# jewettaij/visfd

Hardware: AMD Instinct MI355X
Metric: Mvoxels/s (Gauss+DoG+TV pipeline) on 1024^3 float32; % HBM roofline (higher is better)
Workload: dtype f32

## Files before the change

include/visfd_hip.h:

```cpp
#ifndef VISFD_HIP_H
#define VISFD_HIP_H

#include <stddef.h>
#include <stdint.h>

#ifdef __cplusplus
extern "C" {
#endif

#define VISFD_HIP_OK 0
#define VISFD_HIP_EINVAL 1
#define VISFD_HIP_EDEVICE 2
#define VISFD_HIP_ENOMEM 3
#define VISFD_HIP_ECAPACITY 4

#define VISFD_HIP_INCREASING_EIVALS 0
#define VISFD_HIP_DECREASING_EIVALS 1

typedef struct visfd_hip_ctx visfd_hip_ctx;

int visfd_hip_create(int device, void* stream, visfd_hip_ctx** out);
int visfd_hip_destroy(visfd_hip_ctx* ctx);
int visfd_hip_synchronize(visfd_hip_ctx* ctx);
void* visfd_hip_get_stream(visfd_hip_ctx* ctx);
// ... 146 lines not shown
                              float threshold_tensor_saliency, float threshold_tensor_neighbor,
                              int tensor_is_positive_definite_near_target, int connectivity,
                              int64_t label_undefined, int sort_by_size, int standardize_directions,
                              int start_from_saliency_maxima, int64_t* n_clusters, float* cluster_maxima,
                              float* cluster_sizes, float* cluster_saliencies, int64_t cluster_capacity);
int visfd_hip_label_connected_ex(const float* saliency, int64_t* labels, const float* mask, int64_t nx, int64_t ny,
                              int64_t nz, float threshold_saliency, float* direction,
                              float threshold_vector_saliency, float threshold_vector_neighbor,
                              int consider_dot_product_sign, const float* tensor,
                              float threshold_tensor_saliency, float threshold_tensor_neighbor,
                              int tensor_is_positive_definite_near_target, int connectivity,
                              int64_t label_undefined, int sort_by_size, int standardize_directions,
                              int start_from_saliency_maxima, int64_t* n_clusters, float* cluster_maxima,
                              float* cluster_sizes, float* cluster_saliencies, int64_t cluster_capacity,
                                 const float* voxel_weights, const float* must_link_crds,
                                 const int64_t* must_link_group_sizes, int64_t must_link_ngroups,
                                 const int* must_link_directions);

int visfd_hip_principal_directions_host(const float* tensor, const float* mask, int64_t nvox, int order,
                                        float* direction);
int visfd_hip_tensor_saliency_host(const float* tensor, const float* mask, int64_t nvox, int order,
                                   float* saliency);

int visfd_hip_diagonalize_flat_sym3_host(const float* m6, float* out6, int64_t n, int eival_order);
int visfd_hip_convert_flat_sym2_evects3_host(const float* m6, int eival_order, float* eivals3, float* eivects9);
int visfd_hip_diagonalize_sym3_f32_host(const float* m9, int order, float* eivals3, float* eivects9);
int visfd_hip_surface_points(const float* saliency, const float* voxel2cluster, const float* direction,
                             const float* mask, int64_t nx, int64_t ny, int64_t nz, int select_cluster,
                             const float voxel_width[3], float curve_ds, int find_ridge,
                             float max_distance_to_feature, float* crds, float* norms, int64_t capacity,
                             int64_t* n_points);

int visfd_hip_bin_array3d(visfd_hip_ctx*, const float* src, const int64_t size_src[3], float* dst,
                          const int64_t size_dst[3], const int* offset);
int visfd_hip_bin_array3d_dev(visfd_hip_ctx*, const float* src, const int64_t size_src[3], float* dst,
                              const int64_t size_dst[3], const int* offset);
int visfd_hip_unbin_array3d(visfd_hip_ctx*, const float* src, const int64_t size_src[3], float* dst,
                            const int64_t size_dst[3], const int* offset);
int visfd_hip_unbin_array3d_dev(visfd_hip_ctx*, const float* src, const int64_t size_src[3], float* dst,
                                const int64_t size_dst[3], const int* offset);

int visfd_hip_calc_hessian(visfd_hip_ctx*, const float* src, float* gradient, float* hessian,
                           const float* mask, int64_t nx, int64_t ny, int64_t nz, float sigma,
                           float truncate_ratio);
int visfd_hip_calc_hessian_dev(visfd_hip_ctx*, const float* src, float* gradient, float* hessian,
                               const float* mask, int64_t nx, int64_t ny, int64_t nz, float sigma,
                               float truncate_ratio);

int visfd_hip_diagonalize_flat_sym3(visfd_hip_ctx*, const float* m6, float* out6, int64_t n,
                                    int eival_order);
int visfd_hip_diagonalize_flat_sym3_dev(visfd_hip_ctx*, const float* m6, float* out6, int64_t n,
                                        int eival_order);

int visfd_hip_hessian_saliency(visfd_hip_ctx*, const float* hessian, const float* mask,
                               int64_t nvox, int eival_order, float* saliency, float* direction);
int visfd_hip_hessian_saliency_dev(visfd_hip_ctx*, const float* hessian, const float* mask,
                                   int64_t nvox, int eival_order, float* saliency,
                                   float* direction);
int visfd_hip_ridge_saliency_dev(visfd_hip_ctx*, const float* src, const float* mask,
                                 int64_t nx, int64_t ny, int64_t nz, float sigma,
                                 float truncate_ratio, int eival_order, float* saliency,
                                 float* direction);
int visfd_hip_ridge_scores_dev(visfd_hip_ctx*, const float* src, const float* mask, int64_t nx, int64_t ny,
                               int64_t nz, float sigma, float truncate_ratio, int eival_order, float* saliency,
                               float* smoothed);
int visfd_hip_ridge_directions_dev(visfd_hip_ctx*, const float* smoothed, int64_t nx, int64_t ny, int64_t nz,
                                   float sigma, int eival_order, const float* saliency, float* direction);
int visfd_hip_peak_background_dev(visfd_hip_ctx*, const float* image, const float* mask, int64_t nx, int64_t ny, int64_t nz,
                                  float sigma_background, float truncate_ratio, int normalize, float* background);
int visfd_hip_ridge_scores_bg_dev(visfd_hip_ctx*, const float* src, const float* mask, int64_t nx, int64_t ny,
                                  int64_t nz, float sigma, float truncate_ratio, int eival_order, const float* background,
                                  float* saliency, float* smoothed);

int visfd_hip_threshold_fraction(visfd_hip_ctx*, float* saliency, const float* mask, int64_t nvox,
                                 float fraction, float* threshold_out);
int visfd_hip_threshold_fraction_dev(visfd_hip_ctx*, float* saliency, const float* mask,
                                     int64_t nvox, float fraction, float* threshold_out);
int visfd_hip_select_histogram_dev(visfd_hip_ctx*, const float* saliency, const float* mask,
                                   int64_t nvox, int round, uint32_t prefix,
                                   uint64_t* hist_host , uint64_t* n_unmasked_host);
int visfd_hip_select_histogram_todev(visfd_hip_ctx*, const float* saliency, const float* mask, int64_t nvox, int round,
                                     uint32_t prefix, uint64_t* hist_dev );
int visfd_hip_apply_threshold_dev(visfd_hip_ctx*, float* saliency, int64_t nvox, float threshold);

int visfd_hip_tv_dense_stick(visfd_hip_ctx*, const float* saliency, const float* direction,
                             float* tensor, const float* mask_src, const float* mask_dst,
                             int64_t nx, int64_t ny, int64_t nz, float sigma_tv, int exponent,
                             float cutoff_ratio, int detect_curves);
int visfd_hip_tv_dense_stick_dev(visfd_hip_ctx*, const float* saliency, const float* direction,
                                 float* tensor, const float* mask_src, const float* mask_dst,
                                 int64_t nx, int64_t ny, int64_t nz, float sigma_tv, int exponent,
                                 float cutoff_ratio, int detect_curves);
int visfd_hip_tv_dense_stick_slab_dev(visfd_hip_ctx*, const float* saliency, const float* direction,
                                      float* tensor, const float* mask_src, const float* mask_dst,
                                      int64_t nx, int64_t ny, int64_t nz_local, int64_t z_out0,
                                      int64_t z_out1, float sigma_tv, int exponent,
                                      float cutoff_ratio, int detect_curves);
int visfd_hip_tv_weight_sum(visfd_hip_ctx*, const float* saliency, float* den, const float* mask_src, const float* mask_dst,
                            int64_t nx, int64_t ny, int64_t nz, float sigma_tv, float cutoff_ratio);
int visfd_hip_tv_tables(float sigma_tv, float cutoff_ratio, int* halfwidth_out, float* w,
                        float* rhat);

int visfd_hip_tensor_saliency(visfd_hip_ctx*, const float* tensor, const float* mask, int64_t nvox,
                              int eival_order, float* saliency_inout);
int visfd_hip_tensor_saliency_dev(visfd_hip_ctx*, const float* tensor, const float* mask,
                                  int64_t nvox, int eival_order, float* saliency_inout);
int visfd_hip_tensor_saliency_bg_dev(visfd_hip_ctx*, const float* tensor, const float* mask, int64_t nvox, int eival_order,
                                     const float* image, const float* background, float* saliency_inout);

int visfd_hip_membrane_detect(visfd_hip_ctx*, const float* src, const float* mask,
                              int64_t nx, int64_t ny, int64_t nz, float sigma, float truncate_ratio,
                              int eival_order, float best_fraction, float threshold_abs, float sigma_tv,
                              int tv_exponent, float tv_cutoff_ratio, float* saliency_out,
                              float* tensor_out, float* direction_out, float* threshold_out);
int visfd_hip_membrane_detect_dev(visfd_hip_ctx*, const float* src, const float* mask,
                                  int64_t nx, int64_t ny, int64_t nz, float sigma, float truncate_ratio,
                                  int eival_order, float best_fraction, float threshold_abs,
                                  float sigma_tv, int tv_exponent, float tv_cutoff_ratio,
                                  float* saliency_out, float* tensor_out, float* direction_out,
                                  float* threshold_out);
int visfd_hip_membrane_detect_bg(visfd_hip_ctx*, const float* src, const float* mask,
                                 int64_t nx, int64_t ny, int64_t nz, float sigma, float truncate_ratio,
                                 int eival_order, float best_fraction, float threshold_abs, float sigma_tv,
                                 int tv_exponent, float tv_cutoff_ratio, float sigma_background, int normalize_background,
                                 float* saliency_out, float* tensor_out, float* direction_out, float* threshold_out);
int visfd_hip_membrane_detect_bg_dev(visfd_hip_ctx*, const float* src, const float* mask,
                                     int64_t nx, int64_t ny, int64_t nz, float sigma, float truncate_ratio,
                                     int eival_order, float best_fraction, float threshold_abs,
                                     float sigma_tv, int tv_exponent, float tv_cutoff_ratio, float sigma_background,
                                     int normalize_background, float* saliency_out, float* tensor_out, float* direction_out,
                                     float* threshold_out);

int visfd_hip_apply_gauss_slab_dev(visfd_hip_ctx*, const float* src, float* dst,
                                   int64_t nx, int64_t ny, int64_t nz_local, int64_t z_lo,
                                   int64_t nz_global, const float sigma[3], const int halfwidth[3],
                                   int normalize, float* A_out);

typedef struct visfd_hip_slab visfd_hip_slab;
typedef struct visfd_hip_transport {
  int (*sendrecv)(void* user, int peer, const void* sendbuf, void* recvbuf, size_t bytes, void* stream);
  int (*allreduce_sum_u64)(void* user, uint64_t* buf, size_t count, void* stream);
  int (*group_start)(void* user);
  int (*group_end)(void* user);
  void* user;
} visfd_hip_transport;
int visfd_hip_slab_unique_id(void* id_out_128_bytes);
int visfd_hip_slab_rccl_available(void);
int visfd_hip_slab_create_rccl(visfd_hip_ctx*, const void* unique_id_128_bytes , int rank,
                               int world, int64_t nz_global, int ghost, visfd_hip_slab** out);
int visfd_hip_slab_create_custom(visfd_hip_ctx*, const visfd_hip_transport*, int rank, int world, int64_t nz_global,
                                 int ghost, visfd_hip_slab** out);
int visfd_hip_slab_destroy(visfd_hip_slab*);
int visfd_hip_slab_layout(visfd_hip_slab*, int64_t out[7]);
int visfd_hip_slab_selftest(visfd_hip_slab*, int64_t count);
int visfd_hip_slab_set_reserve(visfd_hip_slab*, int reserve_workgroups);
int visfd_hip_slab_exchange_dev(visfd_hip_slab*, float* const* volumes, int nvol, int64_t nx, int64_t ny, int depth);
int visfd_hip_membrane_detect_slab_dev(visfd_hip_slab*, float* src, float* sal, float* dirs, float* tensor, float* scratch,
                                       int64_t nx, int64_t ny, float sigma, float truncate_ratio, int eival_order,
                                       float best_fraction, float sigma_tv, int exponent, float tv_truncate_ratio,
                                       int src_halo_ready, float* threshold_out);
int visfd_hip_membrane_detect_slab(visfd_hip_slab*, const float* src_owned, int64_t nx, int64_t ny, float sigma,
                                   float truncate_ratio, int eival_order, float best_fraction, float sigma_tv, int exponent,
                                   float tv_truncate_ratio, float* sal_owned, float* tensor_owned, float* threshold_out);
int visfd_hip_membrane_detect_slab_bg_dev(visfd_hip_slab*, float* src, float* sal, float* dirs, float* tensor, float* scratch,
                                          float* background, int64_t nx, int64_t ny, float sigma, float truncate_ratio,
                                          int eival_order, float best_fraction, float sigma_tv, int exponent,
                                          float tv_truncate_ratio, float sigma_background, int normalize_background,
                                          int src_halo_ready, float* threshold_out);
int visfd_hip_membrane_detect_slab_bg(visfd_hip_slab*, const float* src_owned, int64_t nx, int64_t ny, float sigma,
                                      float truncate_ratio, int eival_order, float best_fraction, float sigma_tv, int exponent,
                                      float tv_truncate_ratio, float sigma_background, int normalize_background,
                                      float* sal_owned, float* tensor_owned, float* threshold_out);
int visfd_hip_blob_dog_slab_dev(visfd_hip_slab*, float* src, int64_t nx, int64_t ny, const float* blob_sigma, int n_sigma,
                                float delta_sigma_over_sigma, float truncate_ratio, float minima_threshold,
                                float maxima_threshold, int src_halo_ready,
                                visfd_hip_blob* minima, int64_t minima_capacity, int64_t* n_minima,
                                visfd_hip_blob* maxima, int64_t maxima_capacity, int64_t* n_maxima);
int visfd_hip_blob_halo_depth(const float* blob_sigma, int n_sigma, float delta_sigma_over_sigma, float truncate_ratio,
                              int* depth_out);
int visfd_hip_apply_gauss_slab(visfd_hip_slab*, const float* src_owned, int64_t nx, int64_t ny, const float sigma[3],
                               const int halfwidth[3], int normalize, float* dst_owned, float* A_out);
int visfd_hip_blob_dog_slab(visfd_hip_slab*, const float* src_owned, int64_t nx, int64_t ny, const float* blob_sigma, int n_sigma,
                            float delta_sigma_over_sigma, float truncate_ratio, float minima_threshold, float maxima_threshold,
                            visfd_hip_blob* minima, int64_t minima_capacity, int64_t* n_minima,
                            visfd_hip_blob* maxima, int64_t maxima_capacity, int64_t* n_maxima);

#ifdef __cplusplus
}
#endif
#endif
```

visfd_amd/api.py:

```python
import ctypes as C
import os
import sys

import numpy as np

_HERE = os.path.dirname(os.path.abspath(__file__))
LIB_PATH = os.environ.get("VISFD_HIP_LIB") or os.path.join(_HERE, "libvisfd_hip.so")

INCREASING_EIVALS = 0
DECREASING_EIVALS = 1

MORPH_DILATE, MORPH_ERODE, MORPH_OPEN, MORPH_CLOSE, MORPH_TOP_HAT_WHITE, MORPH_TOP_HAT_BLACK = range(6)
MORPH_PATH_GENERAL, MORPH_PATH_XRUNS = 0, 1

_fp = C.POINTER(C.c_float)
_ip = C.POINTER(C.c_int)
_i64 = C.c_int64
_vp = C.c_void_p


class VisfdHipError(RuntimeError):
    def __init__(self, code, msg):
        super().__init__("visfd_hip error %d: %s" % (code, msg))
        self.code = code
# ... 15 lines not shown
    "visfd_hip_trim": (C.c_int, [_vp]),
    "visfd_hip_last_error": (C.c_char_p, []),
    "visfd_hip_abi_version": (C.c_int, []),
    "visfd_hip_workspace_bytes": (_i64, [_vp]),
    "visfd_hip_set_option": (C.c_int, [_vp, C.c_char_p, _i64]),
    "visfd_hip_get_option": (C.c_int, [_vp, C.c_char_p, C.POINTER(C.c_int64)]),
    "visfd_hip_gauss_taps": (C.c_int, [C.c_float, C.c_int, _fp]),
    "visfd_hip_ratio_from_threshold": (C.c_float, [C.c_float]),
    "visfd_hip_local_fluctuations": (C.c_int, [_vp, _vp, _vp, _vp, _i64, _i64, _i64, _fp, C.c_float, C.c_float, C.c_int]),
    "visfd_hip_local_fluctuations_dev": (C.c_int, [_vp, _vp, _vp, _vp, _i64, _i64, _i64, _fp, C.c_float, C.c_float, C.c_int]),
    "visfd_hip_sphere_structure": (C.c_int, [C.c_float, C.c_float, C.c_float, _ip, _fp, _i64, C.POINTER(C.c_int64)]),
    "visfd_hip_morph_sphere": (C.c_int, [_vp] + _VOL + [C.c_int, C.c_float, C.c_float, C.c_float]),
    "visfd_hip_morph_sphere_dev": (C.c_int, [_vp] + _VOL + [C.c_int, C.c_float, C.c_float, C.c_float]),
    "visfd_hip_morph_table": (C.c_int, [_vp] + _VOL + [C.c_int, _ip, _fp, _i64]),
    "visfd_hip_morph_table_dev": (C.c_int, [_vp] + _VOL + [C.c_int, _ip, _fp, _i64]),
    "visfd_hip_morph_last_path": (C.c_int, [_vp, _ip]),
    "visfd_hip_find_extrema": (C.c_int, [_vp, _vp, _vp, _i64, _i64, _i64] + _EXTREMA_TAIL),
    "visfd_hip_find_extrema_dev": (C.c_int, [_vp, _vp, _vp, _i64, _i64, _i64] + _EXTREMA_TAIL),
    "visfd_hip_fluctuation_sigmas": (C.c_int, [_fp, C.c_float, C.c_float, C.c_float, _fp, C.POINTER(C.c_float)]),
    "visfd_hip_gauss_halfwidths": (C.c_int, [_fp, C.c_float, _ip]),
    "visfd_hip_separable3d": (C.c_int, [_vp] + _VOL + [_fp, C.c_int, _fp, C.c_int, _fp, C.c_int, C.c_int, _fp]),
    "visfd_hip_separable3d_dev": (C.c_int, [_vp] + _VOL + [_fp, C.c_int, _fp, C.c_int, _fp, C.c_int, C.c_int, _fp]),
    "visfd_hip_apply_gauss": (C.c_int, [_vp] + _VOL + [_fp, _ip, C.c_int, _fp]),
    "visfd_hip_apply_gauss_dev": (C.c_int, [_vp] + _VOL + [_fp, _ip, C.c_int, _fp]),
    "visfd_hip_apply_gauss_slab_dev": (C.c_int, [_vp, _vp, _vp, _i64, _i64, _i64, _i64, _i64, _fp, _ip, C.c_int, _fp]),
    "visfd_hip_apply_dog": (C.c_int, [_vp] + _VOL + [_fp, _fp, _ip, _fp, _fp]),
    "visfd_hip_apply_dog_dev": (C.c_int, [_vp] + _VOL + [_fp, _fp, _ip, _fp, _fp]),
    "visfd_hip_apply_log": (C.c_int, [_vp] + _VOL + [_fp, C.c_float, C.c_float, _fp, _fp]),
    "visfd_hip_apply_log_dev": (C.c_int, [_vp] + _VOL + [_fp, C.c_float, C.c_float, _fp, _fp]),
    "visfd_hip_blob_dog": (C.c_int, [_vp, _vp, _vp, _i64, _i64, _i64, _fp, C.c_int, _fp, C.c_float, C.c_float,
                                     C.c_float, C.c_float, C.c_int, C.POINTER(Blob), _i64, C.POINTER(_i64),
                                     C.POINTER(Blob), _i64, C.POINTER(_i64)]),
    "visfd_hip_blob_dog_dev": (C.c_int, [_vp, _vp, _vp, _i64, _i64, _i64, _fp, C.c_int, _fp, C.c_float, C.c_float,
                                         C.c_float, C.c_float, C.c_int, C.POINTER(Blob), _i64, C.POINTER(_i64),
                                         C.POINTER(Blob), _i64, C.POINTER(_i64)]),
    "visfd_hip_blob_dog_begin_dev": (C.c_int, [_vp, _vp, _vp, _i64, _i64, _i64, _fp, C.c_int, _fp, C.c_float, C.c_float,
                                               C.c_float, C.c_float, C.c_int, C.POINTER(_vp)]),
    "visfd_hip_blob_dog_end": (C.c_int, [_vp, C.POINTER(Blob), _i64, C.POINTER(_i64), C.POINTER(Blob), _i64, C.POINTER(_i64)]),
    "visfd_hip_blob_dog_abort": (None, [_vp]),
    "visfd_hip_blob_jobs_pending": (C.c_int, [_vp]),
    "visfd_hip_debug_poison_workspace": (C.c_int, [_vp]),
    "visfd_hip_blob_diameters_to_sigmas": (C.c_int, [_fp, C.c_int, _fp]),
    "visfd_hip_blob_sigmas_to_diameters": (C.c_int, [_fp, C.c_int, _fp]),
    "visfd_hip_calc_hessian": (C.c_int, [_vp, _vp, _vp, _vp, _vp, _i64, _i64, _i64, C.c_float, C.c_float]),
    "visfd_hip_calc_hessian_dev": (C.c_int, [_vp, _vp, _vp, _vp, _vp, _i64, _i64, _i64, C.c_float, C.c_float]),
    "visfd_hip_diagonalize_flat_sym3": (C.c_int, [_vp, _vp, _vp, _i64, C.c_int]),
    "visfd_hip_diagonalize_flat_sym3_dev": (C.c_int, [_vp, _vp, _vp, _i64, C.c_int]),
    "visfd_hip_hessian_saliency": (C.c_int, [_vp, _vp, _vp, _i64, C.c_int, _vp, _vp]),
    "visfd_hip_hessian_saliency_dev": (C.c_int, [_vp, _vp, _vp, _i64, C.c_int, _vp, _vp]),
    "visfd_hip_ridge_saliency_dev": (C.c_int, [_vp, _vp, _vp, _i64, _i64, _i64, C.c_float, C.c_float, C.c_int,
                                               _vp, _vp]),
    "visfd_hip_ridge_scores_dev": (C.c_int, [_vp, _vp, _vp, _i64, _i64, _i64, C.c_float, C.c_float, C.c_int, _vp, _vp]),
    "visfd_hip_ridge_directions_dev": (C.c_int, [_vp, _vp, _i64, _i64, _i64, C.c_float, C.c_int, _vp, _vp]),
    "visfd_hip_threshold_fraction": (C.c_int, [_vp, _vp, _vp, _i64, C.c_float, _fp]),
    "visfd_hip_threshold_fraction_dev": (C.c_int, [_vp, _vp, _vp, _i64, C.c_float, _fp]),
    "visfd_hip_select_histogram_dev": (C.c_int, [_vp, _vp, _vp, _i64, C.c_int, C.c_uint32,
                                                 C.POINTER(C.c_uint64), C.POINTER(C.c_uint64)]),
    "visfd_hip_select_histogram_todev": (C.c_int, [_vp, _vp, _vp, _i64, C.c_int, C.c_uint32, _vp]),
    "visfd_hip_get_stream": (_vp, [_vp]),
    "visfd_hip_apply_threshold_dev": (C.c_int, [_vp, _vp, _i64, C.c_float]),
    "visfd_hip_tv_dense_stick": (C.c_int, [_vp, _vp, _vp, _vp, _vp, _vp, _i64, _i64, _i64, C.c_float, C.c_int,
                                           C.c_float, C.c_int]),
    "visfd_hip_tv_dense_stick_dev": (C.c_int, [_vp, _vp, _vp, _vp, _vp, _vp, _i64, _i64, _i64, C.c_float, C.c_int,
                                               C.c_float, C.c_int]),
    "visfd_hip_tv_dense_stick_slab_dev": (C.c_int, [_vp, _vp, _vp, _vp, _vp, _vp, _i64, _i64, _i64, _i64, _i64,
                                                    C.c_float, C.c_int, C.c_float, C.c_int]),
    "visfd_hip_tv_tables": (C.c_int, [C.c_float, C.c_float, _ip, _fp, _fp]),
    "visfd_hip_tv_weight_sum": (C.c_int, [_vp, _vp, _vp, _vp, _vp, _i64, _i64, _i64, C.c_float, C.c_float]),
    "visfd_hip_membrane_detect": (C.c_int, [_vp, _vp, _vp, _i64, _i64, _i64, C.c_float, C.c_float, C.c_int, C.c_float,
                                            C.c_float, C.c_float, C.c_int, C.c_float, _vp, _vp, _vp, _fp]),
    "visfd_hip_membrane_detect_dev": (C.c_int, [_vp, _vp, _vp, _i64, _i64, _i64, C.c_float, C.c_float, C.c_int,
                                                C.c_float, C.c_float, C.c_float, C.c_int, C.c_float, _vp, _vp, _vp,
                                                _fp]),
    "visfd_hip_tensor_saliency": (C.c_int, [_vp, _vp, _vp, _i64, C.c_int, _vp]),
    "visfd_hip_tensor_saliency_dev": (C.c_int, [_vp, _vp, _vp, _i64, C.c_int, _vp]),
    "visfd_hip_peak_background_dev": (C.c_int, [_vp, _vp, _vp, _i64, _i64, _i64, C.c_float, C.c_float, C.c_int, _vp]),
    "visfd_hip_ridge_scores_bg_dev": (C.c_int, [_vp, _vp, _vp, _i64, _i64, _i64, C.c_float, C.c_float, C.c_int, _vp, _vp, _vp]),
    "visfd_hip_tensor_saliency_bg_dev": (C.c_int, [_vp, _vp, _vp, _i64, C.c_int, _vp, _vp, _vp]),
    "visfd_hip_membrane_detect_bg": (C.c_int, [_vp, _vp, _vp, _i64, _i64, _i64, C.c_float, C.c_float, C.c_int, C.c_float,
                                               C.c_float, C.c_float, C.c_int, C.c_float, C.c_float, C.c_int, _vp, _vp, _vp, _fp]),
    "visfd_hip_membrane_detect_bg_dev": (C.c_int, [_vp, _vp, _vp, _i64, _i64, _i64, C.c_float, C.c_float, C.c_int,
                                                   C.c_float, C.c_float, C.c_float, C.c_int, C.c_float, C.c_float, C.c_int,
                                                   _vp, _vp, _vp, _fp]),
    "visfd_hip_membrane_detect_slab_bg_dev": (C.c_int, [_vp, _vp, _vp, _vp, _vp, _vp, _vp, _i64, _i64, C.c_float, C.c_float, C.c_int,
                                                        C.c_float, C.c_float, C.c_int, C.c_float, C.c_float, C.c_int, C.c_int, _fp]),
    "visfd_hip_membrane_detect_slab_bg": (C.c_int, [_vp, _vp, _i64, _i64, C.c_float, C.c_float, C.c_int, C.c_float, C.c_float,
                                                    C.c_int, C.c_float, C.c_float, C.c_int, _vp, _vp, _fp]),
    "visfd_hip_bin_array3d": (C.c_int, [_vp, _vp, C.POINTER(_i64), _vp, C.POINTER(_i64), _ip]),
    "visfd_hip_bin_array3d_dev": (C.c_int, [_vp, _vp, C.POINTER(_i64), _vp, C.POINTER(_i64), _ip]),
    "visfd_hip_unbin_array3d": (C.c_int, [_vp, _vp, C.POINTER(_i64), _vp, C.POINTER(_i64), _ip]),
    "visfd_hip_unbin_array3d_dev": (C.c_int, [_vp, _vp, C.POINTER(_i64), _vp, C.POINTER(_i64), _ip]),
    "visfd_hip_label_connected": (C.c_int, [_vp, _vp, _vp, _i64, _i64, _i64, C.c_float, _vp, C.c_float, C.c_float, C.c_int,
                                            _vp, C.c_float, C.c_float, C.c_int, C.c_int, _i64, C.c_int, C.c_int, C.c_int,
                                            C.POINTER(_i64), _vp, _vp, _vp, _i64]),
    "visfd_hip_label_connected_ex": (C.c_int, [_vp, _vp, _vp, _i64, _i64, _i64, C.c_float, _vp, C.c_float, C.c_float, C.c_int,
                                               _vp, C.c_float, C.c_float, C.c_int, C.c_int, _i64, C.c_int, C.c_int, C.c_int,
                                               C.POINTER(_i64), _vp, _vp, _vp, _i64, _vp, _vp, _vp, _i64, _vp]),
    "visfd_hip_principal_directions_host": (C.c_int, [_vp, _vp, _i64, C.c_int, _vp]),
    "visfd_hip_tensor_saliency_host": (C.c_int, [_vp, _vp, _i64, C.c_int, _vp]),
    "visfd_hip_diagonalize_sym3_f32_host": (C.c_int, [_vp, C.c_int, _vp, _vp]),
    "visfd_hip_diagonalize_flat_sym3_host": (C.c_int, [_vp, _vp, _i64, C.c_int]),
    "visfd_hip_convert_flat_sym2_evects3_host": (C.c_int, [_vp, C.c_int, _vp, _vp]),
    "visfd_hip_surface_points": (C.c_int, [_vp, _vp, _vp, _vp, _i64, _i64, _i64, C.c_int, _fp, C.c_float, C.c_int, C.c_float,
                                           _vp, _vp, _i64, C.POINTER(_i64)]),
    "visfd_hip_sphere_overlap": (C.c_float, [C.c_float, C.c_float, C.c_float]),
    "visfd_hip_sort_blobs": (C.c_int, [_fp, _fp, _fp, _i64, C.c_int, C.c_int, C.POINTER(C.c_uint64)]),
    "visfd_hip_discard_masked_blobs": (C.c_int, [_fp, _fp, _fp, C.POINTER(_i64), _vp, _i64, _i64, _i64]),
    "visfd_hip_discard_overlapping_blobs": (C.c_int, [_fp, _fp, _fp, C.POINTER(_i64), C.c_float, C.c_float,
                                                     C.c_float, C.c_int, C.c_int]),
    "visfd_hip_slab_unique_id": (C.c_int, [_vp]),
    "visfd_hip_slab_create_rccl": (C.c_int, [_vp, _vp, C.c_int, C.c_int, _i64, C.c_int, C.POINTER(_vp)]),
    "visfd_hip_slab_create_custom": (C.c_int, [_vp, _vp, C.c_int, C.c_int, _i64, C.c_int, C.POINTER(_vp)]),
    "visfd_hip_slab_destroy": (C.c_int, [_vp]),
    "visfd_hip_slab_layout": (C.c_int, [_vp, C.POINTER(_i64)]),
    "visfd_hip_slab_set_reserve": (C.c_int, [_vp, C.c_int]),
    "visfd_hip_slab_rccl_available": (C.c_int, []),
    "visfd_hip_apply_gauss_slab": (C.c_int, [_vp, _vp, _i64, _i64, _fp, _ip, C.c_int, _vp, _fp]),
    "visfd_hip_blob_dog_slab": (C.c_int, [_vp, _vp, _i64, _i64, _fp, C.c_int, C.c_float, C.c_float, C.c_float, C.c_float,
                                          _vp, _i64, C.POINTER(_i64), _vp, _i64, C.POINTER(_i64)]),
    "visfd_hip_blob_halo_depth": (C.c_int, [_fp, C.c_int, C.c_float, C.c_float, _ip]),
    "visfd_hip_slab_selftest": (C.c_int, [_vp, _i64]),
    "visfd_hip_slab_exchange_dev": (C.c_int, [_vp, C.POINTER(_vp), C.c_int, _i64, _i64, C.c_int]),
    "visfd_hip_membrane_detect_slab_dev": (C.c_int, [_vp, _vp, _vp, _vp, _vp, _vp, _i64, _i64, C.c_float, C.c_float, C.c_int,
                                                     C.c_float, C.c_float, C.c_int, C.c_float, C.c_int, _fp]),
    "visfd_hip_membrane_detect_slab": (C.c_int, [_vp, _vp, _i64, _i64, C.c_float, C.c_float, C.c_int, C.c_float, C.c_float,
                                                 C.c_int, C.c_float, _vp, _vp, _fp]),
    "visfd_hip_blob_dog_slab_dev": (C.c_int, [_vp, _vp, _i64, _i64, _fp, C.c_int, C.c_float, C.c_float, C.c_float, C.c_float,
                                              C.c_int, _vp, _i64, C.POINTER(_i64), _vp, _i64, C.POINTER(_i64)]),
}

_SENDRECV = C.CFUNCTYPE(C.c_int, _vp, C.c_int, _vp, _vp, C.c_size_t, _vp)
_ALLREDUCE = C.CFUNCTYPE(C.c_int, _vp, _vp, C.c_size_t, _vp)
_GROUP = C.CFUNCTYPE(C.c_int, _vp)


class Transport(C.Structure):
    _fields_ = [("sendrecv", _SENDRECV), ("allreduce_sum_u64", _ALLREDUCE), ("group_start", _GROUP), ("group_end", _GROUP),
                ("user", _vp)]

_lib = None


def load_library():
    global _lib
    if _lib is None:
        if not os.path.exists(LIB_PATH):
            raise ImportError("%s is missing: build it with `python -m visfd_amd.build` "
                              "(there is no CPU fallback)" % LIB_PATH)
        try:
            import torch
        except ImportError:
            pass
        lib = C.CDLL(LIB_PATH)
        for name, (res, args) in _SIGS.items():
            fn = getattr(lib, name)
            fn.restype = res
            fn.argtypes = args
        _lib = lib
    return _lib


def exported_symbols():
    return sorted(_SIGS)


def _np(a):
# ... 540 lines not shown
        self._chk(self._L.visfd_hip_hessian_saliency(self._h, _np(hess), _np(mask), sal.size, int(order), _np(sal),
                                                     _np(dirs)))
        return sal, dirs

    def threshold_fraction(self, sal, fraction, mask=None):
        thr = C.c_float()
        self._chk(self._L.visfd_hip_threshold_fraction(self._h, _np(sal), _np(mask), sal.size, float(fraction),
                                                       C.byref(thr)))
        return thr.value

    def tv_dense_stick(self, sal, dirs, sigma_tv, exponent=4, cutoff=2.0 ** 0.5, mask_src=None, mask_dst=None,
                       curves=False):
        nz, ny, nx = sal.shape
        tensor = np.zeros((nz, ny, nx, 6), np.float32)
        self._chk(self._L.visfd_hip_tv_dense_stick(self._h, _np(sal), _np(dirs), _np(tensor), _np(mask_src),
                                                   _np(mask_dst), nx, ny, nz, float(sigma_tv), int(exponent),
                                                   float(cutoff), int(curves)))
        return tensor

    def tv_weight_sum(self, sal, sigma_tv, cutoff=2.0 ** 0.5, mask_src=None, mask_dst=None):
        nz, ny, nx = sal.shape
        den = np.zeros_like(sal)
        self._chk(self._L.visfd_hip_tv_weight_sum(self._h, _np(sal), _np(den), _np(mask_src), _np(mask_dst), nx, ny, nz,
                                                  float(sigma_tv), float(cutoff)))
        return den

    def tensor_saliency(self, tensor, order, sal_inout, mask=None):
        self._chk(self._L.visfd_hip_tensor_saliency(self._h, _np(tensor), _np(mask), sal_inout.size, int(order),
                                                    _np(sal_inout)))
        return sal_inout

    @staticmethod
    def _sizes(shape):
        return (_i64 * 3)(int(shape[2]), int(shape[1]), int(shape[0]))

    def bin_array3d(self, src, dst_shape, offset=None):
        dst = np.empty(tuple(dst_shape), np.float32)
        self._chk(self._L.visfd_hip_bin_array3d(self._h, _np(src), self._sizes(src.shape), _np(dst),
                                                self._sizes(dst_shape), _i3(offset) if offset is not None else None))
        return dst

    def unbin_array3d(self, src, dst_shape, offset=None):
        dst = np.empty(tuple(dst_shape), np.float32)
        self._chk(self._L.visfd_hip_unbin_array3d(self._h, _np(src), self._sizes(src.shape), _np(dst),
                                                  self._sizes(dst_shape), _i3(offset) if offset is not None else None))
        return dst

    def bin_array3d_dev(self, src, dst, offset=None):
        self._chk(self._L.visfd_hip_bin_array3d_dev(self._h, _dev(src), self._sizes(src.shape), _dev(dst),
                                                    self._sizes(dst.shape), _i3(offset) if offset is not None else None))

    def unbin_array3d_dev(self, src, dst, offset=None):
        self._chk(self._L.visfd_hip_unbin_array3d_dev(self._h, _dev(src), self._sizes(src.shape), _dev(dst),
                                                      self._sizes(dst.shape), _i3(offset) if offset is not None else None))

    def membrane_detect(self, src, sigma, ratio, order, best_fraction=0.05, threshold_abs=0.0, sigma_tv=0.0,
                        tv_exponent=4, tv_cutoff=2.0 ** 0.5, mask=None, want_tensor=True, want_dir=False,
                        sigma_background=0.0, normalize_background=True):
        nz, ny, nx = src.shape
        sal = np.empty_like(src)
        ten = np.zeros((nz, ny, nx, 6), np.float32) if want_tensor else None
        dirs = np.zeros((nz, ny, nx, 3), np.float32) if want_dir else None
        thr = C.c_float()
        self._chk(self._L.visfd_hip_membrane_detect_bg(self._h, _np(src), _np(mask), nx, ny, nz, float(sigma),
                                                       float(ratio), int(order), float(best_fraction),
                                                       float(threshold_abs), float(sigma_tv), int(tv_exponent),
                                                       float(tv_cutoff), float(sigma_background), int(bool(normalize_background)),
                                                       _np(sal), _np(ten), _np(dirs), C.byref(thr)))
        return sal, ten, dirs, thr.value

    def membrane_detect_dev(self, src, sal, sigma, ratio, order, best_fraction=0.05, threshold_abs=0.0, sigma_tv=0.0,
                            tv_exponent=4, tv_cutoff=2.0 ** 0.5, mask=None, dirs=None, tensor=None, sigma_background=0.0,
                            normalize_background=True):
        nz, ny, nx = src.shape
        thr = C.c_float()
        self._chk(self._L.visfd_hip_membrane_detect_bg_dev(self._h, _dev(src), _dev(mask), nx, ny, nz, float(sigma),
                                                           float(ratio), int(order), float(best_fraction),
                                                           float(threshold_abs), float(sigma_tv), int(tv_exponent),
                                                           float(tv_cutoff), float(sigma_background),
                                                           int(bool(normalize_background)), _dev(sal), _dev(tensor), _dev(dirs),
                                                           C.byref(thr)))
        return thr.value

    def gauss_dev(self, src, dst, sigma, hw, mask=None, normalize=True):
        nz, ny, nx = src.shape
        A = C.c_float()
        self._chk(self._L.visfd_hip_apply_gauss_dev(self._h, _dev(src), _dev(dst), _dev(mask), nx, ny, nz,
                                                    _f3(sigma), _i3(hw), int(normalize), C.byref(A)))
        return A.value

    def local_fluctuations_dev(self, src, dst, sigma, ratio, mask=None, normalize=True, exponent=2.0):
        nz, ny, nx = src.shape
        self._chk(self._L.visfd_hip_local_fluctuations_dev(self._h, _dev(src), _dev(dst), _dev(mask), nx, ny, nz,
                                                           _f3(sigma), float(exponent), float(ratio), int(normalize)))

    def morph_sphere_dev(self, op, src, dst, radius, radius_max=0.0, bmax=0.0, mask=None):
        nz, ny, nx = src.shape
        self._chk(self._L.visfd_hip_morph_sphere_dev(self._h, _dev(src), _dev(dst), _dev(mask), nx, ny, nz, int(op),
                                                     float(radius), float(radius_max), float(bmax)))

    def dilate_sphere_dev(self, src, dst, radius, radius_max=0.0, bmax=0.0, mask=None):
        self.morph_sphere_dev(MORPH_DILATE, src, dst, radius, radius_max, bmax, mask)

    def erode_sphere_dev(self, src, dst, radius, radius_max=0.0, bmax=0.0, mask=None):
        self.morph_sphere_dev(MORPH_ERODE, src, dst, radius, radius_max, bmax, mask)

    def open_sphere_dev(self, src, dst, radius, radius_max=0.0, bmax=0.0, mask=None):
        self.morph_sphere_dev(MORPH_OPEN, src, dst, radius, radius_max, bmax, mask)

    def close_sphere_dev(self, src, dst, radius, radius_max=0.0, bmax=0.0, mask=None):
        self.morph_sphere_dev(MORPH_CLOSE, src, dst, radius, radius_max, bmax, mask)

    def white_top_hat_sphere_dev(self, src, dst, radius, radius_max=0.0, bmax=0.0, mask=None):
        self.morph_sphere_dev(MORPH_TOP_HAT_WHITE, src, dst, radius, radius_max, bmax, mask)

    def black_top_hat_sphere_dev(self, src, dst, radius, radius_max=0.0, bmax=0.0, mask=None):
        self.morph_sphere_dev(MORPH_TOP_HAT_BLACK, src, dst, radius, radius_max, bmax, mask)

    def find_extrema_dev(self, src, mask=None, find_minima=True, find_maxima=True, minima_threshold=float("inf"),
                         maxima_threshold=-float("inf"), connectivity=3, allow_borders=True, labels=None):
        if labels is not None:
            assert labels.is_cuda and labels.is_contiguous() and str(labels.dtype) == "torch.int32" and \
                tuple(labels.shape) == tuple(src.shape), "labels: contiguous cuda int32 of src's shape"
        return tuple(self._find_extrema(self._L.visfd_hip_find_extrema_dev, _dev(src), _dev(mask), tuple(src.shape),
                                        find_minima, find_maxima, minima_threshold, maxima_threshold, connectivity,
                                        allow_borders, None if labels is None else labels.data_ptr()))

    def morph_table_dev(self, op, src, dst, dxyz, b, mask=None):
        nz, ny, nx = src.shape
        d, bb = _morph_table(dxyz, b)
        self._chk(self._L.visfd_hip_morph_table_dev(self._h, _dev(src), _dev(dst), _dev(mask), nx, ny, nz, int(op),
                                                    d.ctypes.data_as(_ip), bb.ctypes.data_as(_fp), len(bb)))

    def dilate_dev(self, src, dst, dxyz, b, mask=None):
        self.morph_table_dev(MORPH_DILATE, src, dst, dxyz, b, mask)

    def erode_dev(self, src, dst, dxyz, b, mask=None):
        self.morph_table_dev(MORPH_ERODE, src, dst, dxyz, b, mask)

    def gauss_slab_dev(self, src, dst, z_lo, nz_global, sigma, hw, normalize=True):
        nz, ny, nx = src.shape
        A = C.c_float()
        self._chk(self._L.visfd_hip_apply_gauss_slab_dev(self._h, _dev(src), _dev(dst), nx, ny, nz, int(z_lo),
                                                         int(nz_global), _f3(sigma), _i3(hw), int(normalize),
                                                         C.byref(A)))
        return A.value

    def log_dev(self, src, dst, sigma, delta, ratio, mask=None):
        nz, ny, nx = src.shape
        self._chk(self._L.visfd_hip_apply_log_dev(self._h, _dev(src), _dev(dst), _dev(mask), nx, ny, nz,
                                                  _f3(sigma), float(delta), float(ratio), None, None))

    def blob_dog_dev(self, src, sigmas, mask=None, aspect=None, delta=0.02, ratio=2.5, minima_threshold=np.inf,
                     maxima_threshold=-np.inf, use_ratios=False, cap=1 << 16):
        return self._blob_call(self._L.visfd_hip_blob_dog_dev, _dev(src), _dev(mask), tuple(src.shape), sigmas,
                               aspect, delta, ratio, minima_threshold, maxima_threshold, use_ratios, cap)

    def calc_hessian_dev(self, src, grad, hess, sigma, ratio, mask=None):
        nz, ny, nx = src.shape
        self._chk(self._L.visfd_hip_calc_hessian_dev(self._h, _dev(src), _dev(grad), _dev(hess), _dev(mask), nx,
                                                     ny, nz, float(sigma), float(ratio)))

    def hessian_saliency_dev(self, hess, sal, dirs, order, mask=None):
        self._chk(self._L.visfd_hip_hessian_saliency_dev(self._h, _dev(hess), _dev(mask), sal.numel(), int(order),
                                                         _dev(sal), _dev(dirs)))

# ... 265 lines not shown
```

visfd_amd/build.py:

```python
import concurrent.futures
import os
import subprocess
import sys
import time

HERE = os.path.dirname(os.path.abspath(__file__))
ROOT = os.path.dirname(HERE)
CSRC = os.path.join(HERE, "csrc")
OBJDIR = os.path.join(ROOT, "build", "visfd_hip")
LIB = os.path.join(HERE, "libvisfd_hip.so")

SOURCES = ["host_math.cpp", "blob_post.cpp", "connect.cpp", "context.hip", "api.hip", "blob_job.hip", "gauss.hip", "blob.hip", "select.hip", "tv.hip", "resample.hip", "slab.hip", "morph.hip", "extrema.hip"]
TV_VARIANT = [("tv_tiled.hip", "tv_tiled", ["-fno-slp-vectorize"]), ("tv_box.hip", "tv_box", ["-fno-slp-vectorize"]),
              ("ridge.hip", "ridge", [])]
VARIANTS = TV_VARIANT + [("gauss_fused.hip", "gauss_fused_h%d" % h, ["-DVH_FUSED_H=%d" % h, "-fno-slp-vectorize"])
                         for h in range(1, 9)]
HEADERS = ["common.hpp", "eigen3.hpp", os.path.join("..", "..", "include", "visfd_hip.h")]

HIPCC = os.environ.get("HIPCC", "/opt/rocm/bin/hipcc")
FLAGS = ["--offload-arch=gfx950", "-O3", "-std=c++17", "-fPIC", "-ffp-contract=off", "-fno-fast-math",
         "-Wall", "-Wno-unused-function"]


def _mtime(p):
    return os.path.getmtime(p) if os.path.exists(p) else 0.0


def _compile(src, obj, extra=()):
    t0 = time.time()
    cmd = [HIPCC] + FLAGS + list(extra) + ["-x", "hip", "-c", os.path.join(CSRC, src), "-o", obj]
    r = subprocess.run(cmd, capture_output=True, text=True)
    return src, r.returncode, r.stdout + r.stderr, time.time() - t0


def build(force=False, jobs=4, verbose=True):
    os.makedirs(OBJDIR, exist_ok=True)
    newest_header = max(_mtime(os.path.join(CSRC, h)) for h in HEADERS)
    todo, objs = [], []
    units = [(s, os.path.splitext(s)[0], []) for s in SOURCES] + VARIANTS
    flagfile = os.path.join(OBJDIR, "flags.txt")
    flagsig = repr((FLAGS, VARIANTS))
    if not os.path.exists(flagfile) or open(flagfile).read() != flagsig:
        force = True
    for s, stem, extra in units:
        obj = os.path.join(OBJDIR, stem + ".o")
        objs.append(obj)
        if force or _mtime(obj) < max(_mtime(os.path.join(CSRC, s)), newest_header):
            todo.append((s, obj, extra))
    if todo:
        with concurrent.futures.ThreadPoolExecutor(max_workers=jobs) as ex:
            for (src, rc, out, dt), (_, obj, _e) in zip(ex.map(lambda a: _compile(*a), todo), todo):
                if verbose:
                    print("[visfd_amd.build] %-22s %5.1fs %s" % (os.path.basename(obj), dt, "ok" if rc == 0 else "FAILED"))
                if rc != 0:
                    sys.stderr.write(out)
                    raise RuntimeError("hipcc failed on " + src)
                elif out.strip() and verbose:
                    sys.stderr.write(out)
    with open(flagfile, "w") as f:
        f.write(flagsig)
    if todo or not os.path.exists(LIB) or _mtime(LIB) < max(_mtime(o) for o in objs):
        cmd = [HIPCC, "--offload-arch=gfx950", "-shared", "-fPIC", "-o", LIB] + objs
        r = subprocess.run(cmd, capture_output=True, text=True)
        if r.returncode != 0:
            sys.stderr.write(r.stdout + r.stderr)
            raise RuntimeError("link failed")
        if verbose:
            print("[visfd_amd.build] linked", LIB)
    build_cli(verbose)
    return LIB


CLI_SRC = os.path.join(HERE, "cli", "filter_mrc.cpp")
CLI_BIN = os.path.join(HERE, "cli", "filter_mrc")


def build_cli(verbose=True):
    deps = [CLI_SRC, os.path.join(ROOT, "include", "visfd_hip.hpp"), os.path.join(ROOT, "include", "visfd_hip.h"), LIB]
    if os.path.exists(CLI_BIN) and _mtime(CLI_BIN) >= max(_mtime(d) for d in deps):
        return CLI_BIN
    cmd = ["g++", "-std=c++11", "-O2", "-Wall", "-o", CLI_BIN, CLI_SRC, "-L" + HERE, "-lvisfd_hip",
           "-Wl,-rpath,$ORIGIN/..", "-Wl,-rpath,/opt/rocm/lib"]
    r = subprocess.run(cmd, capture_output=True, text=True)
    if r.returncode != 0:
        sys.stderr.write(r.stdout + r.stderr)
        raise RuntimeError("building filter_mrc failed")
    if verbose:
        print("[visfd_amd.build] built", CLI_BIN)
    return CLI_BIN


if __name__ == "__main__":
    j = 4
    if "-j" in sys.argv:
        j = int(sys.argv[sys.argv.index("-j") + 1])
    build(force="--force" in sys.argv, jobs=j)
```

visfd_amd/csrc/api.hip:

```cpp
#include <algorithm>
#include <cmath>
#include <vector>

#include "common.hpp"

namespace vh {

int gauss_dev(visfd_hip_ctx* ctx, const float* src, float* dst, const float* mask, i64 nx, i64 ny, i64 nz,
              const float sigma[3], const int hw[3], bool normalize, SlabInfo slab, float* A_out, const float* minuend,
              float log_scale, bool* epilogue_done, bool fma) {
  VH_REQUIRE(ctx && src && dst && sigma && hw, "null argument");
  std::vector<float> t[3];
  for (int d = 0; d < 3; d++) {
    VH_REQUIRE(sigma[d] >= 0.0f, "sigma must be non-negative");
    VH_REQUIRE(hw[d] >= 0 && hw[d] <= MAX_HALFWIDTH, "filter halfwidth must be in [0, 64]");
    t[d].resize(2 * hw[d] + 1);
    host_gauss_taps(sigma[d], hw[d], t[d].data());
  }
  return dev_separable3d(ctx, src, dst, mask, nx, ny, nz, t[0].data(), hw[0], t[1].data(), hw[1],
                         t[2].data(), hw[2], normalize, slab, A_out, minuend, log_scale, epilogue_done, fma);
}

static int dog_dev(visfd_hip_ctx* ctx, const float* src, float* dst, float* tmp, const float* mask, i64 nx, i64 ny,
                   i64 nz, const float sa[3], const float sb[3], const int hw[3], float scale, bool do_scale,
                   float* A, float* B) {
  const SlabInfo whole = {0, nz};
  VH_TRY(gauss_dev(ctx, src, dst, mask, nx, ny, nz, sa, hw, true, whole, A));
  {
    bool fused = false;
    VH_TRY(gauss_dev(ctx, src, dst, mask, nx, ny, nz, sb, hw, true, whole, B, dst, do_scale ? scale : 1.0f, &fused));
    if (fused) return VISFD_HIP_OK;
  }
  VH_TRY(gauss_dev(ctx, src, tmp, mask, nx, ny, nz, sb, hw, true, whole, B));
  return dev_sub_scale(ctx, dst, tmp, nx * ny * nz, scale, do_scale);
}

LogPlan plan_log(const float sigma[3], float delta, float ratio) {
  LogPlan p;
  for (int d = 0; d < 3; d++) {
    p.sa[d] = (float)(sigma[d] * (1.0 - 0.5 * delta));
    p.sb[d] = (float)(sigma[d] * (1.0 + 0.5 * delta));
    p.hw[d] = (int)std::floor(ratio * std::fmax(p.sa[d], p.sb[d]));
  }
  p.scale = (float)(1.0 / (delta * delta));
  return p;
}

int log_dev(visfd_hip_ctx* ctx, const float* src, float* dst, float* tmp, const float* mask, i64 nx, i64 ny,
            i64 nz, const float sigma[3], float delta, float ratio, float* A, float* B) {
  const LogPlan p = plan_log(sigma, delta, ratio);
  for (int d = 0; d < 3; d++)
    VH_REQUIRE(p.hw[d] >= 0 && p.hw[d] <= MAX_HALFWIDTH, "LoG filter halfwidth must be in [0, 64]");
  float a = 0, b = 0;
  VH_TRY(dog_dev(ctx, src, dst, tmp, mask, nx, ny, nz, p.sa, p.sb, p.hw, p.scale, true, &a, &b));
  if (A) *A = a * p.scale;
  if (B) *B = b * p.scale;
  return VISFD_HIP_OK;
}

namespace {

void halfwidths_from_ratio(const float sigma[3], float ratio, int hw[3]) {
  for (int d = 0; d < 3; d++) {
    hw[d] = (int)std::floor(sigma[d] * ratio);
    if (hw[d] < 1) hw[d] = 1;
  }
}

int gauss_iso_dev(visfd_hip_ctx* ctx, const float* src, float* dst, const float* mask, i64 nx, i64 ny, i64 nz, float sigma,
                  float ratio, bool normalize, const char* what, float** out = nullptr) {
  const int hwv = (int)std::floor(sigma * ratio);
  VH_REQUIRE(hwv >= 0 && hwv <= MAX_HALFWIDTH, std::string(what) + " must be in [0, 64]");
  if (!dst) VH_TRY(ws(ctx, WS_D, (size_t)(nx * ny * nz), &dst));
  if (out) *out = dst;
  const float sg[3] = {sigma, sigma, sigma};
  const int hw[3] = {hwv, hwv, hwv};
  const SlabInfo whole = {0, nz};
  return gauss_dev(ctx, src, dst, mask, nx, ny, nz, sg, hw, normalize, whole, nullptr);
}

int calc_hessian_dev(visfd_hip_ctx* ctx, const float* src, float* grad, float* hess, const float* mask,
                     i64 nx, i64 ny, i64 nz, float sigma, float ratio) {
  VH_REQUIRE(ctx && src, "null argument");
  VH_TRY(check_dims(nx, ny, nz));
  float* S = nullptr;
  VH_TRY(gauss_iso_dev(ctx, src, nullptr, mask, nx, ny, nz, sigma, ratio, true, "filter halfwidth", &S));
  return dev_hessian(ctx, S, mask, nx, ny, nz, sigma, grad, hess);
// ... 178 lines not shown
int visfd_hip_calc_hessian_dev(visfd_hip_ctx* ctx, const float* src, float* grad, float* hess,
                               const float* mask, int64_t nx, int64_t ny, int64_t nz, float sigma,
                               float ratio) {
  VH_REQUIRE(ctx, "null context");
  VH_HIP(hipSetDevice(ctx->device));
  return calc_hessian_dev(ctx, src, grad, hess, mask, nx, ny, nz, sigma, ratio);
}

int visfd_hip_calc_hessian(visfd_hip_ctx* ctx, const float* src, float* grad, float* hess, const float* mask,
                           int64_t nx, int64_t ny, int64_t nz, float sigma, float ratio) {
  VH_REQUIRE(ctx && src, "null argument");
  VH_HIP(hipSetDevice(ctx->device));
  VH_TRY(check_dims(nx, ny, nz));
  const Stage st = {ctx, (size_t)(nx * ny * nz)};
  float *ds, *dm, *dg = nullptr, *dh = nullptr, *aos = nullptr;
  VH_TRY(st.up(WS_H2D_0, src, &ds));
  VH_TRY(st.up(WS_H2D_1, mask, &dm));
  if (grad) VH_TRY(st.out(WS_H2D_2, &dg, 3));
  if (hess) VH_TRY(st.out(WS_H2D_3, &dh, 6));
  VH_TRY(st.out(WS_H2D_4, &aos, 6));
  VH_TRY(calc_hessian_dev(ctx, ds, dg, dh, dm, nx, ny, nz, sigma, ratio));
  if (grad) VH_TRY(st.down_interleaved(grad, dg, aos, 3, dm, true));
  if (hess) VH_TRY(st.down_interleaved(hess, dh, aos, 6, dm, true));
  return VISFD_HIP_OK;
}

int visfd_hip_diagonalize_flat_sym3_dev(visfd_hip_ctx* ctx, const float* m6, float* out6, int64_t n,
                                        int order) {
  VH_REQUIRE(ctx && m6 && out6 && n >= 0, "bad argument");
  VH_REQUIRE(order == 0 || order == 1, "unsupported eigenvalue order");
  VH_HIP(hipSetDevice(ctx->device));
  if (n == 0) return VISFD_HIP_OK;
  return dev_diagonalize(ctx, m6, out6, n, order);
}

int visfd_hip_diagonalize_flat_sym3(visfd_hip_ctx* ctx, const float* m6, float* out6, int64_t n, int order) {
  VH_REQUIRE(ctx && m6 && out6 && n >= 0, "bad argument");
  VH_REQUIRE(order == 0 || order == 1, "unsupported eigenvalue order");
  VH_HIP(hipSetDevice(ctx->device));
  if (n == 0) return VISFD_HIP_OK;
  const Stage st = {ctx, (size_t)n};
  float *aos, *pin, *pout;
  VH_TRY(st.up_planar(WS_H2D_0, WS_H2D_1, m6, 6, &pin, &aos));
  VH_TRY(st.out(WS_H2D_2, &pout, 6));
  VH_TRY(dev_diagonalize(ctx, pin, pout, n, order));
  return st.down_interleaved(out6, pout, aos, 6, nullptr, false);
}

int visfd_hip_hessian_saliency_dev(visfd_hip_ctx* ctx, const float* hess, const float* mask, int64_t nvox,
                                   int order, float* sal, float* dir) {
  VH_REQUIRE(ctx && hess && sal && dir && nvox > 0, "bad argument");
  VH_REQUIRE(order == 0 || order == 1, "unsupported eigenvalue order");
  VH_HIP(hipSetDevice(ctx->device));
  return dev_hessian_saliency(ctx, hess, mask, nvox, order, sal, dir);
}

int visfd_hip_hessian_saliency(visfd_hip_ctx* ctx, const float* hess, const float* mask, int64_t nvox, int order,
                               float* sal, float* dir) {
  VH_REQUIRE(ctx && hess && sal && dir && nvox > 0, "bad argument");
  VH_REQUIRE(order == 0 || order == 1, "unsupported eigenvalue order");
  VH_HIP(hipSetDevice(ctx->device));
  const Stage st = {ctx, (size_t)nvox};
  float *aos, *ph, *dm, *dsal, *pdir;
  VH_TRY(st.up_planar(WS_H2D_0, WS_H2D_2, hess, 6, &ph, &aos));
  VH_TRY(st.up(WS_H2D_1, mask, &dm));
  VH_TRY(st.out(WS_H2D_3, &dsal));
  VH_TRY(st.out(WS_H2D_4, &pdir, 3));
  VH_TRY(dev_hessian_saliency(ctx, ph, dm, nvox, order, dsal, pdir));
  VH_TRY(st.down(sal, dsal));
  return st.down_interleaved(dir, pdir, aos, 3, dm, true);
}

int visfd_hip_ridge_saliency_dev(visfd_hip_ctx* ctx, const float* src, const float* mask, int64_t nx, int64_t ny,
                                 int64_t nz, float sigma, float ratio, int order, float* sal, float* dir) {
  VH_REQUIRE(ctx && src && sal && dir, "null argument");
  VH_REQUIRE(order == 0 || order == 1, "unsupported eigenvalue order");
  VH_HIP(hipSetDevice(ctx->device));
  VH_TRY(check_dims(nx, ny, nz));
  float* S = nullptr;
  VH_TRY(gauss_iso_dev(ctx, src, nullptr, mask, nx, ny, nz, sigma, ratio, true, "filter halfwidth", &S));
  return dev_ridge_saliency_fused(ctx, S, mask, nx, ny, nz, sigma, order, sal, dir);
}

int visfd_hip_ridge_scores_bg_dev(visfd_hip_ctx* ctx, const float* src, const float* mask, int64_t nx, int64_t ny,
                                  int64_t nz, float sigma, float ratio, int order, const float* background, float* sal,
                                  float* smoothed) {
  VH_REQUIRE(ctx && src && sal && smoothed, "null argument");
  VH_REQUIRE(smoothed != src && smoothed != sal, "the smoothed volume needs its own buffer");
  VH_REQUIRE(order == 0 || order == 1, "unsupported eigenvalue order");
  VH_HIP(hipSetDevice(ctx->device));
  VH_TRY(check_dims(nx, ny, nz));
  VH_TRY(gauss_iso_dev(ctx, src, smoothed, mask, nx, ny, nz, sigma, ratio, true, "filter halfwidth"));
  return dev_ridge_score(ctx, smoothed, mask, nx, ny, nz, sigma, order, sal, background ? src : nullptr, background);
}
int visfd_hip_ridge_scores_dev(visfd_hip_ctx* ctx, const float* src, const float* mask, int64_t nx, int64_t ny,
                               int64_t nz, float sigma, float ratio, int order, float* sal, float* smoothed) {
  return visfd_hip_ridge_scores_bg_dev(ctx, src, mask, nx, ny, nz, sigma, ratio, order, nullptr, sal, smoothed);
}
int visfd_hip_peak_background_dev(visfd_hip_ctx* ctx, const float* src, const float* mask, int64_t nx, int64_t ny,
                                  int64_t nz, float sigma_background, float ratio, int normalize, float* background) {
  VH_REQUIRE(ctx && src && background && background != src, "bad argument");
  VH_REQUIRE(sigma_background > 0.0f, "the background width must be positive");
  VH_HIP(hipSetDevice(ctx->device));
  VH_TRY(check_dims(nx, ny, nz));
  return gauss_iso_dev(ctx, src, background, mask, nx, ny, nz, sigma_background, ratio, normalize != 0,
                       "background filter halfwidth");
}

int visfd_hip_ridge_directions_dev(visfd_hip_ctx* ctx, const float* smoothed, int64_t nx, int64_t ny, int64_t nz,
                                   float sigma, int order, const float* sal, float* dir) {
  VH_REQUIRE(ctx && smoothed && sal && dir, "null argument");
  VH_REQUIRE(order == 0 || order == 1, "unsupported eigenvalue order");
  VH_HIP(hipSetDevice(ctx->device));
  VH_TRY(check_dims(nx, ny, nz));
  return dev_ridge_directions(ctx, smoothed, sal, nx, ny, nz, sigma, order, dir);
}

int visfd_hip_threshold_fraction_dev(visfd_hip_ctx* ctx, float* sal, const float* mask, int64_t nvox,
                                     float fraction, float* thr_out) {
  VH_REQUIRE(ctx && sal && nvox > 0, "bad argument");
  VH_REQUIRE(fraction >= 0.0f && fraction <= 1.0f, "fraction must be in [0,1]");
  VH_HIP(hipSetDevice(ctx->device));
  return dev_threshold_fraction(ctx, sal, mask, nvox, fraction, thr_out);
}

int visfd_hip_threshold_fraction(visfd_hip_ctx* ctx, float* sal, const float* mask, int64_t nvox, float fraction,
                                 float* thr_out) {
  VH_REQUIRE(ctx && sal && nvox > 0, "bad argument");
  VH_REQUIRE(fraction >= 0.0f && fraction <= 1.0f, "fraction must be in [0,1]");
  VH_HIP(hipSetDevice(ctx->device));
  const Stage st = {ctx, (size_t)nvox};
  float *ds, *dm;
  VH_TRY(st.up(WS_H2D_0, sal, &ds));
  VH_TRY(st.up(WS_H2D_1, mask, &dm));
  VH_TRY(dev_threshold_fraction(ctx, ds, dm, nvox, fraction, thr_out));
  return st.down(sal, ds);
}

int visfd_hip_select_histogram_dev(visfd_hip_ctx* ctx, const float* sal, const float* mask, int64_t nvox,
                                   int pass, uint32_t prefix, uint64_t* hist_host, uint64_t* n_unmasked) {
  VH_REQUIRE(ctx && sal && hist_host && nvox > 0, "bad argument");
  VH_REQUIRE(pass >= 0 && pass <= 2, "round must be 0, 1 or 2");
  VH_HIP(hipSetDevice(ctx->device));
  return dev_select_histogram(ctx, sal, mask, nvox, pass, prefix, hist_host, n_unmasked);
}

int visfd_hip_select_histogram_todev(visfd_hip_ctx* ctx, const float* sal, const float* mask, int64_t nvox, int pass,
                                     uint32_t prefix, uint64_t* hist_dev) {
  VH_REQUIRE(ctx && sal && hist_dev && nvox > 0, "bad argument");
  VH_REQUIRE(pass >= 0 && pass <= 2, "round must be 0, 1 or 2");
  VH_HIP(hipSetDevice(ctx->device));
  return dev_select_histogram_todev(ctx, sal, mask, nvox, pass, prefix, hist_dev);
}

int visfd_hip_apply_threshold_dev(visfd_hip_ctx* ctx, float* sal, int64_t nvox, float thr) {
  VH_REQUIRE(ctx && sal && nvox > 0, "bad argument");
  VH_HIP(hipSetDevice(ctx->device));
  return dev_apply_threshold(ctx, sal, nvox, thr);
}

int visfd_hip_bin_array3d_dev(visfd_hip_ctx* ctx, const float* src, const int64_t size_src[3], float* dst,
                              const int64_t size_dst[3], const int* offset) {
  VH_REQUIRE(ctx && src && dst && size_src && size_dst, "null argument");
  VH_HIP(hipSetDevice(ctx->device));
  return dev_bin_array3d(ctx, src, size_src, dst, size_dst, offset);
}

int visfd_hip_unbin_array3d_dev(visfd_hip_ctx* ctx, const float* src, const int64_t size_src[3], float* dst,
                                const int64_t size_dst[3], const int* offset) {
  VH_REQUIRE(ctx && src && dst && size_src && size_dst, "null argument");
  VH_HIP(hipSetDevice(ctx->device));
  return dev_unbin_array3d(ctx, src, size_src, dst, size_dst, offset);
}

static int resample_host(visfd_hip_ctx* ctx, const float* src, const int64_t size_src[3], float* dst, const int64_t size_dst[3],
                         const int* offset, decltype(dev_bin_array3d)* run) {
  VH_REQUIRE(ctx && src && dst && size_src && size_dst, "null argument");
  VH_HIP(hipSetDevice(ctx->device));
  VH_TRY(check_dims(size_src[0], size_src[1], size_src[2]));
  VH_TRY(check_dims(size_dst[0], size_dst[1], size_dst[2]));
  const Stage in = {ctx, (size_t)(size_src[0] * size_src[1] * size_src[2])};
  const Stage res = {ctx, (size_t)(size_dst[0] * size_dst[1] * size_dst[2])};
  float *ds, *dd;
  VH_TRY(in.up(WS_H2D_0, src, &ds));
  VH_TRY(res.out(WS_H2D_2, &dd));
  VH_TRY(run(ctx, ds, size_src, dd, size_dst, offset));
  return res.down(dst, dd);
}

int visfd_hip_bin_array3d(visfd_hip_ctx* ctx, const float* src, const int64_t size_src[3], float* dst,
                          const int64_t size_dst[3], const int* offset) {
  return resample_host(ctx, src, size_src, dst, size_dst, offset, dev_bin_array3d);
}
int visfd_hip_unbin_array3d(visfd_hip_ctx* ctx, const float* src, const int64_t size_src[3], float* dst,
                            const int64_t size_dst[3], const int* offset) {
  return resample_host(ctx, src, size_src, dst, size_dst, offset, dev_unbin_array3d);
}

int visfd_hip_tv_tables(float sigma_tv, float cutoff, int* h_out, float* w, float* rhat) {
  const int h = host_tv_halfwidth(sigma_tv, cutoff);
  VH_REQUIRE(h >= 0, "negative window");
  if (h_out) *h_out = h;
  if (w) host_tv_tables(sigma_tv, h, w, rhat);
  return VISFD_HIP_OK;
}

int visfd_hip_tv_dense_stick_slab_dev(visfd_hip_ctx* ctx, const float* sal, const float* dir, float* ten,
                                      const float* mask_src, const float* mask_dst, int64_t nx,
                                      int64_t ny, int64_t nz_local, int64_t z_out0, int64_t z_out1,
                                      float sigma_tv, int exponent, float cutoff, int curves) {
  VH_REQUIRE(ctx && sal && dir && ten, "null argument");
  VH_HIP(hipSetDevice(ctx->device));
  return dev_tv_dense_stick(ctx, sal, dir, ten, mask_src, mask_dst, nx, ny, nz_local, z_out0, z_out1,
                            sigma_tv, exponent, cutoff, curves != 0);
}

int visfd_hip_tv_dense_stick_dev(visfd_hip_ctx* ctx, const float* sal, const float* dir, float* ten,
                                 const float* mask_src, const float* mask_dst, int64_t nx, int64_t ny,
                                 int64_t nz, float sigma_tv, int exponent, float cutoff, int curves) {
  return visfd_hip_tv_dense_stick_slab_dev(ctx, sal, dir, ten, mask_src, mask_dst, nx, ny, nz, 0, nz,
                                           sigma_tv, exponent, cutoff, curves);
}

int visfd_hip_tv_dense_stick(visfd_hip_ctx* ctx, const float* sal, const float* dir, float* ten, const float* mask_src,
                             const float* mask_dst, int64_t nx, int64_t ny, int64_t nz, float sigma_tv, int exponent,
                             float cutoff, int curves) {
  VH_REQUIRE(ctx && sal && dir && ten, "null argument");
  VH_HIP(hipSetDevice(ctx->device));
  VH_TRY(check_dims(nx, ny, nz));
  const Stage st = {ctx, (size_t)(nx * ny * nz)};
  float *dsal, *pdir, *pten, *aos6, *dms = nullptr, *dmd = nullptr;
  VH_TRY(st.up(WS_H2D_0, sal, &dsal));
  VH_TRY(st.up_planar(WS_H2D_1, WS_H2D_2, dir, 3, &pdir));
  VH_TRY(st.out(WS_H2D_3, &pten, 6));
  VH_TRY(st.up(WS_H2D_4, mask_src, &dms));
  if (mask_dst == mask_src) dmd = dms;
  else VH_TRY(st.up(WS_A, mask_dst, &dmd));
  VH_TRY(dev_tv_dense_stick(ctx, dsal, pdir, pten, dms, dmd, nx, ny, nz, 0, nz, sigma_tv, exponent, cutoff, curves != 0));
  VH_TRY(st.out(WS_B, &aos6, 6));
  return st.down_interleaved(ten, pten, aos6, 6, dmd, true);
}

int visfd_hip_tv_weight_sum(visfd_hip_ctx* ctx, const float* sal, float* den, const float* mask_src,
                            const float* mask_dst, int64_t nx, int64_t ny, int64_t nz, float sigma_tv, float cutoff) {
  VH_REQUIRE(ctx && sal && den, "null argument");
  VH_HIP(hipSetDevice(ctx->device));
  VH_TRY(check_dims(nx, ny, nz));
  const Stage st = {ctx, (size_t)(nx * ny * nz)};
  float *dsal, *dden, *dms = nullptr, *dmd = nullptr;
  VH_TRY(st.up(WS_H2D_0, sal, &dsal));
  VH_TRY(st.up(WS_H2D_1, den, &dden));
  VH_TRY(st.up(WS_H2D_4, mask_src, &dms));
  if (mask_dst == mask_src) dmd = dms;
  else VH_TRY(st.up(WS_A, mask_dst, &dmd));
  VH_TRY(dev_tv_weight_sum(ctx, dsal, dden, dms, dmd, nx, ny, nz, sigma_tv, cutoff));
  return st.down(den, dden);
}

int visfd_hip_membrane_detect_bg_dev(visfd_hip_ctx* ctx, const float* src, const float* mask, int64_t nx,
                                     int64_t ny, int64_t nz, float sigma, float ratio, int order,
                                     float best_fraction, float threshold_abs, float sigma_tv, int exponent,
                                     float cutoff, float sigma_background, int normalize_background, float* sal, float* ten,
                                     float* dir, float* thr_out) {
  VH_REQUIRE(ctx && src && sal, "null argument");
  VH_REQUIRE(order == 0 || order == 1, "unsupported eigenvalue order");
  VH_REQUIRE(best_fraction <= 1.0f, "fraction must be <= 1");
  VH_HIP(hipSetDevice(ctx->device));
  VH_TRY(check_dims(nx, ny, nz));
  const i64 n = nx * ny * nz;
  float* d = dir;
  if (!d) VH_TRY(ws(ctx, WS_TVAUX, (size_t)(3 * n), &d));
  float* smoothed = nullptr;
  VH_TRY(ws(ctx, WS_D, (size_t)n, &smoothed));
  float* bg = nullptr;
  if (sigma_background > 0.0f) {
    VH_TRY(ws(ctx, WS_C, (size_t)n, &bg));
    VH_TRY(visfd_hip_peak_background_dev(ctx, src, mask, nx, ny, nz, sigma_background, ratio, normalize_background, bg));
  }
  VH_TRY(visfd_hip_ridge_scores_bg_dev(ctx, src, mask, nx, ny, nz, sigma, ratio, order, bg, sal, smoothed));
  float thr = threshold_abs;
  if (best_fraction >= 0.0f) VH_TRY(dev_threshold_fraction(ctx, sal, mask, n, best_fraction, &thr));
  else VH_TRY(dev_apply_threshold(ctx, sal, n, thr));
  if (thr_out) *thr_out = thr;
  if (dir) VH_HIP(hipMemsetAsync(dir, 0, sizeof(float) * 3 * (size_t)n, ctx->stream));
  VH_TRY(dev_ridge_directions(ctx, smoothed, sal, nx, ny, nz, sigma, order, d));
  if (sigma_tv > 0.0f) {
    float* t = ten;
    if (!t) VH_TRY(ws(ctx, WS_B, (size_t)(6 * n), &t));
    VH_TRY(dev_tv_dense_stick(ctx, sal, d, t, mask, mask, nx, ny, nz, 0, nz, sigma_tv, exponent, cutoff, false));
    VH_TRY(dev_tensor_saliency(ctx, t, mask, n, order, sal, bg ? src : nullptr, bg));
  }
  return VISFD_HIP_OK;
}
int visfd_hip_membrane_detect_dev(visfd_hip_ctx* ctx, const float* src, const float* mask, int64_t nx,
                                  int64_t ny, int64_t nz, float sigma, float ratio, int order,
                                  float best_fraction, float threshold_abs, float sigma_tv, int exponent,
                                  float cutoff, float* sal, float* ten, float* dir, float* thr_out) {
  return visfd_hip_membrane_detect_bg_dev(ctx, src, mask, nx, ny, nz, sigma, ratio, order, best_fraction, threshold_abs, sigma_tv,
                                          exponent, cutoff, 0.0f, 1, sal, ten, dir, thr_out);
}

int visfd_hip_membrane_detect_bg(visfd_hip_ctx* ctx, const float* src, const float* mask, int64_t nx, int64_t ny,
                                 int64_t nz, float sigma, float ratio, int order, float best_fraction,
                                 float threshold_abs, float sigma_tv, int exponent, float cutoff,
                                 float sigma_background, int normalize_background, float* sal, float* ten, float* dir,
                                 float* thr_out) {
  VH_REQUIRE(ctx && src && sal, "null argument");
  VH_HIP(hipSetDevice(ctx->device));
  VH_TRY(check_dims(nx, ny, nz));
  const Stage st = {ctx, (size_t)(nx * ny * nz)};
  float *ds, *dm, *dsal, *pdir, *pten = nullptr, *aos = nullptr;
  VH_TRY(st.up(WS_H2D_0, src, &ds));
  VH_TRY(st.up(WS_H2D_1, mask, &dm));
  VH_TRY(st.out(WS_H2D_2, &dsal));
  VH_TRY(st.out(WS_H2D_3, &pdir, 3));
  if (ten && sigma_tv > 0.0f) {
    VH_TRY(st.out(WS_H2D_4, &pten, 6));
    VH_HIP(hipMemsetAsync(pten, 0, sizeof(float) * 6 * st.n, ctx->stream));
  }
  VH_TRY(visfd_hip_membrane_detect_bg_dev(ctx, ds, dm, nx, ny, nz, sigma, ratio, order, best_fraction, threshold_abs, sigma_tv,
                                          exponent, cutoff, sigma_background, normalize_background, dsal, pten, pdir, thr_out));
  VH_TRY(st.down(sal, dsal));
  if ((ten && pten) || dir) VH_TRY(st.out(WS_A, &aos, 6));
  if (ten && pten) VH_TRY(st.down_interleaved(ten, pten, aos, 6, nullptr, false));
  if (dir) VH_TRY(st.down_interleaved(dir, pdir, aos, 3, nullptr, false));
  return VISFD_HIP_OK;
}
int visfd_hip_membrane_detect(visfd_hip_ctx* ctx, const float* src, const float* mask, int64_t nx, int64_t ny,
                              int64_t nz, float sigma, float ratio, int order, float best_fraction,
                              float threshold_abs, float sigma_tv, int exponent, float cutoff, float* sal,
                              float* ten, float* dir, float* thr_out) {
  return visfd_hip_membrane_detect_bg(ctx, src, mask, nx, ny, nz, sigma, ratio, order, best_fraction, threshold_abs, sigma_tv,
                                      exponent, cutoff, 0.0f, 1, sal, ten, dir, thr_out);
}

int visfd_hip_tensor_saliency_bg_dev(visfd_hip_ctx* ctx, const float* ten, const float* mask, int64_t nvox,
                                     int order, const float* image, const float* background, float* sal) {
  VH_REQUIRE(ctx && ten && sal && nvox > 0, "bad argument");
  VH_REQUIRE((image == nullptr) == (background == nullptr), "image and background come as a pair");
  VH_REQUIRE(order == 0 || order == 1, "unsupported eigenvalue order");
  VH_HIP(hipSetDevice(ctx->device));
  return dev_tensor_saliency(ctx, ten, mask, nvox, order, sal, image, background);
}
int visfd_hip_tensor_saliency_dev(visfd_hip_ctx* ctx, const float* ten, const float* mask, int64_t nvox,
                                  int order, float* sal) {
  return visfd_hip_tensor_saliency_bg_dev(ctx, ten, mask, nvox, order, nullptr, nullptr, sal);
}

int visfd_hip_tensor_saliency(visfd_hip_ctx* ctx, const float* ten, const float* mask, int64_t nvox, int order,
                              float* sal) {
  VH_REQUIRE(ctx && ten && sal && nvox > 0, "bad argument");
  VH_REQUIRE(order == 0 || order == 1, "unsupported eigenvalue order");
  VH_HIP(hipSetDevice(ctx->device));
  const Stage st = {ctx, (size_t)nvox};
  float *pten, *dm, *dsal;
  VH_TRY(st.up_planar(WS_H2D_0, WS_H2D_1, ten, 6, &pten));
  VH_TRY(st.up(WS_H2D_2, mask, &dm));
  VH_TRY(st.up(WS_H2D_3, sal, &dsal));
  VH_TRY(dev_tensor_saliency(ctx, pten, dm, nvox, order, dsal));
  return st.down(sal, dsal);
}

int visfd_hip_morph_last_path(visfd_hip_ctx* ctx, int* path) {
  VH_REQUIRE(ctx && path, "null argument");
  *path = ctx->morph_last_path;
  return VISFD_HIP_OK;
}

int visfd_hip_sphere_structure(float radius, float radius_max, float bmax, int* dxyz, float* b, int64_t cap,
                               int64_t* n) {
  VH_REQUIRE(n && cap >= 0 && (cap == 0 || (dxyz && b)), "bad argument");
  VH_REQUIRE(std::isfinite(radius) && std::isfinite(radius_max) && std::isfinite(bmax),
             "sphere radii and bmax must be finite");
  VH_REQUIRE(std::ceil(std::max(radius, radius_max)) <= 128.0f, "sphere radius must be at most 128 voxels");
  *n = host_sphere_structure(radius, radius_max, bmax, dxyz, b, cap);
  if (cap > 0 && cap < *n) return fail(VISFD_HIP_ECAPACITY, "structuring element has more entries than cap");
  return VISFD_HIP_OK;
}

int visfd_hip_morph_sphere_dev(visfd_hip_ctx* ctx, const float* src, float* dst, const float* mask, int64_t nx,
                               int64_t ny, int64_t nz, int op, float radius, float radius_max, float bmax) {
  VH_TRY(morph_check(ctx, src, dst, mask, nx, ny, nz, op, VISFD_HIP_MORPH_TOP_HAT_BLACK));
  int64_t n = 0;
  VH_TRY(visfd_hip_sphere_structure(radius, radius_max, bmax, nullptr, nullptr, 0, &n));
  std::vector<int> dxyz((size_t)(3 * n + 3));
  std::vector<float> b((size_t)(n + 1));
  VH_TRY(visfd_hip_sphere_structure(radius, radius_max, bmax, dxyz.data(), b.data(), n + 1, &n));
  MorphElem el;
  VH_TRY(morph_put_table(ctx, dxyz.data(), b.data(), n, &el));
  return morph_run(ctx, src, dst, mask, nx, ny, nz, op, el);
}

int visfd_hip_morph_sphere(visfd_hip_ctx* ctx, const float* src, float* dst, const float* mask, int64_t nx, int64_t ny,
                           int64_t nz, int op, float radius, float radius_max, float bmax) {
  VH_TRY(morph_check(ctx, src, dst, mask, nx, ny, nz, op, VISFD_HIP_MORPH_TOP_HAT_BLACK));
  return stage_filter(ctx, src, dst, mask, nx, ny, nz, true, [&](const float* ds, float* dd, const float* dm) {
    return visfd_hip_morph_sphere_dev(ctx, ds, dd, dm, nx, ny, nz, op, radius, radius_max, bmax);
  });
// ... 55 lines not shown
```

visfd_amd/csrc/common.hpp:

```cpp
#pragma once

#include <hip/hip_runtime.h>

#include <cstdint>
#include <cstdio>
#include <cstring>
#include <string>
#include <vector>

#include "../../include/visfd_hip.h"

namespace vh {

typedef int64_t i64;

void set_error(const std::string& msg);
int fail(int code, const std::string& msg);

#define VH_HIP(expr)                                                                         \
  do {                                                                                       \
    hipError_t _e = (expr);                                                                  \
    if (_e != hipSuccess)                                                                    \
      return vh::fail(_e == hipErrorOutOfMemory ? VISFD_HIP_ENOMEM : VISFD_HIP_EDEVICE,      \
                      std::string(#expr) + ": " + hipGetErrorString(_e));                    \
  } while (0)

#define VH_TRY(expr)           \
  do {                         \
    int _rc = (expr);          \
    if (_rc != VISFD_HIP_OK) return _rc; \
  } while (0)

#define VH_REQUIRE(cond, msg) \
  do {                        \
    if (!(cond)) return vh::fail(VISFD_HIP_EINVAL, msg); \
  } while (0)

enum Slot {
  WS_A = 0, WS_B, WS_C, WS_D,
  WS_DEN_A, WS_DEN_B,
  WS_NORM,
  WS_LOG0, WS_LOG1, WS_LOG2,
  WS_CAND, WS_COUNTER,
  WS_SCANCNT,
  WS_HIST,
  WS_TVTAB,
  WS_TVAUX,
  WS_TVSCRATCH,
  WS_TVLIST,
  WS_H2D_0, WS_H2D_1, WS_H2D_2, WS_H2D_3, WS_H2D_4,
  WS_MORPH_TAB,
  WS_MORPH_SRC,
  WS_MORPH_TMP,
  WS_EXT_FLAGS,
  WS_EXT_PARENT,
  WS_EXT_COUNT,
  WS_EXT_COUNTERS,
  WS_EXT_LIST,
  WS_EXT_RANKS,
  WS_NSLOTS
};

struct BlobJob;

}

struct visfd_hip_options {
  int gauss_3pass = 0;
  int gauss_cfg = 0;
  int gauss_wg_per_cu = 2;
  int tv_dense = 0;
  int tv_fma = 0;
  int gauss_fma = 0;
  int eig_f32 = 0;
  int tv_zrun = 0;
  int tv_no_replay = 0;
  int tv_exact_tiled = 0;
  int tv_no_fold = 0;
  int tv_poison = 0;
  int tv_reserve_wg = 0;
  int tv_max_wg = 0;
  int64_t blob_test_cap = 0;
  int morph_general = 0;
  int debug = 0;
};

struct visfd_hip_ctx {
  visfd_hip_options opt;
  float* tv_table_dev = nullptr;
  float tv_table_key[2] = {0.0f, 0.0f};
  int tv_table_h = -1;
  int device = 0;
  hipStream_t stream = nullptr;
  bool own_stream = false;
  void* slot_ptr[vh::WS_NSLOTS] = {};
  size_t slot_bytes[vh::WS_NSLOTS] = {};
  int num_cus = 256;
  hipStream_t aux_stream = nullptr;
  std::vector<int> morph_tab;
  int morph_last_path = -1;
  std::vector<vh::BlobJob*> blob_jobs;
};

namespace vh {

int blob_jobs_drain(visfd_hip_ctx* ctx, const BlobJob* except = nullptr);
void blob_jobs_abort(visfd_hip_ctx* ctx);

int ws_get(visfd_hip_ctx* ctx, Slot s, size_t bytes, void** out);
template <typename T>
inline int ws(visfd_hip_ctx* ctx, Slot s, size_t count, T** out) {
  void* p = nullptr;
  int rc = ws_get(ctx, s, count * sizeof(T), &p);
  *out = static_cast<T*>(p);
  return rc;
}

inline int check_dims(i64 nx, i64 ny, i64 nz) {
  if (nx <= 0 || ny <= 0 || nz <= 0) return fail(VISFD_HIP_EINVAL, "image dimensions must be positive");
  return VISFD_HIP_OK;
}
inline int check_dims32(i64 nx, i64 ny, i64 nz) {
  if (nx >= (1LL << 31) || ny >= (1LL << 31) || nz >= (1LL << 31)) return fail(VISFD_HIP_EINVAL, "dimension too large");
  return VISFD_HIP_OK;
}

constexpr int MAX_HALFWIDTH = 64;
struct Taps {
  float t[2 * MAX_HALFWIDTH + 1];
  int h;
};

inline int tv_padded_row(int h) {
  int sp = 2 * h + 1;
  while ((sp & 7) != 4) sp++;
  return sp;
}

inline int tv_box_row(int h) {
  int sp = 2 * h + 1 + 3;
  while ((sp & 7) != 4) sp++;
  return sp;
}
inline int tv_box_slice(int h) { return (2 * h + 1 + 6) * tv_box_row(h) + 8; }

void host_gauss_taps(float sigma, int h, float* t);
void host_conv_ones(i64 n, const float* t, int h, float* out);
int host_tv_halfwidth(float sigma, float cutoff);
void host_tv_tables(float sigma, int h, float* w, float* rhat);
float host_gengauss3d_peak(const float width[3], float m_exp, float ratio);
i64 host_sphere_structure(float radius, float radius_max, float bmax, int* dxyz, float* b, i64 cap);

struct SlabInfo {
  i64 z_lo;
  i64 nz_global;
};

int dev_separable3d(visfd_hip_ctx* ctx, const float* src, float* dst, const float* mask, i64 nx,
                    i64 ny, i64 nz, const float* tx, int hx, const float* ty, int hy,
                    const float* tz, int hz, bool normalize, SlabInfo slab, float* A_out,
                    const float* minuend = nullptr, float log_scale = 1.0f, bool* epilogue_done = nullptr,
                    bool fma = false);
int dev_sub_scale(visfd_hip_ctx* ctx, float* a_inout, const float* b, i64 n, float scale, bool do_scale);

int gauss_dev(visfd_hip_ctx* ctx, const float* src, float* dst, const float* mask, i64 nx, i64 ny, i64 nz,
              const float sigma[3], const int hw[3], bool normalize, SlabInfo slab, float* A_out,
              const float* minuend = nullptr, float log_scale = 1.0f, bool* epilogue_done = nullptr, bool fma = false);
struct LogPlan {
  float sa[3], sb[3], scale;
  int hw[3];
};
LogPlan plan_log(const float sigma[3], float delta, float ratio);
int log_dev(visfd_hip_ctx* ctx, const float* src, float* dst, float* tmp, const float* mask, i64 nx, i64 ny,
            i64 nz, const float sigma[3], float delta, float ratio, float* A, float* B);
int dev_sub_square(visfd_hip_ctx* ctx, const float* a, const float* b, float* out, i64 n);
int dev_scale_clamp_sqrt(visfd_hip_ctx* ctx, float* a_inout, i64 n, float scale);

struct ScanPending {
  const unsigned long long* counters = nullptr;
  const void* survivors = nullptr;
  size_t cap_idx = 0, cap_out = 0;
};
int blob_scan_launch(visfd_hip_ctx* ctx, const BlobJob* owner, int set, hipEvent_t done, const float* lo, const float* mid,
                     const float* hi, const float* mask, i64 nx, i64 ny, i64 nz, float min_thr, float max_thr,
                     ScanPending* pending);
int blob_scan_collect(visfd_hip_ctx* ctx, const ScanPending& pending, hipEvent_t done, hipStream_t aux, i64 nx, i64 ny,
                      int scale_index,
                      float sigma, std::vector<visfd_hip_blob>* minima, std::vector<visfd_hip_blob>* maxima,
                      bool* overflow);
int dev_blob_scan(visfd_hip_ctx* ctx, const float* lo, const float* mid, const float* hi,
                  const float* mask, i64 nx, i64 ny, i64 nz, int scale_index, float sigma,
                  float min_thr, float max_thr, bool want_min, bool want_max,
                  std::vector<visfd_hip_blob>* minima, std::vector<visfd_hip_blob>* maxima);

int dev_hessian(visfd_hip_ctx* ctx, const float* smoothed, const float* mask, i64 nx, i64 ny, i64 nz,
                float sigma, float* grad_planar, float* hess_planar);
int dev_hessian_saliency(visfd_hip_ctx* ctx, const float* hess_planar, const float* mask, i64 nvox,
                         int order, float* saliency, float* dir_planar);
int dev_ridge_saliency_fused(visfd_hip_ctx* ctx, const float* smoothed, const float* mask, i64 nx,
                             i64 ny, i64 nz, float sigma, int order, float* saliency,
                             float* dir_planar);
int dev_ridge_score(visfd_hip_ctx* ctx, const float* smoothed, const float* mask, i64 nx, i64 ny, i64 nz,
                    float sigma, int order, float* saliency, const float* peak_img = nullptr, const float* peak_bg = nullptr);
int dev_ridge_directions(visfd_hip_ctx* ctx, const float* smoothed, const float* saliency, i64 nx, i64 ny, i64 nz,
                         float sigma, int order, float* dir_planar);
int dev_diagonalize(visfd_hip_ctx* ctx, const float* m6_planar, float* out6_planar, i64 n, int order);
int dev_tensor_saliency(visfd_hip_ctx* ctx, const float* tensor_planar, const float* mask, i64 nvox,
                        int order, float* saliency, const float* peak_img = nullptr, const float* peak_bg = nullptr);

int dev_select_histogram(visfd_hip_ctx* ctx, const float* sal, const float* mask, i64 nvox, int pass,
                         uint32_t prefix, uint64_t* hist_host, uint64_t* n_unmasked_host);
int dev_select_histogram_todev(visfd_hip_ctx* ctx, const float* sal, const float* mask, i64 nvox, int pass, uint32_t prefix,
                               uint64_t* hist_dev);
int dev_apply_threshold(visfd_hip_ctx* ctx, float* sal, i64 nvox, float thr);
int dev_threshold_fraction(visfd_hip_ctx* ctx, float* sal, const float* mask, i64 nvox, float fraction,
                           float* thr_out);

int dev_tv_dense_stick(visfd_hip_ctx* ctx, const float* sal, const float* dir_planar,
                       float* tensor_planar, const float* mask_src, const float* mask_dst, i64 nx,
                       i64 ny, i64 nz, i64 z_out0, i64 z_out1, float sigma_tv, int exponent,
                       float cutoff, bool curves);

int dev_tv_weight_sum(visfd_hip_ctx* ctx, const float* sal, float* den, const float* mask_src, const float* mask_dst, i64 nx,
                      i64 ny, i64 nz, float sigma_tv, float cutoff);

constexpr int MORPH_RUN_MAX_R = 10;
struct MorphElem {
  i64 n = 0;
  int lo[3] = {0, 0, 0}, hi[3] = {0, 0, 0};
  bool flat = true;
  bool runs = false;
  int R = 0;
  signed char run_len[(2 * MORPH_RUN_MAX_R + 1) * (2 * MORPH_RUN_MAX_R + 1)];
};

int dev_morph_table(visfd_hip_ctx* ctx, const float* src, float* dst, const float* mask, i64 nx, i64 ny, i64 nz,
                    const MorphElem& el, bool dilate, int epi, bool nan_masked, int* path);
int dev_nan_masked(visfd_hip_ctx* ctx, const float* src, const float* mask, float* out, i64 n);
int morph_put_table(visfd_hip_ctx* ctx, const int* dxyz, const float* b, i64 n, MorphElem* el);
int morph_run(visfd_hip_ctx* ctx, const float* src, float* dst, const float* mask, i64 nx, i64 ny, i64 nz, int op,
              MorphElem el);

struct ExtremaArgs {
  const float* src;
  const float* mask;
  i64 nx, ny, nz;
  int find_minima, find_maxima;
  float minima_threshold, maxima_threshold;
  int connectivity, allow_borders;
  int64_t *min_index, *min_nvoxels, *max_index, *max_nvoxels;
  float *min_score, *max_score;
  int64_t min_cap, max_cap;
  int64_t *n_min, *n_max;
  int32_t* labels;
};
int extrema_check_args(const visfd_hip_ctx* ctx, const ExtremaArgs& a);
int dev_find_extrema(visfd_hip_ctx* ctx, const ExtremaArgs& a);

int dev_bin_array3d(visfd_hip_ctx* ctx, const float* src, const int64_t size_src[3], float* dst,
                    const int64_t size_dst[3], const int* offset);
int dev_unbin_array3d(visfd_hip_ctx* ctx, const float* src, const int64_t size_src[3], float* dst,
                      const int64_t size_dst[3], const int* offset);

int dev_interleaved_to_planar(visfd_hip_ctx* ctx, const float* aos, float* planar, i64 n, int channels);
int dev_planar_to_interleaved(visfd_hip_ctx* ctx, const float* planar, float* aos, i64 n, int channels,
                              const float* mask );

struct Stage {
  visfd_hip_ctx* ctx;
  size_t n;

  int out(Slot s, float** dev, int channels = 1, const float* fill = nullptr) const {
    VH_TRY(ws(ctx, s, channels * n, dev));
    if (fill) VH_HIP(hipMemcpyAsync(*dev, fill, sizeof(float) * channels * n, hipMemcpyHostToDevice, ctx->stream));
    return VISFD_HIP_OK;
  }
  int up(Slot s, const float* host, float** dev, int channels = 1) const {
    *dev = nullptr;
    return host ? out(s, dev, channels, host) : VISFD_HIP_OK;
  }
  int down(float* host, const float* dev, int channels = 1) const {
    VH_HIP(hipMemcpyAsync(host, dev, sizeof(float) * channels * n, hipMemcpyDeviceToHost, ctx->stream));
    VH_HIP(hipStreamSynchronize(ctx->stream));
    return VISFD_HIP_OK;
  }
  int up_planar(Slot s_aos, Slot s_planar, const float* host, int channels, float** planar, float** aos = nullptr) const {
    float* a = nullptr;
    VH_TRY(out(s_aos, &a, channels, host));
    VH_TRY(out(s_planar, planar, channels));
    if (aos) *aos = a;
    return dev_interleaved_to_planar(ctx, a, *planar, (i64)n, channels);
  }
  int down_interleaved(float* host, const float* planar, float* aos, int channels, const float* mask, bool keep) const {
    if (keep) VH_HIP(hipMemcpyAsync(aos, host, sizeof(float) * channels * n, hipMemcpyHostToDevice, ctx->stream));
    VH_TRY(dev_planar_to_interleaved(ctx, planar, aos, (i64)n, channels, mask));
    return down(host, aos, channels);
  }
};

template <typename Run>
int stage_filter(visfd_hip_ctx* ctx, const float* src, float* dst, const float* mask, i64 nx, i64 ny, i64 nz, bool dst_up,
                 Run run) {
  VH_REQUIRE(ctx && src && dst, "null argument");
  VH_HIP(hipSetDevice(ctx->device));
// ... 19 lines not shown
```

visfd_amd/csrc/context.hip:

```cpp
#include <cctype>
#include <cstdlib>

#include "common.hpp"

namespace vh {

static thread_local std::string g_last_error;
void set_error(const std::string& msg) { g_last_error = msg; }
int fail(int code, const std::string& msg) {
  g_last_error = msg;
  return code;
}

int ws_get(visfd_hip_ctx* ctx, Slot s, size_t bytes, void** out) {
  if (bytes == 0) bytes = 16;
  if (ctx->slot_bytes[s] < bytes) {
    if (ctx->slot_ptr[s] && (s == WS_CAND || s == WS_SCANCNT)) VH_TRY(blob_jobs_drain(ctx));
    if (ctx->slot_ptr[s]) {
      VH_HIP(hipStreamSynchronize(ctx->stream));
      VH_HIP(hipFree(ctx->slot_ptr[s]));
      ctx->slot_ptr[s] = nullptr;
      ctx->slot_bytes[s] = 0;
    }
    void* p = nullptr;
    hipError_t e = hipMalloc(&p, bytes);
    if (e != hipSuccess)
      return fail(VISFD_HIP_ENOMEM, "hipMalloc of " + std::to_string(bytes) + " bytes failed: " +
                                        hipGetErrorString(e));
    ctx->slot_ptr[s] = p;
    ctx->slot_bytes[s] = bytes;
  }
  *out = ctx->slot_ptr[s];
  return VISFD_HIP_OK;
}

namespace {

struct OptionDesc { const char* name; int visfd_hip_options::*i; int64_t visfd_hip_options::*l; };
const OptionDesc kOptions[] = {
    {"gauss_3pass", &visfd_hip_options::gauss_3pass, nullptr},   {"gauss_cfg", &visfd_hip_options::gauss_cfg, nullptr},
    {"gauss_wg_per_cu", &visfd_hip_options::gauss_wg_per_cu, nullptr}, {"tv_dense", &visfd_hip_options::tv_dense, nullptr},
    {"tv_zrun", &visfd_hip_options::tv_zrun, nullptr}, {"tv_fma", &visfd_hip_options::tv_fma, nullptr},
    {"gauss_fma", &visfd_hip_options::gauss_fma, nullptr}, {"eig_f32", &visfd_hip_options::eig_f32, nullptr},
    {"tv_no_replay", &visfd_hip_options::tv_no_replay, nullptr}, {"tv_max_wg", &visfd_hip_options::tv_max_wg, nullptr},
    {"tv_poison", &visfd_hip_options::tv_poison, nullptr}, {"tv_no_fold", &visfd_hip_options::tv_no_fold, nullptr}, {"tv_exact_tiled", &visfd_hip_options::tv_exact_tiled, nullptr}, {"tv_reserve_wg", &visfd_hip_options::tv_reserve_wg, nullptr},
    {"blob_test_cap", nullptr, &visfd_hip_options::blob_test_cap}, {"debug", &visfd_hip_options::debug, nullptr},
    {"morph_general", &visfd_hip_options::morph_general, nullptr},
};
bool set_option(visfd_hip_options* o, const char* name, int64_t value) {
  for (const OptionDesc& d : kOptions) {
    if (std::strcmp(d.name, name) != 0) continue;
    if (d.i) o->*(d.i) = (int)value; else o->*(d.l) = value;
    return true;
  }
  return false;
}
bool get_option(const visfd_hip_options* o, const char* name, int64_t* value) {
  for (const OptionDesc& d : kOptions) {
    if (std::strcmp(d.name, name) != 0) continue;
    *value = d.i ? (int64_t)(o->*(d.i)) : o->*(d.l);
    return true;
  }
  return false;
}
void options_from_environment(visfd_hip_options* o) {
  for (const OptionDesc& d : kOptions) {
    std::string env = "VISFD_HIP_";
    for (const char* c = d.name; *c; c++) env += (char)std::toupper((unsigned char)*c);
    if (const char* e = std::getenv(env.c_str())) set_option(o, d.name, (int64_t)std::atoll(e));
  }
}

void forget_slot_caches(visfd_hip_ctx* ctx) {
  ctx->tv_table_dev = nullptr;
  ctx->tv_table_h = -1;
  ctx->morph_tab.clear();
}

}
}

using namespace vh;

extern "C" {

int visfd_hip_abi_version(void) { return 10; }
const char* visfd_hip_last_error(void) { return g_last_error.c_str(); }

int visfd_hip_create(int device, void* stream, visfd_hip_ctx** out) {
  VH_REQUIRE(out, "null output pointer");
  int count = 0;
  hipError_t e = hipGetDeviceCount(&count);
  if (e != hipSuccess || count <= 0)
    return fail(VISFD_HIP_EDEVICE, "no HIP device available (libvisfd_hip has no CPU fallback)");
  VH_REQUIRE(device >= 0 && device < count, "bad device ordinal");
  VH_HIP(hipSetDevice(device));
  hipDeviceProp_t prop;
  VH_HIP(hipGetDeviceProperties(&prop, device));
  visfd_hip_ctx* ctx = new visfd_hip_ctx();
  ctx->device = device;
  ctx->num_cus = prop.multiProcessorCount > 0 ? prop.multiProcessorCount : 256;
  options_from_environment(&ctx->opt);
  if (stream) {
    ctx->stream = (hipStream_t)stream;
    ctx->own_stream = false;
  } else {
    e = hipStreamCreateWithFlags(&ctx->stream, hipStreamNonBlocking);
    if (e != hipSuccess) {
      delete ctx;
      return fail(VISFD_HIP_EDEVICE, std::string("hipStreamCreate: ") + hipGetErrorString(e));
    }
    ctx->own_stream = true;
  }
  *out = ctx;
  return VISFD_HIP_OK;
}

int visfd_hip_set_option(visfd_hip_ctx* ctx, const char* name, int64_t value) {
  VH_REQUIRE(ctx && name, "null argument");
  if (!set_option(&ctx->opt, name, value)) return fail(VISFD_HIP_EINVAL, std::string("unknown option: ") + name);
  return VISFD_HIP_OK;
}

int visfd_hip_get_option(visfd_hip_ctx* ctx, const char* name, int64_t* value) {
  VH_REQUIRE(ctx && name && value, "null argument");
  if (!get_option(&ctx->opt, name, value)) return fail(VISFD_HIP_EINVAL, std::string("unknown option: ") + name);
  return VISFD_HIP_OK;
}

int visfd_hip_trim(visfd_hip_ctx* ctx) {
// ... 55 lines not shown
```

visfd_amd/csrc/ridge.hip:

```cpp
#include "common.hpp"
#include "eigen3.hpp"

namespace vh {

namespace {

constexpr int BLOCK = 256;

struct Stencil {
  const float* S;
  i64 c;
  i64 sx, sy, sz;
  __device__ __forceinline__ float at(int dx, int dy, int dz) const {
    return S[c + dx * sx + dy * sy + dz * sz];
  }
};

__device__ __forceinline__ void hessian_at(const Stencil& f, float s2, float h6[6]) {
  const float f0 = f.at(0, 0, 0);
  const float two_f0 = 2 * f0;
  const float hxx = (f.at(1, 0, 0) + f.at(-1, 0, 0)) - two_f0;
  const float hyy = (f.at(0, 1, 0) + f.at(0, -1, 0)) - two_f0;
  const float hzz = (f.at(0, 0, 1) + f.at(0, 0, -1)) - two_f0;
  const float hxy = 0.25f * (((f.at(1, 1, 0) + f.at(-1, -1, 0)) - f.at(1, -1, 0)) - f.at(-1, 1, 0));
  const float hyz = 0.25f * (((f.at(0, 1, 1) + f.at(0, -1, -1)) - f.at(0, 1, -1)) - f.at(0, -1, 1));
  const float hzx = 0.25f * (((f.at(1, 0, 1) + f.at(-1, 0, -1)) - f.at(-1, 0, 1)) - f.at(1, 0, -1));
  h6[0] = hxx * s2; h6[1] = hyy * s2; h6[2] = hzz * s2;
  h6[3] = hxy * s2; h6[4] = hyz * s2; h6[5] = hzx * s2;
}

__device__ __forceinline__ bool voxel_of_block(int nx, int ny, int& ix, int& iy, int& iz) {
  const int xblocks = (nx + BLOCK - 1) / BLOCK;
  unsigned b = blockIdx.x;
  const int bx = b % xblocks;
  b /= xblocks;
  iy = b % ny;
  iz = b / ny;
  ix = bx * BLOCK + threadIdx.x;
  return ix < nx;
}

__device__ __forceinline__ Stencil clamped_stencil(const float* S, int ix, int iy, int iz, int nx, int ny,
                                                   int nz) {
  const int x = min(max(ix, 1), nx - 2), y = min(max(iy, 1), ny - 2), z = min(max(iz, 1), nz - 2);
  Stencil f;
  f.S = S;
  f.sx = 1; f.sy = nx; f.sz = (i64)nx * ny;
  f.c = (i64)z * f.sz + (i64)y * nx + x;
  return f;
}

template <bool F32>
__device__ __forceinline__ void saliency_dir(const float h6[6], int order, float& sal, float dir[3]) {
  float d6[6];
  eig::diagonalize_flat<F32>(h6, order, d6);
  const double l1 = d6[0], l2 = d6[1];
  double N = l1 * l1 - l2 * l2;
  N *= N;
  sal = (float)N;
  eig::shoemake_row0(d6 + 3, dir);
}

__global__ void __launch_bounds__(BLOCK)
hessian_kernel(const float* __restrict__ S, const float* __restrict__ mask, int nx, int ny, int nz,
               float sigma, float* __restrict__ grad, float* __restrict__ hess) {
  int ix, iy, iz;
  if (!voxel_of_block(nx, ny, ix, iy, iz)) return;
  const i64 nvox = (i64)nx * ny * nz;
  const i64 v = ((i64)iz * ny + iy) * nx + ix;
  if (mask && mask[v] == 0.0f) return;
  const Stencil f = clamped_stencil(S, ix, iy, iz, nx, ny, nz);
  if (grad) {
    const float g0 = 0.5f * (f.at(1, 0, 0) - f.at(-1, 0, 0));
    const float g1 = 0.5f * (f.at(0, 1, 0) - f.at(0, -1, 0));
    const float g2 = 0.5f * (f.at(0, 0, 1) - f.at(0, 0, -1));
    grad[v] = g0 * sigma;
    grad[nvox + v] = g1 * sigma;
    grad[2 * nvox + v] = g2 * sigma;
  }
  if (hess) {
    float h6[6];
    hessian_at(f, sigma * sigma, h6);
#pragma unroll
    for (int c = 0; c < 6; c++) hess[c * nvox + v] = h6[c];
  }
}

template <bool F32>
__global__ void __launch_bounds__(BLOCK)
hessian_saliency_kernel(const float* __restrict__ hess, const float* __restrict__ mask, i64 nvox,
                        int order, float* __restrict__ sal, float* __restrict__ dir) {
  const i64 v = (i64)blockIdx.x * BLOCK + threadIdx.x;
  if (v >= nvox) return;
  if (mask && mask[v] == 0.0f) { sal[v] = 0.0f; return; }
  float h6[6];
#pragma unroll
  for (int c = 0; c < 6; c++) h6[c] = hess[c * nvox + v];
  float s, d[3];
  saliency_dir<F32>(h6, order, s, d);
  sal[v] = s;
  dir[v] = d[0];
  dir[nvox + v] = d[1];
  dir[2 * nvox + v] = d[2];
}

template <bool F32>
__global__ void __launch_bounds__(BLOCK)
ridge_fused_kernel(const float* __restrict__ S, const float* __restrict__ mask, int nx, int ny, int nz,
                   float sigma, int order, float* __restrict__ sal, float* __restrict__ dir) {
  int ix, iy, iz;
  if (!voxel_of_block(nx, ny, ix, iy, iz)) return;
  const i64 nvox = (i64)nx * ny * nz;
  const i64 v = ((i64)iz * ny + iy) * nx + ix;
  if (mask && mask[v] == 0.0f) { sal[v] = 0.0f; return; }
  const Stencil f = clamped_stencil(S, ix, iy, iz, nx, ny, nz);
  float h6[6];
  hessian_at(f, sigma * sigma, h6);
  float s, d[3];
  saliency_dir<F32>(h6, order, s, d);
  sal[v] = s;
  dir[v] = d[0];
  dir[nvox + v] = d[1];
  dir[2 * nvox + v] = d[2];
}

template <bool F32>
__global__ void __launch_bounds__(BLOCK)
ridge_score_kernel(const float* __restrict__ S, const float* __restrict__ mask, int nx, int ny, int nz,
                   float sigma, int order, float* __restrict__ sal,
                   const float* __restrict__ peak_img, const float* __restrict__ peak_bg) {
  int ix, iy, iz;
  if (!voxel_of_block(nx, ny, ix, iy, iz)) return;
  const i64 v = ((i64)iz * ny + iy) * nx + ix;
  if (mask && mask[v] == 0.0f) { sal[v] = 0.0f; return; }
  const Stencil f = clamped_stencil(S, ix, iy, iz, nx, ny, nz);
  float h6[6];
  hessian_at(f, sigma * sigma, h6);
  double lam[3];
  eig::D3 E[3];
  eig::eig_sym3<F32>(h6, order, lam, E, false);
  const double l1 = (float)lam[0], l2 = (float)lam[1];
  double N = l1 * l1 - l2 * l2;
  N *= N;
  float score = (float)N;
  if (peak_img) score *= peak_img[v] - peak_bg[v];
  __builtin_nontemporal_store(score, &sal[v]);
}

constexpr int DIR_PER = 16;
constexpr int DIR_CHUNK = DIR_PER * BLOCK;
template <bool F32>
__global__ void __launch_bounds__(BLOCK)
ridge_directions_kernel(const float* __restrict__ S, const float* __restrict__ sal, int nx, int ny, int nz,
                        float sigma, int order, float* __restrict__ dir) {
  __shared__ unsigned short list[DIR_CHUNK];
  __shared__ int wave_tot[BLOCK / 64];
  const i64 nvox = (i64)nx * ny * nz;
  const i64 base = (i64)blockIdx.x * DIR_CHUNK;
  const int tid = threadIdx.x, lane = tid & 63, wave = tid >> 6;
  unsigned keep = 0u;
  int cnt = 0;
#pragma unroll
  for (int k = 0; k < DIR_PER; k++) {
    const i64 v = base + k * BLOCK + tid;
    const bool kp = v < nvox && sal[v] != 0.0f;
    keep |= (kp ? 1u : 0u) << k;
    cnt += kp ? 1 : 0;
  }
  int incl = cnt;
#pragma unroll
  for (int d = 1; d < 64; d <<= 1) {
    const int o = __shfl_up(incl, d);
    if (lane >= d) incl += o;
  }
  if (lane == 63) wave_tot[wave] = incl;
  __syncthreads();
  int off = incl - cnt, total = 0;
#pragma unroll
  for (int w = 0; w < BLOCK / 64; w++) {
    const int t = wave_tot[w];
    off += (w < wave) ? t : 0;
    total += t;
  }
#pragma unroll
  for (int k = 0; k < DIR_PER; k++)
    if ((keep >> k) & 1u) list[off++] = (unsigned short)(k * BLOCK + tid);
  __syncthreads();
  const i64 plane = (i64)nx * ny;
  for (int i = tid; i < total; i += BLOCK) {
    const i64 v = base + list[i];
    const int iz = (int)(v / plane);
    const i64 r = v - (i64)iz * plane;
    const int iy = (int)(r / nx), ix = (int)(r - (i64)iy * nx);
    const Stencil f = clamped_stencil(S, ix, iy, iz, nx, ny, nz);
    float h6[6];
    hessian_at(f, sigma * sigma, h6);
    float s, d[3];
    saliency_dir<F32>(h6, order, s, d);
    dir[v] = d[0];
    dir[nvox + v] = d[1];
    dir[2 * nvox + v] = d[2];
  }
}

template <bool F32>
__global__ void __launch_bounds__(BLOCK)
diagonalize_kernel(const float* __restrict__ m, float* __restrict__ out, i64 n, int order) {
  const i64 v = (i64)blockIdx.x * BLOCK + threadIdx.x;
  if (v >= n) return;
  float h6[6], d6[6];
#pragma unroll
  for (int c = 0; c < 6; c++) h6[c] = m[c * n + v];
  eig::diagonalize_flat<F32>(h6, order, d6);
#pragma unroll
  for (int c = 0; c < 6; c++) out[c * n + v] = d6[c];
}

template <bool F32>
__global__ void __launch_bounds__(BLOCK)
tensor_saliency_kernel(const float* __restrict__ ten, const float* __restrict__ mask, i64 nvox, int order,
                       float* __restrict__ sal,
                       const float* __restrict__ peak_img, const float* __restrict__ peak_bg) {
  const i64 v = (i64)blockIdx.x * BLOCK + threadIdx.x;
  if (v >= nvox) return;
  if (mask && mask[v] == 0.0f) return;
  float t6[6];
#pragma unroll
  for (int c = 0; c < 6; c++) t6[c] = ten[c * nvox + v];
  double lam[3];
  eig::D3 E[3];
  eig::eig_sym3<F32>(t6, order, lam, E, false);
  const double l1 = (float)lam[0], l2 = (float)lam[1];
  float score = (float)(l1 - l2);
  if (peak_img) score *= peak_img[v] - peak_bg[v];
  __builtin_nontemporal_store(score, &sal[v]);
}

__global__ void __launch_bounds__(BLOCK)
aos_to_planar_kernel(const float* __restrict__ aos, float* __restrict__ planar, i64 n, int ch) {
  const i64 i = (i64)blockIdx.x * BLOCK + threadIdx.x;
  if (i >= n * ch) return;
  const i64 v = i / ch;
  const int c = (int)(i - v * ch);
  planar[c * n + v] = aos[i];
}

__global__ void __launch_bounds__(BLOCK)
planar_to_aos_kernel(const float* __restrict__ planar, float* __restrict__ aos, i64 n, int ch,
                     const float* __restrict__ mask) {
  const i64 i = (i64)blockIdx.x * BLOCK + threadIdx.x;
  if (i >= n * ch) return;
  const i64 v = i / ch;
  const int c = (int)(i - v * ch);
  if (mask && mask[v] == 0.0f) return;
  aos[i] = planar[c * n + v];
}

#define VH_EIG_LAUNCH(kernel, grid, ...)                                                          \
  do {                                                                                            \
    if (ctx->opt.eig_f32) kernel<true><<<grid, dim3(BLOCK), 0, ctx->stream>>>(__VA_ARGS__);       \
    else kernel<false><<<grid, dim3(BLOCK), 0, ctx->stream>>>(__VA_ARGS__);                       \
  } while (0)

int voxel_grid(i64 nx, i64 ny, i64 nz, unsigned* g) {
  if (nx >= (1LL << 31) || ny >= (1LL << 31) || nz >= (1LL << 31))
    return fail(VISFD_HIP_EINVAL, "dimension too large");
  const i64 nb = ((nx + BLOCK - 1) / BLOCK) * ny * nz;
  if (nb > 0x7fffffffLL) return fail(VISFD_HIP_EINVAL, "volume too large for one launch");
  *g = (unsigned)nb;
  return VISFD_HIP_OK;
}

int linear_grid(i64 n, unsigned* g) {
  const i64 nb = (n + BLOCK - 1) / BLOCK;
  if (nb > 0x7fffffffLL) return fail(VISFD_HIP_EINVAL, "array too large for one launch");
  *g = (unsigned)(nb < 1 ? 1 : nb);
  return VISFD_HIP_OK;
}

}

int dev_hessian(visfd_hip_ctx* ctx, const float* S, const float* mask, i64 nx, i64 ny, i64 nz,
                float sigma, float* grad, float* hess) {
  if (nx < 3 || ny < 3 || nz < 3)
    return fail(VISFD_HIP_EINVAL, "CalcHessian requires an image at least 3 voxels wide in x,y,z");
  unsigned g;
  VH_TRY(voxel_grid(nx, ny, nz, &g));
  hessian_kernel<<<dim3(g), dim3(BLOCK), 0, ctx->stream>>>(S, mask, (int)nx, (int)ny, (int)nz, sigma,
                                                          grad, hess);
  VH_HIP(hipGetLastError());
  return VISFD_HIP_OK;
}

int dev_hessian_saliency(visfd_hip_ctx* ctx, const float* hess, const float* mask, i64 nvox, int order,
                         float* sal, float* dir) {
  unsigned g;
  VH_TRY(linear_grid(nvox, &g));
  VH_EIG_LAUNCH(hessian_saliency_kernel, dim3(g), hess, mask, nvox, order, sal, dir);
  VH_HIP(hipGetLastError());
  return VISFD_HIP_OK;
}

int dev_ridge_saliency_fused(visfd_hip_ctx* ctx, const float* S, const float* mask, i64 nx, i64 ny,
                             i64 nz, float sigma, int order, float* sal, float* dir) {
  if (nx < 3 || ny < 3 || nz < 3)
    return fail(VISFD_HIP_EINVAL, "ridge detection requires an image at least 3 voxels wide in x,y,z");
  unsigned g;
  VH_TRY(voxel_grid(nx, ny, nz, &g));
  VH_EIG_LAUNCH(ridge_fused_kernel, dim3(g), S, mask, (int)nx, (int)ny, (int)nz, sigma, order, sal, dir);
  VH_HIP(hipGetLastError());
  return VISFD_HIP_OK;
}

int dev_ridge_score(visfd_hip_ctx* ctx, const float* S, const float* mask, i64 nx, i64 ny, i64 nz, float sigma,
                    int order, float* sal, const float* peak_img, const float* peak_bg) {
  if (nx < 3 || ny < 3 || nz < 3)
    return fail(VISFD_HIP_EINVAL, "ridge detection requires an image at least 3 voxels wide in x,y,z");
  unsigned g;
  VH_TRY(voxel_grid(nx, ny, nz, &g));
  VH_EIG_LAUNCH(ridge_score_kernel, dim3(g), S, mask, (int)nx, (int)ny, (int)nz, sigma, order, sal, peak_img, peak_bg);
  VH_HIP(hipGetLastError());
  return VISFD_HIP_OK;
}

int dev_ridge_directions(visfd_hip_ctx* ctx, const float* S, const float* sal, i64 nx, i64 ny, i64 nz, float sigma,
                         int order, float* dir) {
  if (nx < 3 || ny < 3 || nz < 3)
    return fail(VISFD_HIP_EINVAL, "ridge detection requires an image at least 3 voxels wide in x,y,z");
  if (nx >= (1LL << 31) || ny >= (1LL << 31) || nz >= (1LL << 31)) return fail(VISFD_HIP_EINVAL, "dimension too large");
  const i64 nb = (nx * ny * nz + DIR_CHUNK - 1) / DIR_CHUNK;
  if (nb > 0x7fffffffLL) return fail(VISFD_HIP_EINVAL, "volume too large for one launch");
  VH_EIG_LAUNCH(ridge_directions_kernel, dim3((unsigned)nb), S, sal, (int)nx, (int)ny, (int)nz, sigma, order, dir);
  VH_HIP(hipGetLastError());
  return VISFD_HIP_OK;
}

int dev_diagonalize(visfd_hip_ctx* ctx, const float* m, float* out, i64 n, int order) {
  unsigned g;
  VH_TRY(linear_grid(n, &g));
  VH_EIG_LAUNCH(diagonalize_kernel, dim3(g), m, out, n, order);
  VH_HIP(hipGetLastError());
  return VISFD_HIP_OK;
}

int dev_tensor_saliency(visfd_hip_ctx* ctx, const float* ten, const float* mask, i64 nvox, int order,
                        float* sal, const float* peak_img, const float* peak_bg) {
  unsigned g;
  VH_TRY(linear_grid(nvox, &g));
  VH_EIG_LAUNCH(tensor_saliency_kernel, dim3(g), ten, mask, nvox, order, sal, peak_img, peak_bg);
  VH_HIP(hipGetLastError());
  return VISFD_HIP_OK;
}

int dev_interleaved_to_planar(visfd_hip_ctx* ctx, const float* aos, float* planar, i64 n, int ch) {
  unsigned g;
  VH_TRY(linear_grid(n * ch, &g));
  aos_to_planar_kernel<<<dim3(g), dim3(BLOCK), 0, ctx->stream>>>(aos, planar, n, ch);
  VH_HIP(hipGetLastError());
  return VISFD_HIP_OK;
}

int dev_planar_to_interleaved(visfd_hip_ctx* ctx, const float* planar, float* aos, i64 n, int ch,
                              const float* mask) {
  unsigned g;
  VH_TRY(linear_grid(n * ch, &g));
  planar_to_aos_kernel<<<dim3(g), dim3(BLOCK), 0, ctx->stream>>>(planar, aos, n, ch, mask);
  VH_HIP(hipGetLastError());
  return VISFD_HIP_OK;
}

}
```

visfd_amd/csrc/select.hip:

```cpp
#include <cmath>
#include <vector>

#include "common.hpp"

namespace vh {

namespace {

constexpr int BLOCK = 256;
constexpr int NBINS = 2048;

__device__ __forceinline__ uint32_t order_key(float f) {
  const uint32_t u = __float_as_uint(f);
  return (u & 0x80000000u) ? ~u : (u | 0x80000000u);
}
inline float key_to_float(uint32_t k) {
  const uint32_t u = (k & 0x80000000u) ? (k & 0x7fffffffu) : ~k;
  float f;
  std::memcpy(&f, &u, 4);
  return f;
}

__global__ void __launch_bounds__(BLOCK)
histogram_kernel(const float* __restrict__ sal, const float* __restrict__ mask, i64 n, int round,
                 uint32_t prefix, unsigned long long* __restrict__ hist) {
  __shared__ unsigned int lh[NBINS];
  for (int i = threadIdx.x; i < NBINS; i += BLOCK) lh[i] = 0;
  __syncthreads();
  const int shift = (round == 0) ? 21 : (round == 1) ? 10 : 0;
  const uint32_t dmask = (round == 2) ? 0x3ffu : 0x7ffu;
  const int pshift = (round == 0) ? 32 : (round == 1) ? 21 : 10;
  auto count = [&](float v) {
    const uint32_t k = order_key(v);
    if (round > 0 && (k >> pshift) != prefix) return;
    atomicAdd(&lh[(k >> shift) & dmask], 1u);
  };
  const i64 step = (i64)gridDim.x * BLOCK;
  const i64 n4 = (!mask && (reinterpret_cast<uintptr_t>(sal) & 15u) == 0) ? (n >> 2) : 0;
  const float4* sal4 = reinterpret_cast<const float4*>(sal);
  i64 j = (i64)blockIdx.x * BLOCK + threadIdx.x;
  for (; j + step < n4; j += 2 * step) {
    const float4 a = sal4[j], b = sal4[j + step];
    count(a.x); count(a.y); count(a.z); count(a.w);
    count(b.x); count(b.y); count(b.z); count(b.w);
  }
  if (j < n4) {
    const float4 a = sal4[j];
    count(a.x); count(a.y); count(a.z); count(a.w);
  }
  for (i64 i = 4 * n4 + (i64)blockIdx.x * BLOCK + threadIdx.x; i < n; i += step) {
    if (mask && mask[i] == 0.0f) continue;
    count(sal[i]);
  }
  __syncthreads();
  for (int i = threadIdx.x; i < NBINS; i += BLOCK) {
    const unsigned int c = lh[i];
    if (c) atomicAdd(&hist[i], (unsigned long long)c);
  }
}

__global__ void __launch_bounds__(BLOCK)
apply_threshold_kernel(float* __restrict__ sal, i64 n, float thr) {
  i64 i = (i64)blockIdx.x * BLOCK + threadIdx.x;
  const i64 step = (i64)gridDim.x * BLOCK;
  for (; i < n; i += step) {
    const float s = sal[i];
    if (s < thr) sal[i] = 0.0f;
  }
}

}

int dev_select_histogram(visfd_hip_ctx* ctx, const float* sal, const float* mask, i64 nvox, int pass,
                         uint32_t prefix, uint64_t* hist_host, uint64_t* n_unmasked_host) {
  unsigned long long* hist = nullptr;
  VH_TRY(ws(ctx, WS_HIST, (size_t)NBINS, &hist));
  hipStream_t st = ctx->stream;
  VH_HIP(hipMemsetAsync(hist, 0, sizeof(unsigned long long) * NBINS, st));
  const unsigned g = grid_for(nvox, BLOCK, (i64)ctx->num_cus * 32);
  histogram_kernel<<<dim3(g), dim3(BLOCK), 0, st>>>(sal, mask, nvox, pass, prefix, hist);
  VH_HIP(hipGetLastError());
  VH_HIP(hipMemcpyAsync(hist_host, hist, sizeof(uint64_t) * NBINS, hipMemcpyDeviceToHost, st));
  VH_HIP(hipStreamSynchronize(st));
  if (n_unmasked_host) {
    uint64_t tot = 0;
    for (int b = 0; b < NBINS; b++) tot += hist_host[b];
    *n_unmasked_host = tot;
  }
  return VISFD_HIP_OK;
}

int dev_select_histogram_todev(visfd_hip_ctx* ctx, const float* sal, const float* mask, i64 nvox, int pass, uint32_t prefix,
                               uint64_t* hist_dev) {
  hipStream_t st = ctx->stream;
  VH_HIP(hipMemsetAsync(hist_dev, 0, sizeof(unsigned long long) * NBINS, st));
  const unsigned g = grid_for(nvox, BLOCK, (i64)ctx->num_cus * 32);
  histogram_kernel<<<dim3(g), dim3(BLOCK), 0, st>>>(sal, mask, nvox, pass, prefix, reinterpret_cast<unsigned long long*>(hist_dev));
  VH_HIP(hipGetLastError());
  return VISFD_HIP_OK;
}

int dev_apply_threshold(visfd_hip_ctx* ctx, float* sal, i64 nvox, float thr) {
  const unsigned g = grid_for(nvox, BLOCK, (i64)ctx->num_cus * 32);
  apply_threshold_kernel<<<dim3(g), dim3(BLOCK), 0, ctx->stream>>>(sal, nvox, thr);
  VH_HIP(hipGetLastError());
  return VISFD_HIP_OK;
}

static int pick_bin_descending(const std::vector<uint64_t>& h, uint64_t* k) {
  uint64_t seen = 0;
  for (int b = NBINS - 1; b >= 0; b--) {
    if (seen + h[b] > *k) { *k -= seen; return b; }
    seen += h[b];
  }
  return -1;
}

int select_pick_digit(const uint64_t* hist, uint64_t* k) {
  return pick_bin_descending(std::vector<uint64_t>(hist, hist + NBINS), k);
}
float select_key_to_float(uint32_t key) { return key_to_float(key); }

int dev_threshold_fraction(visfd_hip_ctx* ctx, float* sal, const float* mask, i64 nvox, float fraction,
                           float* thr_out) {
  std::vector<uint64_t> h(NBINS);
  uint64_t n_unmasked = 0;
  VH_TRY(dev_select_histogram(ctx, sal, mask, nvox, 0, 0, h.data(), &n_unmasked));
  const float prod = (float)n_unmasked * fraction;
  uint64_t k = (uint64_t)std::floor(prod);
  if (n_unmasked == 0 || k >= n_unmasked)
    return fail(VISFD_HIP_EINVAL, "threshold fraction selects no voxel (the reference would read past its array)");
  const int d0 = pick_bin_descending(h, &k);
  if (d0 < 0) return fail(VISFD_HIP_EDEVICE, "radix select: inconsistent histogram");
  VH_TRY(dev_select_histogram(ctx, sal, mask, nvox, 1, (uint32_t)d0, h.data(), nullptr));
  const int d1 = pick_bin_descending(h, &k);
  if (d1 < 0) return fail(VISFD_HIP_EDEVICE, "radix select: inconsistent histogram");
  VH_TRY(dev_select_histogram(ctx, sal, mask, nvox, 2, ((uint32_t)d0 << 11) | (uint32_t)d1, h.data(), nullptr));
  const int d2 = pick_bin_descending(h, &k);
  if (d2 < 0) return fail(VISFD_HIP_EDEVICE, "radix select: inconsistent histogram");
  const float thr = key_to_float(((uint32_t)d0 << 21) | ((uint32_t)d1 << 10) | (uint32_t)d2);
  if (thr_out) *thr_out = thr;
  return dev_apply_threshold(ctx, sal, nvox, thr);
}

}
```

visfd_amd/csrc/tv.hip:

```cpp
#include <vector>

#include "common.hpp"

namespace vh {

namespace {

constexpr int BLOCK = 256;

struct TvParams {
  int nx, ny, nz;
  int z_out0, z_out1;
  int h;
  int exponent;
  int curves;
  int weights_only;
};

__device__ __forceinline__ float decay_of(float ang, int exponent) {
  if (exponent == 2) return ang;
  if (exponent == 4) return ang * ang;
  return (float)pow((double)ang, 0.5 * (double)exponent);
}

__device__ __forceinline__ void add_vote(float T[6], float sal, float fv, float r0, float r1, float r2,
                                         float n0, float n1, float n2, int exponent, int curves) {
  const float u = (r0 * n0 + r1 * n1) + r2 * n2;
  const float ux2 = u * 2.0f;
  const float u2 = u * u;
  const float c2 = 1.0f - u2;
  const float ang = curves ? u2 : c2;
  const float dec = decay_of(ang, exponent);
  float m0, m1, m2;
  if (curves) {
    m0 = n0 - ux2 * r0; m1 = n1 - ux2 * r1; m2 = n2 - ux2 * r2;
  } else {
    m0 = ux2 * r0 - n0; m1 = ux2 * r1 - n1; m2 = ux2 * r2 - n2;
  }
  const float base = (sal * fv) * dec;
  const float b0 = base * m0, b1 = base * m1, b2 = base * m2;
  T[0] = T[0] + b0 * m0;
  T[3] = T[3] + b0 * m1;
  T[5] = T[5] + b0 * m2;
  T[1] = T[1] + b1 * m1;
  T[4] = T[4] + b1 * m2;
  T[2] = T[2] + b2 * m2;
}

__global__ void __launch_bounds__(BLOCK)
tv_dense_kernel(const float* __restrict__ sal, const float* __restrict__ dir,
                float* __restrict__ ten, const float* __restrict__ mask_src,
                const float* __restrict__ mask_dst, const float4* __restrict__ table ,
                TvParams p) {
  const int xblocks = (p.nx + BLOCK - 1) / BLOCK;
  unsigned b = blockIdx.x;
  const int bx = b % xblocks;
  b /= xblocks;
  const int iy = b % p.ny;
  const int iz = p.z_out0 + (int)(b / p.ny);
  const int ix = bx * BLOCK + (int)threadIdx.x;
  if (ix >= p.nx) return;
  const i64 plane = (i64)p.nx * p.ny;
  const i64 nvox = plane * p.nz;
  const i64 c = (i64)iz * plane + (i64)iy * p.nx + ix;
  if (mask_dst && mask_dst[c] == 0.0f) return;
  float T[6] = {0.0f, 0.0f, 0.0f, 0.0f, 0.0f, 0.0f};
  const int h = p.h, n = 2 * h + 1;
  for (int jz = -h; jz <= h; jz++) {
    const int sz = iz - jz;
    if (sz < 0 || sz >= p.nz) continue;
    for (int jy = -h; jy <= h; jy++) {
      const int sy = iy - jy;
      if (sy < 0 || sy >= p.ny) continue;
      const i64 row = (i64)sz * plane + (i64)sy * p.nx;
      const float4* trow = table + ((i64)(jz + h) * n + (jy + h)) * n + h;
      for (int jx = -h; jx <= h; jx++) {
        const float4 t = trow[jx];
        if (t.x == 0.0f) continue;
        const int sx = ix - jx;
        if (sx < 0 || sx >= p.nx) continue;
        const i64 s = row + sx;
        float fv = t.x;
        if (mask_src) {
          const float mv = mask_src[s];
          if (mv == 0.0f) continue;
          fv = fv * mv;
        }
        const float sv = sal[s];
        if (sv == 0.0f) continue;
        if (fv == 0.0f) continue;
        if (p.weights_only) { T[0] = T[0] + fv; continue; }
        add_vote(T, sv, fv, t.y, t.z, t.w, dir[s], dir[nvox + s], dir[2 * nvox + s], p.exponent,
                 p.curves);
      }
    }
  }
  if (p.weights_only) { ten[c] = T[0]; return; }
#pragma unroll
  for (int k = 0; k < 6; k++) ten[k * nvox + c] = T[k];
}

}

int dev_tv_tiled(visfd_hip_ctx* ctx, const float* sal, const float* dir, float* ten,
                 const float* mask_src, const float* mask_dst, i64 nx, i64 ny, i64 nz, i64 z_out0,
                 i64 z_out1, int h, const float4* dtab, int exponent, bool curves, bool weights_only, bool* handled);

int dev_tv_box(visfd_hip_ctx* ctx, const float* sal, const float* dir, float* ten, const float* mask_src,
               const float* mask_dst, i64 nx, i64 ny, i64 nz, i64 z_out0, i64 z_out1, int h, const float4* dtab_box,
               int exponent, bool* handled, bool exact);


static int tv_table_device(visfd_hip_ctx* ctx, float sigma_tv, float cutoff, int h, const float4** out) {
  const size_t n = 2 * (size_t)h + 1, m = n * n * n;
  if (ctx->tv_table_dev && ctx->tv_table_h == h && ctx->tv_table_key[0] == sigma_tv && ctx->tv_table_key[1] == cutoff) {
    *out = reinterpret_cast<const float4*>(ctx->tv_table_dev);
    return VISFD_HIP_OK;
  }
  VH_HIP(hipStreamSynchronize(ctx->stream));
  std::vector<float> w(m), rh(3 * m);
  host_tv_tables(sigma_tv, h, w.data(), rh.data());
  const size_t sp = (size_t)tv_padded_row(h), m2 = n * n * sp;
  const size_t spb = (size_t)tv_box_row(h), nslb = (size_t)tv_box_slice(h), m3 = (n + 1) * nslb;
  std::vector<float4> tab(m + m2 + 2 * m3, make_float4(0.0f, 0.0f, 0.0f, 0.0f));
  const float rt2 = 1.41421356237309504880f;
  for (size_t k = 0; k < m; k++) {
    tab[k] = make_float4(w[k], rh[3 * k], rh[3 * k + 1], rh[3 * k + 2]);
    tab[m + (k / n) * sp + (k % n)] = tab[k];
    const size_t kb = (k / (n * n)) * nslb + 4 + ((k / n) % n + 3) * spb + (k % n);
    tab[m + m2 + kb] = make_float4(w[k], rt2 * rh[3 * k], rt2 * rh[3 * k + 1], rt2 * rh[3 * k + 2]);
    tab[m + m2 + m3 + kb] = tab[k];
  }
  float4* dtab = nullptr;
  ctx->tv_table_dev = nullptr;
  VH_TRY(ws(ctx, WS_TVTAB, m + m2 + 2 * m3, &dtab));
  VH_HIP(hipMemcpyAsync(dtab, tab.data(), sizeof(float4) * (m + m2 + 2 * m3), hipMemcpyHostToDevice, ctx->stream));
  VH_HIP(hipStreamSynchronize(ctx->stream));
  ctx->tv_table_dev = reinterpret_cast<float*>(dtab);
  ctx->tv_table_h = h;
  ctx->tv_table_key[0] = sigma_tv;
  ctx->tv_table_key[1] = cutoff;
  *out = dtab;
  return VISFD_HIP_OK;
}

int dev_tv_dense_stick(visfd_hip_ctx* ctx, const float* sal, const float* dir, float* ten,
                       const float* mask_src, const float* mask_dst, i64 nx, i64 ny, i64 nz,
                       i64 z_out0, i64 z_out1, float sigma_tv, int exponent, float cutoff, bool curves) {
  VH_TRY(check_dims(nx, ny, nz));
  VH_TRY(check_dims32(nx, ny, nz));
  VH_REQUIRE(z_out0 >= 0 && z_out1 <= nz && z_out0 <= z_out1, "bad receiver plane range");
  if (z_out0 == z_out1) return VISFD_HIP_OK;
  const int h = host_tv_halfwidth(sigma_tv, cutoff);
  VH_REQUIRE(h >= 0 && h <= 255, "tensor-voting window halfwidth out of range");
  const float4* dtab = nullptr;
  VH_TRY(tv_table_device(ctx, sigma_tv, cutoff, h, &dtab));

  const size_t m_packed = (size_t)(2 * h + 1) * (2 * h + 1) * (2 * h + 1);
  const size_t m_padded = (size_t)(2 * h + 1) * (2 * h + 1) * (size_t)tv_padded_row(h);
  bool handled = false;
  if (!ctx->opt.tv_dense && ctx->opt.tv_fma && !curves)
    VH_TRY(dev_tv_box(ctx, sal, dir, ten, mask_src, mask_dst, nx, ny, nz, z_out0, z_out1, h, dtab + m_packed + m_padded, exponent,
                      &handled, false));
  if (handled) return VISFD_HIP_OK;
  if (!ctx->opt.tv_dense && !ctx->opt.tv_exact_tiled && !curves)
    VH_TRY(dev_tv_box(ctx, sal, dir, ten, mask_src, mask_dst, nx, ny, nz, z_out0, z_out1, h,
                      dtab + m_packed + m_padded + (size_t)(2 * h + 2) * (size_t)tv_box_slice(h), exponent, &handled, true));
  if (handled) return VISFD_HIP_OK;
  if (!ctx->opt.tv_dense)
    VH_TRY(dev_tv_tiled(ctx, sal, dir, ten, mask_src, mask_dst, nx, ny, nz, z_out0, z_out1, h, dtab + m_packed, exponent, curves,
                        false, &handled));
  if (handled) return VISFD_HIP_OK;

  hipStream_t st = ctx->stream;
  TvParams p;
  p.nx = (int)nx; p.ny = (int)ny; p.nz = (int)nz;
  p.z_out0 = (int)z_out0; p.z_out1 = (int)z_out1;
  p.h = h; p.exponent = exponent; p.curves = curves ? 1 : 0; p.weights_only = 0;
  const i64 nb = ((nx + BLOCK - 1) / BLOCK) * ny * (z_out1 - z_out0);
  if (nb > 0x7fffffffLL) return fail(VISFD_HIP_EINVAL, "volume too large for one launch");
  tv_dense_kernel<<<dim3((unsigned)nb), dim3(BLOCK), 0, st>>>(sal, dir, ten, mask_src, mask_dst, dtab, p);
  VH_HIP(hipGetLastError());
  return VISFD_HIP_OK;
}

int dev_tv_weight_sum(visfd_hip_ctx* ctx, const float* sal, float* den, const float* mask_src, const float* mask_dst, i64 nx,
                      i64 ny, i64 nz, float sigma_tv, float cutoff) {
  VH_TRY(check_dims(nx, ny, nz));
  VH_TRY(check_dims32(nx, ny, nz));
  const int h = host_tv_halfwidth(sigma_tv, cutoff);
  VH_REQUIRE(h >= 0 && h <= 255, "tensor-voting window halfwidth out of range");
  const float4* dtab = nullptr;
  VH_TRY(tv_table_device(ctx, sigma_tv, cutoff, h, &dtab));
  bool handled = false;
  if (!ctx->opt.tv_dense)
    VH_TRY(dev_tv_tiled(ctx, sal, nullptr, den, mask_src, mask_dst, nx, ny, nz, 0, nz, h,
                        dtab + (size_t)(2 * h + 1) * (2 * h + 1) * (2 * h + 1), 4, false, true, &handled));
  if (handled) return VISFD_HIP_OK;
  TvParams p;
  p.nx = (int)nx; p.ny = (int)ny; p.nz = (int)nz;
  p.z_out0 = 0; p.z_out1 = (int)nz;
  p.h = h; p.exponent = 4; p.curves = 0; p.weights_only = 1;
  const i64 nb = ((nx + BLOCK - 1) / BLOCK) * ny * nz;
  if (nb > 0x7fffffffLL) return fail(VISFD_HIP_EINVAL, "volume too large for one launch");
  tv_dense_kernel<<<dim3((unsigned)nb), dim3(BLOCK), 0, ctx->stream>>>(sal, nullptr, den, mask_src, mask_dst, dtab, p);
  VH_HIP(hipGetLastError());
  return VISFD_HIP_OK;
}

}
```

visfd_amd/csrc/tv_box.hip:

```cpp
#include <algorithm>
#include <type_traits>
#include <vector>

#include "common.hpp"

namespace vh {

namespace {

constexpr int NT = 512;
constexpr int NW = NT / 64;
constexpr int TX = 16, TY = 4 * NW;
constexpr int NH = TX / 8;
constexpr int NLIST = 2;
constexpr int NSUB = 2;
constexpr int LSLOTS = NT;
constexpr int HCAP = 36;
constexpr int YPAD = 3;

typedef float f4v __attribute__((ext_vector_type(4)));
typedef unsigned u4v __attribute__((ext_vector_type(4)));
typedef unsigned u2v __attribute__((ext_vector_type(2)));

__device__ __forceinline__ unsigned lds_addr(const void* p) {
  return (unsigned)(uintptr_t)(const __attribute__((address_space(3))) void*)p;
}
template <typename T>
__device__ __forceinline__ const __attribute__((address_space(3))) T* lds_ptr(unsigned a) {
  return (const __attribute__((address_space(3))) T*)(uintptr_t)a;
}

#ifdef VH_TV_STAMPS
__device__ unsigned long long g_box_stamps[8];
#define VH_STAMP(i) do { const unsigned long long t_ = __builtin_amdgcn_s_memtime(); st_acc[i] += (unsigned)(t_ - st_last); st_last = t_; } while (0)
#else
#define VH_STAMP(i) do {} while (0)
#endif
#ifdef VH_TV_COUNT
__device__ unsigned long long g_box_counts[8];
#endif

struct BoxParams {
  int nx, ny, nz;
  int z_out0, z_out1;
  int h;
  int rw, rh;
  int tiles_x, tiles_y;
  int zrun;
  int zl0, nzl;
  int sp;
  int nsl;
};

__device__ __forceinline__ void fmacc(float& t, float a, float b) {
  asm("v_fmac_f32 %0, %1, %2" : "+v"(t) : "v"(a), "v"(b));
}

template <int MODE, bool ZNEG, bool FOLD>
__device__ __forceinline__ void vote_fma(float (&T)[6], const f4v& snd , const f4v& tw ) {
  const float Rz = ZNEG ? -tw.w : tw.w;
  const float t = __builtin_fmaf(Rz, snd.w, __builtin_fmaf(tw.z, snd.z, tw.y * snd.y));
  const float q = __builtin_fmaf(-t, t, FOLD ? snd.x : 2.0f);
  const float m0 = __builtin_fmaf(t, tw.y, -snd.y);
  const float m1 = __builtin_fmaf(t, tw.z, -snd.z);
  const float m2 = __builtin_fmaf(t, Rz, -snd.w);
  const float sw = FOLD ? tw.x : snd.x * tw.x;
  const float bse = (MODE == 0) ? (sw * q) * q : sw * q;
  const float b0 = bse * m0, b1 = bse * m1, b2 = bse * m2;
  fmacc(T[0], b0, m0);
  fmacc(T[3], b0, m1);
  fmacc(T[5], b0, m2);
  fmacc(T[1], b1, m1);
  fmacc(T[4], b1, m2);
  fmacc(T[2], b2, m2);
}

__device__ __forceinline__ f4v lds_f4(unsigned a) { return *(const volatile __attribute__((address_space(3))) f4v*)(uintptr_t)a; }
__device__ __forceinline__ void lds_store_u2(unsigned a, unsigned x, unsigned y) {
  u2v v = {x, y};
  *(__attribute__((address_space(3))) u2v*)(uintptr_t)a = v;
}
__device__ __forceinline__ uint2 lds_u2(unsigned a) {
  const u2v v = *(const volatile __attribute__((address_space(3))) u2v*)(uintptr_t)a;
  return make_uint2(v.x, v.y);
}

__device__ __forceinline__ u4v lds_u4(unsigned a) { return *(const volatile __attribute__((address_space(3))) u4v*)(uintptr_t)a; }
// ... 625 lines not shown
          __syncthreads();
          VH_STAMP(2);
          int i0[NLIST], i1[NLIST];
#pragma unroll
          for (int k = 0; k < NLIST; k++) {
            i0[k] = i1[k] = 0;
            if (len[k] > 0) {
              const unsigned rg = __builtin_amdgcn_readfirstlane(l_rng[(plane_slot(lsz[k]) * NPAIR + k) * NW + wave]);
              const int off = c[k] + done - pre[k];
              i0[k] = min(max((int)(rg & 0xffffu) - off, 0), len[k]);
              i1[k] = min(max((int)(rg >> 16) - off, 0), len[k]);
            }
          }
          if (i1[0] > i0[0] || i1[1] > i0[1]) {
            const float cy = (float)(4 * wave + h) + 1.5f;
            const unsigned ln = fresh_lane();
            const int fq = (int)((ln & 31u) >> 2);
            const int fcol = (int)(ln & 3u) + 4 * (int)(ln >> 5), frow = fq >> 1, fpl = (0x96 >> fq) & 1;
            const unsigned r16_0 = lds_addr(slices) + 16u * (unsigned)(4 + (4 * wave + frow + 2 * h + YPAD) * SP + fcol + 2 * h);
            const unsigned null_e16 = 16u * (unsigned)((4 * wave + h) * SP + h);
            const unsigned r16 = r16_0 + (unsigned)(16 * nsl) * (unsigned)((t + fpl) & 1);
            if (i1[0] > i0[0]) test_vote(std::integral_constant<int, 0>{}, c[0], i0[0], i1[0], r16, cy, rr, null_e16);
            if (i1[1] > i0[1]) test_vote(std::integral_constant<int, 1>{}, c[1], i0[1], i1[1], r16, cy, rr, null_e16);
          }
          VH_STAMP(3);
          __syncthreads();
          VH_STAMP(4);
          done += NT;
        } while (done < total);
      }

#pragma unroll
      for (int q = 0; q < NPAIR; q++)
#pragma unroll
        for (int pp = 0; pp < NH; pp++) {
          const int rx = x0 + 8 * pp + 4 * sub + lcol, ry = y0 + 4 * wave + lrow, rzl = rz + 2 * q + lpl;
          const bool in = rx < p.nx && ry < p.ny && rzl < z_run1;
          const i64 rc = (i64)rzl * plane + (i64)ry * p.nx + rx;
          const bool live = in && !(mask_dst && mask_dst[in ? rc : 0] == 0.0f);
          if (live) {
#pragma unroll
            for (int k = 0; k < 6; k++) __builtin_nontemporal_store(TT[q][pp][k], &ten[k * nvox + rc]);
          }
        }
    }
  }
#ifdef VH_TV_STAMPS
  VH_STAMP(5);
  if (lane == 0) {
#pragma unroll
    for (int i = 0; i < 6; i++) atomicAdd(&g_box_stamps[i], st_acc[i]);
  }
#endif
#ifdef VH_TV_COUNT
  if (lane == 0) {
    atomicAdd(&g_box_counts[0], (unsigned long long)cnt_tested);
    atomicAdd(&g_box_counts[1], (unsigned long long)cnt_hits);
    atomicAdd(&g_box_counts[2], (unsigned long long)cnt_steps);
  }
#endif
}

struct ListGeo {
  int nx, ny, nz;
  int zl0, nzl;
  int ntx, h;
};
constexpr int LNT = 256;
constexpr int LWORDS_MAX = 512;

__device__ __forceinline__ unsigned popc_range(const unsigned* w, int lo, int hi) {
  unsigned c = 0;
  for (int i = lo >> 5; i <= (hi - 1) >> 5 && lo < hi; i++) {
    unsigned m = w[i];
    if (i == (lo >> 5)) m &= ~0u << (lo & 31);
    if (i == ((hi - 1) >> 5) && (hi & 31)) m &= ~0u >> (32 - (hi & 31));
    c += (unsigned)__builtin_popcount(m);
  }
  return c;
}

template <bool WRITE, int MODE>
__global__ void __launch_bounds__(LNT)
tvl_row_kernel(const float* __restrict__ sal, const float* __restrict__ dir, const float* __restrict__ mask_src, ListGeo g,
               unsigned* __restrict__ rows, float4* __restrict__ ent, unsigned* __restrict__ pos,
               unsigned* __restrict__ neg_flag ,
               int fold ) {
  constexpr int LB = 8;
  __shared__ unsigned bits_all[LNT / 64][LWORDS_MAX + 4];
  __shared__ unsigned base_all[WRITE ? LNT / 64 : 1][WRITE ? LWORDS_MAX * 2 + 4 : 1];
  __shared__ unsigned cum_all[WRITE ? LNT / 64 : 1][WRITE ? LWORDS_MAX / 2 + 4 : 1];
  const int wave = __builtin_amdgcn_readfirstlane((int)threadIdx.x >> 6), lane = threadIdx.x & 63;
  const i64 r = (i64)blockIdx.x * (LNT / 64) + wave;
  if (r >= (i64)g.nzl * g.ny) return;
  unsigned* const bits = bits_all[wave];
  const int y = (int)(r % g.ny), zl = (int)(r / g.ny);
  const i64 plane = (i64)g.nx * g.ny, nvox = plane * g.nz;
  const i64 row = (i64)(g.zl0 + zl) * plane + (i64)y * g.nx;
  const int nchunks = (g.nx + 63) >> 6;
  unsigned* const rrow = rows + ((size_t)zl * (size_t)(g.ny + 1) + (size_t)y) * (size_t)g.ntx;
  if (WRITE) {
    unsigned* const base = base_all[WRITE ? wave : 0];
    for (int tx = lane; tx < g.ntx; tx += 64) base[tx] = rrow[g.ntx + tx];
  }
  unsigned any = 0, total = 0;
  unsigned* const cum = cum_all[WRITE ? wave : 0];
  for (int c0 = 0; c0 < nchunks; c0 += LB) {
    float v[LB], m[LB];
#pragma unroll
    for (int k = 0; k < LB; k++) {
      const int x = 64 * (c0 + k) + lane;
      v[k] = x < g.nx ? sal[row + x] : 0.0f;
      m[k] = (mask_src && x < g.nx) ? mask_src[row + x] : 1.0f;
    }
#pragma unroll
    for (int k = 0; k < LB; k++) {
      if (c0 + k >= nchunks) break;
      const bool f = v[k] != 0.0f && m[k] != 0.0f;
      const unsigned long long bal = __builtin_amdgcn_ballot_w64(f);
      if (lane == 0) {
        bits[2 * (c0 + k)] = (unsigned)bal;
        bits[2 * (c0 + k) + 1] = (unsigned)(bal >> 32);
        if (WRITE) cum[c0 + k] = total;
      }
      any |= (unsigned)bal | (unsigned)(bal >> 32);
      if (WRITE) total += (unsigned)__builtin_popcountll(bal);
      if (!WRITE && f) {
        const float s = mask_src ? v[k] * m[k] : v[k];
        if (!(s > 0.0f)) atomicOr(neg_flag, 1u);
        if (!(__builtin_fabsf(s) <= 3.402823466e38f)) atomicOr(neg_flag, 2u);
        if (mask_src && m[k] != 1.0f) atomicOr(neg_flag, 4u);
      }
    }
  }
  __builtin_amdgcn_wave_barrier();
  asm volatile("s_waitcnt vmcnt(0) lgkmcnt(0)" ::: "memory");
  if (!WRITE) {
    for (int tx = lane; tx < g.ntx; tx += 64)
      rrow[tx] = any ? popc_range(bits, max(TX * tx - g.h, 0), min(TX * tx + TX + g.h, g.nx)) : 0u;
    return;
  }
  if (!any) return;
  const unsigned* const base = base_all[WRITE ? wave : 0];
  for (unsigned j0 = 0; j0 < total; j0 += 64) {
    const unsigned j = j0 + lane;
    if (j >= total) break;
    int lo = 0, hi = nchunks;
    while (hi - lo > 1) {
      const int mid = (lo + hi) >> 1;
      if (cum[mid] <= j) lo = mid; else hi = mid;
    }
    unsigned k = j - cum[lo];
    unsigned w = bits[2 * lo];
    int x = 64 * lo;
    {
      const unsigned t = (unsigned)__builtin_popcount(w);
      if (k >= t) { k -= t; x += 32; w = bits[2 * lo + 1]; }
    }
#pragma unroll
    for (int sft = 16; sft >= 1; sft >>= 1) {
      const unsigned t = (unsigned)__builtin_popcount(w & ((1u << sft) - 1u));
      if (k >= t) { k -= t; x += sft; w >>= sft; }
    }
    float4 q = make_float4(sal[row + x] * (MODE == 0 ? 0.25f : (MODE == 2 ? 0.5f : 1.0f)), dir[row + x], dir[nvox + row + x], dir[2 * nvox + row + x]);
    if (mask_src) q.x = q.x * mask_src[row + x];
    if (fold) {
      const double r2 = sqrt((double)q.x);
      const float a = (float)(MODE == 0 ? cbrt(r2) : sqrt(r2));
      q = make_float4(2.0f * a * a, a * q.y, a * q.z, a * q.w);
    }
    const int t0 = max((x - TX - g.h) / TX + ((x - TX - g.h) >= 0 ? 1 : 0), 0);
    const int t1 = min((x + g.h) / TX, g.ntx - 1);
    for (int tx = t0; tx <= t1; tx++) {
      const int lo_x = TX * tx - g.h, hi_x = min(TX * tx + TX + g.h, g.nx);
      if (x < lo_x || x >= hi_x) continue;
      const unsigned idx = base[tx] + popc_range(bits, x + 1, hi_x);
      ent[idx] = q;
      pos[idx] = (unsigned)(x - lo_x) | ((unsigned)y << 8);
    }
  }
}

__global__ void __launch_bounds__(LNT)
tvl_scan_kernel(ListGeo g, unsigned* __restrict__ rows, unsigned long long* __restrict__ total) {
  const int i = blockIdx.x * LNT + threadIdx.x;
  if (i >= g.nzl * g.ntx) return;
  const int zl = i / g.ntx, tx = i - zl * g.ntx;
  unsigned* const col = rows + (size_t)zl * (size_t)(g.ny + 1) * (size_t)g.ntx + tx;
  unsigned sum = 0;
  for (int y = 0; y < g.ny; y++) sum += col[(size_t)y * g.ntx];
  const unsigned base = (unsigned)atomicAdd(total, (unsigned long long)sum);
  unsigned run = base;
  unsigned prev = col[(size_t)(g.ny - 1) * g.ntx];
  col[(size_t)g.ny * g.ntx] = run;
  for (int y = g.ny - 1; y >= 0; y--) {
    const unsigned c = prev;
    if (y > 0) prev = col[(size_t)(y - 1) * g.ntx];
    run += c;
    col[(size_t)y * g.ntx] = run;
  }
}

__global__ void __launch_bounds__(256) lds_poison_kernel(unsigned* sink) {
  extern __shared__ unsigned pz[];
  for (int i = threadIdx.x; i < 160 * 256; i += 256) pz[i] = 0xffffffffu;
  __syncthreads();
  if (pz[(threadIdx.x * 37) % (160 * 256)] == 1u) sink[0] = 1u;
}

}

int dev_tv_box(visfd_hip_ctx* ctx, const float* sal, const float* dir, float* ten, const float* mask_src,
               const float* mask_dst, i64 nx, i64 ny, i64 nz, i64 z_out0, i64 z_out1, int h, const float4* dtab_box,
               int exponent, bool* handled, bool exact) {
  *handled = false;
  if (exponent != 2 && exponent != 4) return VISFD_HIP_OK;
  if (h < 1 || h > 40) return VISFD_HIP_OK;
  if (nx * ny >= (1LL << 29) || nx > 32 * LWORDS_MAX || ny >= (1 << 24)) return VISFD_HIP_OK;
  hipStream_t st = ctx->stream;
  BoxParams p;
  p.nx = (int)nx; p.ny = (int)ny; p.nz = (int)nz;
  p.z_out0 = (int)z_out0; p.z_out1 = (int)z_out1;
  p.h = h;
  p.rw = TX + 2 * h;
  p.rh = TY + 2 * h;
  if (p.rw > 255 || p.rh > 255) return VISFD_HIP_OK;
  p.sp = tv_box_row(h);
  p.nsl = tv_box_slice(h);
  const size_t slice_bytes = sizeof(float4) * (size_t)p.nsl;
  p.tiles_x = (int)((nx + TX - 1) / TX);
  p.tiles_y = (int)((ny + TY - 1) / TY);
  p.zrun = 8;
  if (ctx->opt.tv_zrun >= 1 && ctx->opt.tv_zrun <= 4096) p.zrun = ctx->opt.tv_zrun;
  if ((i64)p.zrun > z_out1 - z_out0) p.zrun = (int)(z_out1 - z_out0);
  if (p.zrun < 1) p.zrun = 1;
  const i64 nruns = (z_out1 - z_out0 + p.zrun - 1) / p.zrun;
  const i64 nblk = (i64)p.tiles_x * p.tiles_y * nruns;
  if (nblk > 0x7fffffffLL) return fail(VISFD_HIP_EINVAL, "volume too large for one launch");
  if (nblk <= 0) { *handled = true; return VISFD_HIP_OK; }
  const size_t lds = 2 * slice_bytes + sizeof(unsigned) * (size_t)(2 * h + 4) * NW * (exact ? NPAIR : 1);
  const size_t lds_static = sizeof(float4) * (LSLOTS + 1) + sizeof(uint2) * LSLOTS + sizeof(uint2) * NW * NSUB * 2 * HCAP + 1536;
  static_assert(2 * HCAP == HX, "the two kernels' hit lists take the same LDS");
  if (lds + lds_static > 150 * 1024) return VISFD_HIP_OK;

  ListGeo g;
  g.nx = p.nx; g.ny = p.ny; g.nz = p.nz; g.h = h; g.ntx = p.tiles_x;
  g.zl0 = (int)std::max<i64>(z_out0 - h, 0);
  g.nzl = (int)(std::min<i64>(z_out1 + h, nz) - g.zl0);
  p.zl0 = g.zl0; p.nzl = g.nzl;
  const size_t nrows = (size_t)g.nzl * (size_t)(ny + 1) * (size_t)g.ntx;
  if ((i64)g.nzl * ny > 0x7fffffffLL) return VISFD_HIP_OK;
  unsigned* rows = nullptr;
  unsigned* counter = nullptr;
  VH_TRY(ws(ctx, WS_COUNTER, 16, &counter));
  if (ws(ctx, WS_TVLIST, nrows, &rows) != VISFD_HIP_OK) { set_error(""); (void)hipGetLastError(); return VISFD_HIP_OK; }
  unsigned long long* total_dev = reinterpret_cast<unsigned long long*>(counter + 4);
  VH_HIP(hipMemsetAsync(counter, 0, 16 * sizeof(unsigned), st));
  const unsigned row_blocks = (unsigned)(((i64)g.nzl * ny + LNT / 64 - 1) / (LNT / 64));
#define VH_TVL_ROWS(WR, ENT, POS)                                                                                         \
  do {                                                                                                                    \
    if (exact) tvl_row_kernel<WR, 1><<<dim3(row_blocks), dim3(LNT), 0, st>>>(sal, dir, mask_src, g, rows, ENT, POS, counter + 6, 0);             \
    else if (exponent == 4) tvl_row_kernel<WR, 0><<<dim3(row_blocks), dim3(LNT), 0, st>>>(sal, dir, mask_src, g, rows, ENT, POS, counter + 6, fold); \
    else tvl_row_kernel<WR, 2><<<dim3(row_blocks), dim3(LNT), 0, st>>>(sal, dir, mask_src, g, rows, ENT, POS, counter + 6, fold);             \
  } while (0)
  int fold = 0;
  VH_TVL_ROWS(false, nullptr, nullptr);
  tvl_scan_kernel<<<dim3((unsigned)(((size_t)g.nzl * g.ntx + LNT - 1) / LNT)), dim3(LNT), 0, st>>>(g, rows, total_dev);
  VH_HIP(hipGetLastError());
  unsigned long long tot2[2] = {0, 0};
  VH_HIP(hipMemcpyAsync(tot2, total_dev, sizeof(tot2), hipMemcpyDeviceToHost, st));
  VH_HIP(hipStreamSynchronize(st));
  const unsigned long long total = tot2[0];
  fold = ((unsigned)tot2[1] & 1u) ? 0 : 1;
  if (ctx->opt.tv_no_fold) fold = 0;
  if (exact && ((unsigned)tot2[1] & 2u)) return VISFD_HIP_OK;
  if (exact && ((unsigned)tot2[1] & 4u)) return VISFD_HIP_OK;
  if (total >= (1ull << 32) - 2048) return VISFD_HIP_OK;
  unsigned char* lists = nullptr;
  if (ws(ctx, WS_TVSCRATCH, (size_t)(total + 16) * 20, &lists) != VISFD_HIP_OK) { set_error(""); (void)hipGetLastError(); return VISFD_HIP_OK; }
  float4* const lst_ent = reinterpret_cast<float4*>(lists);
  unsigned* const lst_pos = reinterpret_cast<unsigned*>(lists + (size_t)(total + 16) * 16);
  if (ctx->opt.tv_poison) VH_HIP(hipMemsetAsync(lists, 0xff, (size_t)(total + 16) * 20, st));
  VH_TVL_ROWS(true, lst_ent, lst_pos);
#undef VH_TVL_ROWS
  VH_HIP(hipGetLastError());

  size_t wg_per_cu = (160 * 1024) / (lds + lds_static);
  if (wg_per_cu > 3) wg_per_cu = 3;
  if (wg_per_cu < 1) wg_per_cu = 1;
  i64 ngrid = (i64)ctx->num_cus * (i64)wg_per_cu;
  if (ctx->opt.tv_reserve_wg > 0) ngrid = std::max<i64>(ngrid - ctx->opt.tv_reserve_wg, 1);
  if (ctx->opt.tv_max_wg > 0 && ngrid > ctx->opt.tv_max_wg) ngrid = ctx->opt.tv_max_wg;
  if (ngrid > nblk) ngrid = nblk;
  if (ctx->opt.tv_poison) {
    VH_HIP(hipMemsetAsync(ten, 0xff, sizeof(float) * 6 * (size_t)(nx * ny * nz), st));
    VH_HIP(hipFuncSetAttribute(reinterpret_cast<const void*>(&lds_poison_kernel), hipFuncAttributeMaxDynamicSharedMemorySize, 160 * 1024));
    lds_poison_kernel<<<dim3(1024), dim3(256), 160 * 1024, st>>>(counter + 8);
  }
#define VH_BOX_LAUNCH(MD, FD)                                                                                          \
  do {                                                                                                                 \
    VH_HIP(hipFuncSetAttribute(reinterpret_cast<const void*>(&tv_box_kernel<MD, FD>),                                  \
                               hipFuncAttributeMaxDynamicSharedMemorySize, (int)lds));                                 \
    tv_box_kernel<MD, FD><<<dim3((unsigned)ngrid), dim3(NT), lds, st>>>(ten, mask_dst, dtab_box, p, counter, (unsigned)nblk, \
                                                                       lst_ent, lst_pos, rows);                        \
  } while (0)
#define VH_BOXX_LAUNCH(MD)                                                                                             \
  do {                                                                                                                 \
    VH_HIP(hipFuncSetAttribute(reinterpret_cast<const void*>(&tv_boxx_kernel<MD>),                                     \
                               hipFuncAttributeMaxDynamicSharedMemorySize, (int)lds));                                 \
    tv_boxx_kernel<MD><<<dim3((unsigned)ngrid), dim3(NT), lds, st>>>(ten, mask_dst, dtab_box, p, counter, (unsigned)nblk, \
                                                                    lst_ent, lst_pos, rows);                           \
  } while (0)
  if (exact)              { if (exponent == 4) VH_BOXX_LAUNCH(0); else VH_BOXX_LAUNCH(2); }
  else if (exponent == 4) { if (fold) VH_BOX_LAUNCH(0, true); else VH_BOX_LAUNCH(0, false); }
  else                    { if (fold) VH_BOX_LAUNCH(2, true); else VH_BOX_LAUNCH(2, false); }
#undef VH_BOX_LAUNCH
#undef VH_BOXX_LAUNCH
  VH_HIP(hipGetLastError());
#ifdef VH_TV_COUNT
  {
    unsigned long long c4[8], z4[8] = {};
    VH_HIP(hipStreamSynchronize(st));
    VH_HIP(hipMemcpyFromSymbol(c4, HIP_SYMBOL(g_box_counts), sizeof(c4)));
    fprintf(stderr, "[tv_box counts] list entries tested %.4g  hits (sender, sub-patch) %.4g  vote steps %.4g  -> hits per tested entry %.3f, "
            "stream fill %.3f\n", (double)c4[0], (double)c4[1], (double)c4[2], (double)c4[1] / (double)c4[0], (double)c4[1] / (2.0 * (double)c4[2]));
    VH_HIP(hipMemcpyToSymbol(HIP_SYMBOL(g_box_counts), z4, sizeof(z4)));
  }
#endif
#ifdef VH_TV_STAMPS
  {
    unsigned long long st8[8], z8[8] = {};
    VH_HIP(hipStreamSynchronize(st));
    VH_HIP(hipMemcpyFromSymbol(st8, HIP_SYMBOL(g_box_stamps), sizeof(st8)));
    double tot = 0;
    for (int i = 0; i < 6; i++) tot += (double)st8[i];
    fprintf(stderr, "[tv_box stamps] share of wave time: listing+claim %.3f | fill %.3f | barrier before sweep %.3f | test+vote %.3f | "
            "barrier after sweep %.3f | stores+rest %.3f  (total %.3g ticks over %lld waves)\n", st8[0] / tot, st8[1] / tot,
            st8[2] / tot, st8[3] / tot, st8[4] / tot, st8[5] / tot, tot, (long long)ngrid * NW);
    VH_HIP(hipMemcpyToSymbol(HIP_SYMBOL(g_box_stamps), z8, sizeof(z8)));
  }
#endif
  *handled = true;
  return VISFD_HIP_OK;
}

}
```

visfd_amd/pipeline.py:

```python
import math

import numpy as np

from . import api

TRUNCATE_THRESHOLD = 0.03


def cli_blob_sigmas(width_min, width_max, growth):
    wmin, wmax, g = np.float32(width_min), np.float32(width_max), np.float32(growth)
    N = 1 + int(math.ceil(np.float32(np.log(np.float32(wmax / wmin), dtype=np.float32) / np.log(g, dtype=np.float32))))
    g = np.float32(math.pow(float(np.float32(wmax / wmin)), 1.0 / N))
    d = np.empty(N, np.float32)
    d[0] = np.float32(wmin * np.float32(2.0 * math.sqrt(3.0)))
    for n in range(1, N):
        d[n] = np.float32(d[n - 1] * g)
    return api.diameters_to_sigmas(d)


def gauss(ctx, src, dst, sigma, truncate_threshold=TRUNCATE_THRESHOLD, mask=None, normalize=True):
    ratio = api.ratio_from_threshold(truncate_threshold)
    sig = (sigma,) * 3 if np.isscalar(sigma) else tuple(sigma)
    hw = api.gauss_halfwidths(sig, ratio)
    return ctx.gauss_dev(src, dst, sig, hw, mask, normalize)


def blob_detect(ctx, src, sigmas, truncate_threshold=TRUNCATE_THRESHOLD, delta=0.02, mask=None,
                minima_threshold=np.inf, maxima_threshold=-np.inf, use_ratios=False, cap=1 << 22):
    ratio = api.ratio_from_threshold(truncate_threshold)
    return ctx.blob_dog_dev(src, sigmas, mask, None, delta, ratio, minima_threshold, maxima_threshold,
                            use_ratios, cap)


def blob_detect_begin(ctx, src, sigmas, truncate_threshold=TRUNCATE_THRESHOLD, delta=0.02, mask=None,
                      minima_threshold=np.inf, maxima_threshold=-np.inf, use_ratios=False):
    ratio = api.ratio_from_threshold(truncate_threshold)
    return ctx.blob_dog_begin_dev(src, sigmas, mask, None, delta, ratio, minima_threshold, maxima_threshold, use_ratios)


def blob_detect_end(ctx, job, cap=1 << 22):
    return ctx.blob_dog_end(job, cap)


def membrane_detect(ctx, src, sal, dirs, tensor, sigma, tv_sigma_ratio, tv_exponent=4, best_fraction=0.05,
                    truncate_threshold=TRUNCATE_THRESHOLD, tv_truncate_ratio=math.sqrt(2.0), minima=True,
                    mask=None, scratch=None, sigma_background=0.0, background=None):
    order = api.DECREASING_EIVALS if minima else api.INCREASING_EIVALS
    ratio = api.ratio_from_threshold(truncate_threshold)
    smoothed = scratch if scratch is not None else src.new_empty(src.shape)
    bg = None
    if sigma_background > 0:
        bg = background if background is not None else src.new_empty(src.shape)
        ctx.peak_background_dev(src, bg, sigma_background, ratio, mask)
    ctx.ridge_scores_dev(src, sal, smoothed, sigma, ratio, order, mask, bg)
    thr = ctx.threshold_fraction_dev(sal, best_fraction, mask)
    ctx.ridge_directions_dev(smoothed, sal, dirs, sigma, order)
    sigma_tv = float(np.float32(tv_sigma_ratio) * np.float32(sigma))
    ctx.tv_dense_stick_dev(sal, dirs, tensor, sigma_tv, tv_exponent, tv_truncate_ratio, mask, mask)
    ctx.tensor_saliency_dev(tensor, sal, order, mask, src if bg is not None else None, bg)
    return thr
```

Before: 2536.

## Fuse membrane stage: histogram in ridge score, threshold folded into directions and TV

Adds a single native membrane stage entry point that builds the first radix-select histogram inside the ridge-score kernel, finishes the selection on device, and passes the threshold into the ridge-directions and TV sender-list kernels instead of running a separate apply-threshold pass. The aim is to cut full-volume passes over saliency and the Python and host overhead of calling each stage separately. The Python pipeline now routes through this fused call. This adds new kernel parameters and more code paths. Saliency must be writable for the thresholded TV path, and the fallback TV paths still run an explicit threshold pass.

```diff
diff --git a/include/visfd_hip.h b/include/visfd_hip.h
--- a/include/visfd_hip.h
+++ b/include/visfd_hip.h
@@ -252,6 +252,17 @@
 int visfd_hip_select_histogram_todev(visfd_hip_ctx*, const float* saliency, const float* mask, int64_t nvox, int round,
                                      uint32_t prefix, uint64_t* hist_dev );
 int visfd_hip_apply_threshold_dev(visfd_hip_ctx*, float* saliency, int64_t nvox, float threshold);
+int visfd_hip_ridge_scores_hist_dev(visfd_hip_ctx*, const float* src, const float* mask, int64_t nx, int64_t ny, int64_t nz,
+                                    float sigma, float truncate_ratio, int eival_order, const float* background,
+                                    float* saliency, float* smoothed, uint64_t* hist_dev);
+int visfd_hip_select_pick_dev(visfd_hip_ctx*, const uint64_t* hist_dev, int pass, float fraction, uint32_t* prefix_inout,
+                              uint64_t* rank_inout, int* status);
+int visfd_hip_ridge_directions_thr_dev(visfd_hip_ctx*, const float* smoothed, int64_t nx, int64_t ny, int64_t nz,
+                                       float sigma, int eival_order, const float* saliency, float threshold, float* direction);
+int visfd_hip_tv_dense_stick_thr_dev(visfd_hip_ctx*, float* saliency, const float* direction, float* tensor,
+                                     const float* mask_src, const float* mask_dst, int64_t nx, int64_t ny, int64_t nz,
+                                     float sigma_tv, int exponent, float cutoff_ratio, float threshold);
+int visfd_hip_tv_last_senders(visfd_hip_ctx*, int64_t* entries);
 
 int visfd_hip_tv_dense_stick(visfd_hip_ctx*, const float* saliency, const float* direction,
                              float* tensor, const float* mask_src, const float* mask_dst,
@@ -278,6 +289,11 @@
 int visfd_hip_tensor_saliency_bg_dev(visfd_hip_ctx*, const float* tensor, const float* mask, int64_t nvox, int eival_order,
                                      const float* image, const float* background, float* saliency_inout);
 
+int visfd_hip_membrane_stage_dev(visfd_hip_ctx*, const float* src, const float* mask, int64_t nx, int64_t ny, int64_t nz,
+                                 float sigma, float truncate_ratio, int eival_order, float best_fraction, float threshold_abs,
+                                 float sigma_tv, int tv_exponent, float tv_cutoff_ratio, float sigma_background,
+                                 int normalize_background, float* saliency_out, float* tensor_out, float* direction_out,
+                                 float* smoothed, float* background, float* threshold_out);
 int visfd_hip_membrane_detect(visfd_hip_ctx*, const float* src, const float* mask,
                               int64_t nx, int64_t ny, int64_t nz, float sigma, float truncate_ratio,
                               int eival_order, float best_fraction, float threshold_abs, float sigma_tv,
diff --git a/visfd_amd/api.py b/visfd_amd/api.py
--- a/visfd_amd/api.py
+++ b/visfd_amd/api.py
@@ -121,6 +121,16 @@
     "visfd_hip_membrane_detect_bg_dev": (C.c_int, [_vp, _vp, _vp, _i64, _i64, _i64, C.c_float, C.c_float, C.c_int,
                                                    C.c_float, C.c_float, C.c_float, C.c_int, C.c_float, C.c_float, C.c_int,
                                                    _vp, _vp, _vp, _fp]),
+    "visfd_hip_membrane_stage_dev": (C.c_int, [_vp, _vp, _vp, _i64, _i64, _i64, C.c_float, C.c_float, C.c_int,
+                                               C.c_float, C.c_float, C.c_float, C.c_int, C.c_float, C.c_float, C.c_int,
+                                               _vp, _vp, _vp, _vp, _vp, _fp]),
+    "visfd_hip_ridge_scores_hist_dev": (C.c_int, [_vp, _vp, _vp, _i64, _i64, _i64, C.c_float, C.c_float, C.c_int, _vp, _vp, _vp,
+                                                  _vp]),
+    "visfd_hip_select_pick_dev": (C.c_int, [_vp, _vp, C.c_int, C.c_float, C.POINTER(C.c_uint32), C.POINTER(C.c_uint64), _ip]),
+    "visfd_hip_ridge_directions_thr_dev": (C.c_int, [_vp, _vp, _i64, _i64, _i64, C.c_float, C.c_int, _vp, C.c_float, _vp]),
+    "visfd_hip_tv_dense_stick_thr_dev": (C.c_int, [_vp, _vp, _vp, _vp, _vp, _vp, _i64, _i64, _i64, C.c_float, C.c_int,
+                                                   C.c_float, C.c_float]),
+    "visfd_hip_tv_last_senders": (C.c_int, [_vp, C.POINTER(_i64)]),
     "visfd_hip_membrane_detect_slab_bg_dev": (C.c_int, [_vp, _vp, _vp, _vp, _vp, _vp, _vp, _i64, _i64, C.c_float, C.c_float, C.c_int,
                                                         C.c_float, C.c_float, C.c_int, C.c_float, C.c_float, C.c_int, C.c_int, _fp]),
     "visfd_hip_membrane_detect_slab_bg": (C.c_int, [_vp, _vp, _i64, _i64, C.c_float, C.c_float, C.c_int, C.c_float, C.c_float,
@@ -827,6 +837,50 @@
                                                            C.byref(thr)))
         return thr.value
 
+    def membrane_stage_dev(self, src, sal, sigma, ratio, order, best_fraction=0.05, threshold_abs=0.0, sigma_tv=0.0,
+                           tv_exponent=4, tv_cutoff=2.0 ** 0.5, mask=None, dirs=None, tensor=None, smoothed=None,
+                           background=None, sigma_background=0.0, normalize_background=True):
+        nz, ny, nx = src.shape
+        thr = C.c_float()
+        self._chk(self._L.visfd_hip_membrane_stage_dev(self._h, _dev(src), _dev(mask), nx, ny, nz, float(sigma), float(ratio),
+                                                       int(order), float(best_fraction), float(threshold_abs),
+                                                       float(sigma_tv), int(tv_exponent), float(tv_cutoff),
+                                                       float(sigma_background), int(bool(normalize_background)), _dev(sal),
+                                                       _dev(tensor), _dev(dirs), _dev(smoothed), _dev(background),
+                                                       C.byref(thr)))
+        return thr.value
+
+    def ridge_scores_hist_dev(self, src, sal, smoothed, hist, sigma, ratio, order, mask=None, background=None):
+        assert hist.is_cuda and hist.numel() == 2048 and hist.element_size() == 8 and hist.is_contiguous()
+        nz, ny, nx = src.shape
+        self._chk(self._L.visfd_hip_ridge_scores_hist_dev(self._h, _dev(src), _dev(mask), nx, ny, nz, float(sigma),
+                                                          float(ratio), int(order), _dev(background), _dev(sal),
+                                                          _dev(smoothed), hist.data_ptr()))
+
+    def select_pick_dev(self, hist, pass_, fraction=0.0, prefix=0, rank=0):
+        assert hist.is_cuda and hist.numel() == 2048 and hist.element_size() == 8 and hist.is_contiguous()
+        p, k, st = C.c_uint32(int(prefix)), C.c_uint64(int(rank)), C.c_int()
+        self._chk(self._L.visfd_hip_select_pick_dev(self._h, hist.data_ptr(), int(pass_), float(fraction), C.byref(p),
+                                                    C.byref(k), C.byref(st)))
+        return int(p.value), int(k.value), int(st.value)
+
+    def ridge_directions_thr_dev(self, smoothed, sal, dirs, sigma, order, thr):
+        nz, ny, nx = smoothed.shape
+        self._chk(self._L.visfd_hip_ridge_directions_thr_dev(self._h, _dev(smoothed), nx, ny, nz, float(sigma), int(order),
+                                                             _dev(sal), float(thr), _dev(dirs)))
+
+    def tv_dense_stick_thr_dev(self, sal, dirs, tensor, sigma_tv, thr, exponent=4, cutoff=2.0 ** 0.5, mask_src=None,
+                               mask_dst=None):
+        nz, ny, nx = sal.shape
+        self._chk(self._L.visfd_hip_tv_dense_stick_thr_dev(self._h, _dev(sal), _dev(dirs), _dev(tensor), _dev(mask_src),
+                                                           _dev(mask_dst), nx, ny, nz, float(sigma_tv), int(exponent),
+                                                           float(cutoff), float(thr)))
+
+    def tv_last_senders(self):
+        n = C.c_int64()
+        self._chk(self._L.visfd_hip_tv_last_senders(self._h, C.byref(n)))
+        return int(n.value)
+
     def gauss_dev(self, src, dst, sigma, hw, mask=None, normalize=True):
         nz, ny, nx = src.shape
         A = C.c_float()
diff --git a/visfd_amd/build.py b/visfd_amd/build.py
--- a/visfd_amd/build.py
+++ b/visfd_amd/build.py
@@ -15,7 +15,7 @@
               ("ridge.hip", "ridge", [])]
 VARIANTS = TV_VARIANT + [("gauss_fused.hip", "gauss_fused_h%d" % h, ["-DVH_FUSED_H=%d" % h, "-fno-slp-vectorize"])
                          for h in range(1, 9)]
-HEADERS = ["common.hpp", "eigen3.hpp", os.path.join("..", "..", "include", "visfd_hip.h")]
+HEADERS = ["common.hpp", "eigen3.hpp", "select_dev.hpp", os.path.join("..", "..", "include", "visfd_hip.h")]
 
 HIPCC = os.environ.get("HIPCC", "/opt/rocm/bin/hipcc")
 FLAGS = ["--offload-arch=gfx950", "-O3", "-std=c++17", "-fPIC", "-ffp-contract=off", "-fno-fast-math",
diff --git a/visfd_amd/csrc/api.hip b/visfd_amd/csrc/api.hip
--- a/visfd_amd/csrc/api.hip
+++ b/visfd_amd/csrc/api.hip
@@ -3,6 +3,7 @@
 #include <vector>
 
 #include "common.hpp"
+#include "select_dev.hpp"
 
 namespace vh {
 
@@ -347,16 +348,21 @@
   return dev_ridge_saliency_fused(ctx, S, mask, nx, ny, nz, sigma, order, sal, dir);
 }
 
+int visfd_hip_ridge_scores_hist_dev(visfd_hip_ctx* ctx, const float* src, const float* mask, int64_t nx, int64_t ny,
+                                    int64_t nz, float sigma, float ratio, int order, const float* background, float* sal,
+                                    float* smoothed, uint64_t* hist_dev) {
+  VH_REQUIRE(ctx && src && sal && smoothed, "null argument");
+  VH_REQUIRE(smoothed != src && smoothed != sal, "the smoothed volume needs its own buffer");
+  VH_REQUIRE(order == 0 || order == 1, "unsupported eigenvalue order");
+  VH_HIP(hipSetDevice(ctx->device));
+  VH_TRY(check_dims(nx, ny, nz));
+  VH_TRY(gauss_iso_dev(ctx, src, smoothed, mask, nx, ny, nz, sigma, ratio, true, "filter halfwidth"));
+  return dev_ridge_score(ctx, smoothed, mask, nx, ny, nz, sigma, order, sal, background ? src : nullptr, background, hist_dev);
+}
 int visfd_hip_ridge_scores_bg_dev(visfd_hip_ctx* ctx, const float* src, const float* mask, int64_t nx, int64_t ny,
                                   int64_t nz, float sigma, float ratio, int order, const float* background, float* sal,
                                   float* smoothed) {
-  VH_REQUIRE(ctx && src && sal && smoothed, "null argument");
-  VH_REQUIRE(smoothed != src && smoothed != sal, "the smoothed volume needs its own buffer");
-  VH_REQUIRE(order == 0 || order == 1, "unsupported eigenvalue order");
-  VH_HIP(hipSetDevice(ctx->device));
-  VH_TRY(check_dims(nx, ny, nz));
-  VH_TRY(gauss_iso_dev(ctx, src, smoothed, mask, nx, ny, nz, sigma, ratio, true, "filter halfwidth"));
-  return dev_ridge_score(ctx, smoothed, mask, nx, ny, nz, sigma, order, sal, background ? src : nullptr, background);
+  return visfd_hip_ridge_scores_hist_dev(ctx, src, mask, nx, ny, nz, sigma, ratio, order, background, sal, smoothed, nullptr);
 }
 int visfd_hip_ridge_scores_dev(visfd_hip_ctx* ctx, const float* src, const float* mask, int64_t nx, int64_t ny,
                                int64_t nz, float sigma, float ratio, int order, float* sal, float* smoothed) {
@@ -372,13 +378,17 @@
                        "background filter halfwidth");
 }
 
+int visfd_hip_ridge_directions_thr_dev(visfd_hip_ctx* ctx, const float* smoothed, int64_t nx, int64_t ny, int64_t nz,
+                                       float sigma, int order, const float* sal, float thr, float* dir) {
+  VH_REQUIRE(ctx && smoothed && sal && dir, "null argument");
+  VH_REQUIRE(order == 0 || order == 1, "unsupported eigenvalue order");
+  VH_HIP(hipSetDevice(ctx->device));
+  VH_TRY(check_dims(nx, ny, nz));
+  return dev_ridge_directions(ctx, smoothed, sal, nx, ny, nz, sigma, order, dir, thr);
+}
 int visfd_hip_ridge_directions_dev(visfd_hip_ctx* ctx, const float* smoothed, int64_t nx, int64_t ny, int64_t nz,
                                    float sigma, int order, const float* sal, float* dir) {
-  VH_REQUIRE(ctx && smoothed && sal && dir, "null argument");
-  VH_REQUIRE(order == 0 || order == 1, "unsupported eigenvalue order");
-  VH_HIP(hipSetDevice(ctx->device));
-  VH_TRY(check_dims(nx, ny, nz));
-  return dev_ridge_directions(ctx, smoothed, sal, nx, ny, nz, sigma, order, dir);
+  return visfd_hip_ridge_directions_thr_dev(ctx, smoothed, nx, ny, nz, sigma, order, sal, VH_THR_NONE, dir);
 }
 
 int visfd_hip_threshold_fraction_dev(visfd_hip_ctx* ctx, float* sal, const float* mask, int64_t nvox,
@@ -416,6 +426,26 @@
   VH_REQUIRE(pass >= 0 && pass <= 2, "round must be 0, 1 or 2");
   VH_HIP(hipSetDevice(ctx->device));
   return dev_select_histogram_todev(ctx, sal, mask, nvox, pass, prefix, hist_dev);
+}
+
+int visfd_hip_select_pick_dev(visfd_hip_ctx* ctx, const uint64_t* hist_dev, int pass, float fraction, uint32_t* prefix_inout,
+                              uint64_t* k_inout, int* status) {
+  VH_REQUIRE(ctx && hist_dev && prefix_inout && k_inout && status, "null argument");
+  VH_REQUIRE(pass >= 0 && pass <= 2, "round must be 0, 1 or 2");
+  VH_HIP(hipSetDevice(ctx->device));
+  uint64_t* hist = nullptr;
+  SelectState* state = nullptr;
+  VH_TRY(select_workspace(ctx, &hist, &state));
+  VH_REQUIRE(hist_dev != hist, "the histogram needs its own buffer");
+  SelectState s = {(unsigned long long)*k_inout, *prefix_inout, SELECT_OK};
+  VH_HIP(hipMemcpyAsync(state, &s, sizeof(s), hipMemcpyHostToDevice, ctx->stream));
+  VH_TRY(dev_select_pick(ctx, hist_dev, pass, fraction, state));
+  VH_HIP(hipMemcpyAsync(&s, state, sizeof(s), hipMemcpyDeviceToHost, ctx->stream));
+  VH_HIP(hipStreamSynchronize(ctx->stream));
+  *k_inout = s.k;
+  *prefix_inout = s.prefix;
+  *status = (int)s.status;
+  return VISFD_HIP_OK;
 }
 
 int visfd_hip_apply_threshold_dev(visfd_hip_ctx* ctx, float* sal, int64_t nvox, float thr) {
@@ -478,6 +508,19 @@
   VH_HIP(hipSetDevice(ctx->device));
   return dev_tv_dense_stick(ctx, sal, dir, ten, mask_src, mask_dst, nx, ny, nz_local, z_out0, z_out1,
                             sigma_tv, exponent, cutoff, curves != 0);
+}
+
+int visfd_hip_tv_dense_stick_thr_dev(visfd_hip_ctx* ctx, float* sal, const float* dir, float* ten, const float* mask_src,
+                                     const float* mask_dst, int64_t nx, int64_t ny, int64_t nz, float sigma_tv, int exponent,
+                                     float cutoff, float thr) {
+  VH_REQUIRE(ctx && sal && dir && ten, "null argument");
+  VH_HIP(hipSetDevice(ctx->device));
+  return dev_tv_dense_stick(ctx, sal, dir, ten, mask_src, mask_dst, nx, ny, nz, 0, nz, sigma_tv, exponent, cutoff, false, thr, sal);
+}
+int visfd_hip_tv_last_senders(visfd_hip_ctx* ctx, int64_t* n) {
+  VH_REQUIRE(ctx && n, "null argument");
+  *n = ctx->tv_last_senders;
+  return VISFD_HIP_OK;
 }
 
 int visfd_hip_tv_dense_stick_dev(visfd_hip_ctx* ctx, const float* sal, const float* dir, float* ten,
@@ -522,40 +565,53 @@
   return st.down(den, dden);
 }
 
+int visfd_hip_membrane_stage_dev(visfd_hip_ctx* ctx, const float* src, const float* mask, int64_t nx, int64_t ny, int64_t nz,
+                                 float sigma, float ratio, int order, float best_fraction, float threshold_abs, float sigma_tv,
+                                 int exponent, float cutoff, float sigma_background, int normalize_background, float* sal,
+                                 float* ten, float* dir, float* smoothed, float* background, float* thr_out) {
+  VH_REQUIRE(ctx && src && sal, "null argument");
+  VH_REQUIRE(order == 0 || order == 1, "unsupported eigenvalue order");
+  VH_REQUIRE(best_fraction <= 1.0f, "fraction must be <= 1");
+  VH_REQUIRE(!smoothed || (smoothed != src && smoothed != sal), "the smoothed volume needs its own buffer");
+  VH_HIP(hipSetDevice(ctx->device));
+  VH_TRY(check_dims(nx, ny, nz));
+  const i64 n = nx * ny * nz;
+  float* d = dir;
+  if (!d) VH_TRY(ws(ctx, WS_TVAUX, (size_t)(3 * n), &d));
+  if (!smoothed) VH_TRY(ws(ctx, WS_D, (size_t)n, &smoothed));
+  float* bg = nullptr;
+  if (sigma_background > 0.0f) {
+    bg = background;
+    if (!bg) VH_TRY(ws(ctx, WS_C, (size_t)n, &bg));
+    VH_TRY(visfd_hip_peak_background_dev(ctx, src, mask, nx, ny, nz, sigma_background, ratio, normalize_background, bg));
+  }
+  const bool select = best_fraction >= 0.0f;
+  uint64_t* hist = nullptr;
+  if (select) VH_TRY(select_workspace(ctx, &hist, nullptr));
+  VH_TRY(gauss_iso_dev(ctx, src, smoothed, mask, nx, ny, nz, sigma, ratio, true, "filter halfwidth"));
+  VH_TRY(dev_ridge_score(ctx, smoothed, mask, nx, ny, nz, sigma, order, sal, bg ? src : nullptr, bg, hist));
+  float thr = threshold_abs;
+  if (select) VH_TRY(dev_select_finish(ctx, sal, mask, n, best_fraction, &thr));
+  if (thr_out) *thr_out = thr;
+  VH_TRY(dev_ridge_directions(ctx, smoothed, sal, nx, ny, nz, sigma, order, d, thr));
+  if (sigma_tv > 0.0f) {
+    float* t = ten;
+    if (!t) VH_TRY(ws(ctx, WS_B, (size_t)(6 * n), &t));
+    VH_TRY(dev_tv_dense_stick(ctx, sal, d, t, mask, mask, nx, ny, nz, 0, nz, sigma_tv, exponent, cutoff, false, thr, sal));
+    VH_TRY(dev_tensor_saliency(ctx, t, mask, n, order, sal, bg ? src : nullptr, bg));
+  } else {
+    VH_TRY(dev_apply_threshold(ctx, sal, n, thr));
+  }
+  return VISFD_HIP_OK;
+}
 int visfd_hip_membrane_detect_bg_dev(visfd_hip_ctx* ctx, const float* src, const float* mask, int64_t nx,
                                      int64_t ny, int64_t nz, float sigma, float ratio, int order,
                                      float best_fraction, float threshold_abs, float sigma_tv, int exponent,
                                      float cutoff, float sigma_background, int normalize_background, float* sal, float* ten,
                                      float* dir, float* thr_out) {
-  VH_REQUIRE(ctx && src && sal, "null argument");
-  VH_REQUIRE(order == 0 || order == 1, "unsupported eigenvalue order");
-  VH_REQUIRE(best_fraction <= 1.0f, "fraction must be <= 1");
-  VH_HIP(hipSetDevice(ctx->device));
-  VH_TRY(check_dims(nx, ny, nz));
-  const i64 n = nx * ny * nz;
-  float* d = dir;
-  if (!d) VH_TRY(ws(ctx, WS_TVAUX, (size_t)(3 * n), &d));
-  float* smoothed = nullptr;
-  VH_TRY(ws(ctx, WS_D, (size_t)n, &smoothed));
-  float* bg = nullptr;
-  if (sigma_background > 0.0f) {
-    VH_TRY(ws(ctx, WS_C, (size_t)n, &bg));
-    VH_TRY(visfd_hip_peak_background_dev(ctx, src, mask, nx, ny, nz, sigma_background, ratio, normalize_background, bg));
-  }
-  VH_TRY(visfd_hip_ridge_scores_bg_dev(ctx, src, mask, nx, ny, nz, sigma, ratio, order, bg, sal, smoothed));
-  float thr = threshold_abs;
-  if (best_fraction >= 0.0f) VH_TRY(dev_threshold_fraction(ctx, sal, mask, n, best_fraction, &thr));
-  else VH_TRY(dev_apply_threshold(ctx, sal, n, thr));
-  if (thr_out) *thr_out = thr;
-  if (dir) VH_HIP(hipMemsetAsync(dir, 0, sizeof(float) * 3 * (size_t)n, ctx->stream));
-  VH_TRY(dev_ridge_directions(ctx, smoothed, sal, nx, ny, nz, sigma, order, d));
-  if (sigma_tv > 0.0f) {
-    float* t = ten;
-    if (!t) VH_TRY(ws(ctx, WS_B, (size_t)(6 * n), &t));
-    VH_TRY(dev_tv_dense_stick(ctx, sal, d, t, mask, mask, nx, ny, nz, 0, nz, sigma_tv, exponent, cutoff, false));
-    VH_TRY(dev_tensor_saliency(ctx, t, mask, n, order, sal, bg ? src : nullptr, bg));
-  }
-  return VISFD_HIP_OK;
+  return visfd_hip_membrane_stage_dev(ctx, src, mask, nx, ny, nz, sigma, ratio, order, best_fraction, threshold_abs, sigma_tv,
+                                      exponent, cutoff, sigma_background, normalize_background, sal, ten, dir, nullptr, nullptr,
+                                      thr_out);
 }
 int visfd_hip_membrane_detect_dev(visfd_hip_ctx* ctx, const float* src, const float* mask, int64_t nx,
                                   int64_t ny, int64_t nz, float sigma, float ratio, int order,
@@ -579,6 +635,7 @@
   VH_TRY(st.up(WS_H2D_1, mask, &dm));
   VH_TRY(st.out(WS_H2D_2, &dsal));
   VH_TRY(st.out(WS_H2D_3, &pdir, 3));
+  if (dir) VH_HIP(hipMemsetAsync(pdir, 0, sizeof(float) * 3 * st.n, ctx->stream));
   if (ten && sigma_tv > 0.0f) {
     VH_TRY(st.out(WS_H2D_4, &pten, 6));
     VH_HIP(hipMemsetAsync(pten, 0, sizeof(float) * 6 * st.n, ctx->stream));
diff --git a/visfd_amd/csrc/common.hpp b/visfd_amd/csrc/common.hpp
--- a/visfd_amd/csrc/common.hpp
+++ b/visfd_amd/csrc/common.hpp
@@ -81,6 +81,7 @@
   int tv_reserve_wg = 0;
   int tv_max_wg = 0;
   int64_t blob_test_cap = 0;
+  int ridge_no_tile = 0;
   int morph_general = 0;
   int debug = 0;
 };
@@ -98,6 +99,7 @@
   int num_cus = 256;
   hipStream_t aux_stream = nullptr;
   std::vector<int> morph_tab;
+  int64_t tv_last_senders = -1;
   int morph_last_path = -1;
   std::vector<vh::BlobJob*> blob_jobs;
 };
@@ -201,9 +203,10 @@
                              i64 ny, i64 nz, float sigma, int order, float* saliency,
                              float* dir_planar);
 int dev_ridge_score(visfd_hip_ctx* ctx, const float* smoothed, const float* mask, i64 nx, i64 ny, i64 nz,
-                    float sigma, int order, float* saliency, const float* peak_img = nullptr, const float* peak_bg = nullptr);
+                    float sigma, int order, float* saliency, const float* peak_img = nullptr, const float* peak_bg = nullptr,
+                    uint64_t* hist_dev = nullptr);
 int dev_ridge_directions(visfd_hip_ctx* ctx, const float* smoothed, const float* saliency, i64 nx, i64 ny, i64 nz,
-                         float sigma, int order, float* dir_planar);
+                         float sigma, int order, float* dir_planar, float thr = -__builtin_inff());
 int dev_diagonalize(visfd_hip_ctx* ctx, const float* m6_planar, float* out6_planar, i64 n, int order);
 int dev_tensor_saliency(visfd_hip_ctx* ctx, const float* tensor_planar, const float* mask, i64 nvox,
                         int order, float* saliency, const float* peak_img = nullptr, const float* peak_bg = nullptr);
@@ -215,11 +218,15 @@
 int dev_apply_threshold(visfd_hip_ctx* ctx, float* sal, i64 nvox, float thr);
 int dev_threshold_fraction(visfd_hip_ctx* ctx, float* sal, const float* mask, i64 nvox, float fraction,
                            float* thr_out);
+struct SelectState;
+int select_workspace(visfd_hip_ctx* ctx, uint64_t** hist, SelectState** state);
+int dev_select_pick(visfd_hip_ctx* ctx, const uint64_t* hist_dev, int round, float fraction, SelectState* state);
+int dev_select_finish(visfd_hip_ctx* ctx, const float* sal, const float* mask, i64 nvox, float fraction, float* thr_out);
 
 int dev_tv_dense_stick(visfd_hip_ctx* ctx, const float* sal, const float* dir_planar,
                        float* tensor_planar, const float* mask_src, const float* mask_dst, i64 nx,
                        i64 ny, i64 nz, i64 z_out0, i64 z_out1, float sigma_tv, int exponent,
-                       float cutoff, bool curves);
+                       float cutoff, bool curves, float thr = -__builtin_inff(), float* sal_rw = nullptr);
 
 int dev_tv_weight_sum(visfd_hip_ctx* ctx, const float* sal, float* den, const float* mask_src, const float* mask_dst, i64 nx,
                       i64 ny, i64 nz, float sigma_tv, float cutoff);
diff --git a/visfd_amd/csrc/context.hip b/visfd_amd/csrc/context.hip
--- a/visfd_amd/csrc/context.hip
+++ b/visfd_amd/csrc/context.hip
@@ -45,7 +45,7 @@
     {"tv_no_replay", &visfd_hip_options::tv_no_replay, nullptr}, {"tv_max_wg", &visfd_hip_options::tv_max_wg, nullptr},
     {"tv_poison", &visfd_hip_options::tv_poison, nullptr}, {"tv_no_fold", &visfd_hip_options::tv_no_fold, nullptr}, {"tv_exact_tiled", &visfd_hip_options::tv_exact_tiled, nullptr}, {"tv_reserve_wg", &visfd_hip_options::tv_reserve_wg, nullptr},
     {"blob_test_cap", nullptr, &visfd_hip_options::blob_test_cap}, {"debug", &visfd_hip_options::debug, nullptr},
-    {"morph_general", &visfd_hip_options::morph_general, nullptr},
+    {"morph_general", &visfd_hip_options::morph_general, nullptr}, {"ridge_no_tile", &visfd_hip_options::ridge_no_tile, nullptr},
 };
 bool set_option(visfd_hip_options* o, const char* name, int64_t value) {
   for (const OptionDesc& d : kOptions) {
diff --git a/visfd_amd/csrc/ridge.hip b/visfd_amd/csrc/ridge.hip
--- a/visfd_amd/csrc/ridge.hip
+++ b/visfd_amd/csrc/ridge.hip
@@ -1,5 +1,8 @@
+#include <algorithm>
+
 #include "common.hpp"
 #include "eigen3.hpp"
+#include "select_dev.hpp"
 
 namespace vh {
 
@@ -16,7 +19,16 @@
   }
 };
 
-__device__ __forceinline__ void hessian_at(const Stencil& f, float s2, float h6[6]) {
+constexpr int SCORE_ROWS = 4;
+constexpr int TILE_W = BLOCK + 3;
+constexpr int TILE_H = SCORE_ROWS + 3;
+struct TileStencil {
+  const float* c;
+  __device__ __forceinline__ float at(int dx, int dy, int dz) const { return c[(dz * TILE_H + dy) * TILE_W + dx]; }
+};
+
+template <typename St>
+__device__ __forceinline__ void hessian_at(const St& f, float s2, float h6[6]) {
   const float f0 = f.at(0, 0, 0);
   const float two_f0 = 2 * f0;
   const float hxx = (f.at(1, 0, 0) + f.at(-1, 0, 0)) - two_f0;
@@ -124,35 +136,87 @@
   dir[2 * nvox + v] = d[2];
 }
 
-template <bool F32>
-__global__ void __launch_bounds__(BLOCK)
+template <bool F32, bool TILE>
+__global__ void __launch_bounds__(BLOCK) __attribute__((amdgpu_waves_per_eu(F32 ? 5 : 4)))
 ridge_score_kernel(const float* __restrict__ S, const float* __restrict__ mask, int nx, int ny, int nz,
                    float sigma, int order, float* __restrict__ sal,
-                   const float* __restrict__ peak_img, const float* __restrict__ peak_bg) {
-  int ix, iy, iz;
-  if (!voxel_of_block(nx, ny, ix, iy, iz)) return;
-  const i64 v = ((i64)iz * ny + iy) * nx + ix;
-  if (mask && mask[v] == 0.0f) { sal[v] = 0.0f; return; }
-  const Stencil f = clamped_stencil(S, ix, iy, iz, nx, ny, nz);
-  float h6[6];
-  hessian_at(f, sigma * sigma, h6);
-  double lam[3];
-  eig::D3 E[3];
-  eig::eig_sym3<F32>(h6, order, lam, E, false);
-  const double l1 = (float)lam[0], l2 = (float)lam[1];
-  double N = l1 * l1 - l2 * l2;
-  N *= N;
-  float score = (float)N;
-  if (peak_img) score *= peak_img[v] - peak_bg[v];
-  __builtin_nontemporal_store(score, &sal[v]);
+                   const float* __restrict__ peak_img, const float* __restrict__ peak_bg,
+                   unsigned long long* __restrict__ hist, i64 nunits) {
+  __shared__ float tile[TILE ? 3 * TILE_H * TILE_W : 1];
+  __shared__ unsigned int lh[SELECT_NBINS];
+  const int tid = threadIdx.x;
+  if (hist) {
+    for (int i = tid; i < SELECT_NBINS; i += BLOCK) lh[i] = 0;
+    __syncthreads();
+  }
+  const int xblocks = (nx + BLOCK - 1) / BLOCK, yblocks = (ny + SCORE_ROWS - 1) / SCORE_ROWS;
+  const i64 plane = (i64)nx * ny;
+  const float s2 = sigma * sigma;
+  for (i64 u = blockIdx.x; u < nunits; u += gridDim.x) {
+    const int bx = (int)(u % xblocks);
+    const i64 t = u / xblocks;
+    const int by = (int)(t % yblocks), iz = (int)(t / yblocks);
+    const int x0 = bx * BLOCK, y0 = by * SCORE_ROWS;
+    if (TILE) {
+      const int zc = min(max(iz, 1), nz - 2);
+      __syncthreads();
+#pragma unroll
+      for (int r = 0; r < 3 * TILE_H; r++) {
+        const int tp = r / TILE_H, ty = r - tp * TILE_H;
+        const int gy = y0 - 2 + ty;
+        if (gy < 0 || gy >= ny) continue;
+        const float* const row = S + (i64)(zc - 1 + tp) * plane + (i64)gy * nx;
+        for (int tx = tid; tx < TILE_W; tx += BLOCK) {
+          const int gx = x0 - 2 + tx;
+          if (gx >= 0 && gx < nx) tile[r * TILE_W + tx] = row[gx];
+        }
+      }
+      __syncthreads();
+    }
+    const int ix = x0 + tid;
+    if (ix >= nx) continue;
+    const int xc = min(max(ix, 1), nx - 2);
+#pragma unroll 1
+    for (int j = 0; j < SCORE_ROWS; j++) {
+      const int iy = y0 + j;
+      if (iy >= ny) break;
+      const i64 v = ((i64)iz * ny + iy) * nx + ix;
+      if (mask && mask[v] == 0.0f) { sal[v] = 0.0f; continue; }
+      float h6[6];
+      if (TILE) {
+        const int yc = min(max(iy, 1), ny - 2);
+        const TileStencil f = {tile + (TILE_H + (yc - y0 + 2)) * TILE_W + (xc - x0 + 2)};
+        hessian_at(f, s2, h6);
+      } else {
+        hessian_at(clamped_stencil(S, ix, iy, iz, nx, ny, nz), s2, h6);
+      }
+      double lam[3];
+      eig::D3 E[3];
+      eig::eig_sym3<F32>(h6, order, lam, E, false);
+      const double l1 = (float)lam[0], l2 = (float)lam[1];
+      double N = l1 * l1 - l2 * l2;
+      N *= N;
+      float score = (float)N;
+      if (peak_img) score *= peak_img[v] - peak_bg[v];
+      __builtin_nontemporal_store(score, &sal[v]);
+      if (hist) atomicAdd(&lh[select_bin(select_order_key(score), 0)], 1u);
+    }
+  }
+  if (hist) {
+    __syncthreads();
+    for (int i = tid; i < SELECT_NBINS; i += BLOCK) {
+      const unsigned int c = lh[i];
+      if (c) atomicAdd(&hist[i], (unsigned long long)c);
+    }
+  }
 }
 
 constexpr int DIR_PER = 16;
 constexpr int DIR_CHUNK = DIR_PER * BLOCK;
 template <bool F32>
 __global__ void __launch_bounds__(BLOCK)
-ridge_directions_kernel(const float* __restrict__ S, const float* __restrict__ sal, int nx, int ny, int nz,
-                        float sigma, int order, float* __restrict__ dir) {
+ridge_directions_kernel(const float* __restrict__ S, const float* __restrict__ sal, float thr ,
+                        int nx, int ny, int nz, float sigma, int order, float* __restrict__ dir) {
   __shared__ unsigned short list[DIR_CHUNK];
   __shared__ int wave_tot[BLOCK / 64];
   const i64 nvox = (i64)nx * ny * nz;
@@ -163,7 +227,7 @@
 #pragma unroll
   for (int k = 0; k < DIR_PER; k++) {
     const i64 v = base + k * BLOCK + tid;
-    const bool kp = v < nvox && sal[v] != 0.0f;
+    const bool kp = v < nvox && select_survives(sal[v], thr);
     keep |= (kp ? 1u : 0u) << k;
     cnt += kp ? 1 : 0;
   }
@@ -313,24 +377,32 @@
 }
 
 int dev_ridge_score(visfd_hip_ctx* ctx, const float* S, const float* mask, i64 nx, i64 ny, i64 nz, float sigma,
-                    int order, float* sal, const float* peak_img, const float* peak_bg) {
+                    int order, float* sal, const float* peak_img, const float* peak_bg, uint64_t* hist_dev) {
   if (nx < 3 || ny < 3 || nz < 3)
     return fail(VISFD_HIP_EINVAL, "ridge detection requires an image at least 3 voxels wide in x,y,z");
-  unsigned g;
-  VH_TRY(voxel_grid(nx, ny, nz, &g));
-  VH_EIG_LAUNCH(ridge_score_kernel, dim3(g), S, mask, (int)nx, (int)ny, (int)nz, sigma, order, sal, peak_img, peak_bg);
+  if (nx >= (1LL << 31) || ny >= (1LL << 31) || nz >= (1LL << 31)) return fail(VISFD_HIP_EINVAL, "dimension too large");
+  const i64 nunits = ((nx + BLOCK - 1) / BLOCK) * ((ny + SCORE_ROWS - 1) / SCORE_ROWS) * nz;
+  const unsigned g = (unsigned)std::min<i64>(nunits, (i64)ctx->num_cus * 20);
+  unsigned long long* const hist = reinterpret_cast<unsigned long long*>(hist_dev);
+  if (hist) VH_HIP(hipMemsetAsync(hist, 0, sizeof(unsigned long long) * SELECT_NBINS, ctx->stream));
+#define VH_SCORE_LAUNCH(F32, TILE)                                                                               \
+  ridge_score_kernel<F32, TILE><<<dim3(g), dim3(BLOCK), 0, ctx->stream>>>(S, mask, (int)nx, (int)ny, (int)nz, sigma, order, sal, \
+                                                                          peak_img, peak_bg, hist, nunits)
+  if (ctx->opt.ridge_no_tile) { if (ctx->opt.eig_f32) VH_SCORE_LAUNCH(true, false); else VH_SCORE_LAUNCH(false, false); }
+  else                        { if (ctx->opt.eig_f32) VH_SCORE_LAUNCH(true, true); else VH_SCORE_LAUNCH(false, true); }
+#undef VH_SCORE_LAUNCH
   VH_HIP(hipGetLastError());
   return VISFD_HIP_OK;
 }
 
 int dev_ridge_directions(visfd_hip_ctx* ctx, const float* S, const float* sal, i64 nx, i64 ny, i64 nz, float sigma,
-                         int order, float* dir) {
+                         int order, float* dir, float thr) {
   if (nx < 3 || ny < 3 || nz < 3)
     return fail(VISFD_HIP_EINVAL, "ridge detection requires an image at least 3 voxels wide in x,y,z");
   if (nx >= (1LL << 31) || ny >= (1LL << 31) || nz >= (1LL << 31)) return fail(VISFD_HIP_EINVAL, "dimension too large");
   const i64 nb = (nx * ny * nz + DIR_CHUNK - 1) / DIR_CHUNK;
   if (nb > 0x7fffffffLL) return fail(VISFD_HIP_EINVAL, "volume too large for one launch");
-  VH_EIG_LAUNCH(ridge_directions_kernel, dim3((unsigned)nb), S, sal, (int)nx, (int)ny, (int)nz, sigma, order, dir);
+  VH_EIG_LAUNCH(ridge_directions_kernel, dim3((unsigned)nb), S, sal, thr, (int)nx, (int)ny, (int)nz, sigma, order, dir);
   VH_HIP(hipGetLastError());
   return VISFD_HIP_OK;
 }
diff --git a/visfd_amd/csrc/select.hip b/visfd_amd/csrc/select.hip
--- a/visfd_amd/csrc/select.hip
+++ b/visfd_amd/csrc/select.hip
@@ -2,18 +2,15 @@
 #include <vector>
 
 #include "common.hpp"
+#include "select_dev.hpp"
 
 namespace vh {
 
 namespace {
 
 constexpr int BLOCK = 256;
-constexpr int NBINS = 2048;
+constexpr int NBINS = SELECT_NBINS;
 
-__device__ __forceinline__ uint32_t order_key(float f) {
-  const uint32_t u = __float_as_uint(f);
-  return (u & 0x80000000u) ? ~u : (u | 0x80000000u);
-}
 inline float key_to_float(uint32_t k) {
   const uint32_t u = (k & 0x80000000u) ? (k & 0x7fffffffu) : ~k;
   float f;
@@ -23,17 +20,16 @@
 
 __global__ void __launch_bounds__(BLOCK)
 histogram_kernel(const float* __restrict__ sal, const float* __restrict__ mask, i64 n, int round,
-                 uint32_t prefix, unsigned long long* __restrict__ hist) {
+                 uint32_t prefix, const SelectState* __restrict__ state, unsigned long long* __restrict__ hist) {
   __shared__ unsigned int lh[NBINS];
   for (int i = threadIdx.x; i < NBINS; i += BLOCK) lh[i] = 0;
   __syncthreads();
-  const int shift = (round == 0) ? 21 : (round == 1) ? 10 : 0;
-  const uint32_t dmask = (round == 2) ? 0x3ffu : 0x7ffu;
+  if (state) prefix = state->prefix;
   const int pshift = (round == 0) ? 32 : (round == 1) ? 21 : 10;
   auto count = [&](float v) {
-    const uint32_t k = order_key(v);
+    const uint32_t k = select_order_key(v);
     if (round > 0 && (k >> pshift) != prefix) return;
-    atomicAdd(&lh[(k >> shift) & dmask], 1u);
+    atomicAdd(&lh[select_bin(k, round)], 1u);
   };
   const i64 step = (i64)gridDim.x * BLOCK;
   const i64 n4 = (!mask && (reinterpret_cast<uintptr_t>(sal) & 15u) == 0) ? (n >> 2) : 0;
@@ -59,6 +55,43 @@
   }
 }
 
+constexpr int PICK_PER = NBINS / BLOCK;
+__global__ void __launch_bounds__(BLOCK)
+select_pick_kernel(const unsigned long long* __restrict__ hist, int round, float fraction, SelectState* __restrict__ state) {
+  __shared__ unsigned long long lh[NBINS];
+  __shared__ unsigned long long group[BLOCK];
+  unsigned long long sum = 0;
+#pragma unroll
+  for (int j = 0; j < PICK_PER; j++) {
+    const unsigned long long c = hist[threadIdx.x * PICK_PER + j];
+    lh[threadIdx.x * PICK_PER + j] = c;
+    sum += c;
+  }
+  group[threadIdx.x] = sum;
+  __syncthreads();
+  if (threadIdx.x != 0) return;
+  SelectState s = *state;
+  if (round == 0) {
+    uint64_t n = 0;
+    for (int g = 0; g < BLOCK; g++) n += group[g];
+    uint64_t k = 0;
+    s.status = select_rank(n, fraction, &k) ? SELECT_OK : SELECT_NO_VOXEL;
+    s.k = k;
+    s.prefix = 0;
+  }
+  if (s.status == SELECT_OK) {
+    uint64_t k = s.k;
+    const int g = select_pick_descending(group, BLOCK, &k);
+    const int b = g < 0 ? -1 : select_pick_descending(lh + g * PICK_PER, PICK_PER, &k);
+    if (b < 0) s.status = SELECT_INCONSISTENT;
+    else {
+      s.prefix = (s.prefix << select_digit_bits(round)) | (uint32_t)(g * PICK_PER + b);
+      s.k = k;
+    }
+  }
+  *state = s;
+}
+
 __global__ void __launch_bounds__(BLOCK)
 apply_threshold_kernel(float* __restrict__ sal, i64 n, float thr) {
   i64 i = (i64)blockIdx.x * BLOCK + threadIdx.x;
@@ -74,11 +107,11 @@
 int dev_select_histogram(visfd_hip_ctx* ctx, const float* sal, const float* mask, i64 nvox, int pass,
                          uint32_t prefix, uint64_t* hist_host, uint64_t* n_unmasked_host) {
   unsigned long long* hist = nullptr;
-  VH_TRY(ws(ctx, WS_HIST, (size_t)NBINS, &hist));
+  VH_TRY(ws(ctx, WS_HIST, (size_t)NBINS + 2, &hist));
   hipStream_t st = ctx->stream;
   VH_HIP(hipMemsetAsync(hist, 0, sizeof(unsigned long long) * NBINS, st));
   const unsigned g = grid_for(nvox, BLOCK, (i64)ctx->num_cus * 32);
-  histogram_kernel<<<dim3(g), dim3(BLOCK), 0, st>>>(sal, mask, nvox, pass, prefix, hist);
+  histogram_kernel<<<dim3(g), dim3(BLOCK), 0, st>>>(sal, mask, nvox, pass, prefix, nullptr, hist);
   VH_HIP(hipGetLastError());
   VH_HIP(hipMemcpyAsync(hist_host, hist, sizeof(uint64_t) * NBINS, hipMemcpyDeviceToHost, st));
   VH_HIP(hipStreamSynchronize(st));
@@ -95,7 +128,7 @@
   hipStream_t st = ctx->stream;
   VH_HIP(hipMemsetAsync(hist_dev, 0, sizeof(unsigned long long) * NBINS, st));
   const unsigned g = grid_for(nvox, BLOCK, (i64)ctx->num_cus * 32);
-  histogram_kernel<<<dim3(g), dim3(BLOCK), 0, st>>>(sal, mask, nvox, pass, prefix, reinterpret_cast<unsigned long long*>(hist_dev));
+  histogram_kernel<<<dim3(g), dim3(BLOCK), 0, st>>>(sal, mask, nvox, pass, prefix, nullptr, reinterpret_cast<unsigned long long*>(hist_dev));
   VH_HIP(hipGetLastError());
   return VISFD_HIP_OK;
 }
@@ -107,38 +140,54 @@
   return VISFD_HIP_OK;
 }
 
-static int pick_bin_descending(const std::vector<uint64_t>& h, uint64_t* k) {
-  uint64_t seen = 0;
-  for (int b = NBINS - 1; b >= 0; b--) {
-    if (seen + h[b] > *k) { *k -= seen; return b; }
-    seen += h[b];
-  }
-  return -1;
+int select_pick_digit(const uint64_t* hist, uint64_t* k) { return select_pick_descending(hist, NBINS, k); }
+float select_key_to_float(uint32_t key) { return key_to_float(key); }
+
+int select_workspace(visfd_hip_ctx* ctx, uint64_t** hist, SelectState** state) {
+  unsigned long long* p = nullptr;
+  VH_TRY(ws(ctx, WS_HIST, (size_t)NBINS + 2, &p));
+  *hist = reinterpret_cast<uint64_t*>(p);
+  if (state) *state = reinterpret_cast<SelectState*>(p + NBINS);
+  return VISFD_HIP_OK;
 }
 
-int select_pick_digit(const uint64_t* hist, uint64_t* k) {
-  return pick_bin_descending(std::vector<uint64_t>(hist, hist + NBINS), k);
+int dev_select_pick(visfd_hip_ctx* ctx, const uint64_t* hist_dev, int round, float fraction, SelectState* state) {
+  select_pick_kernel<<<dim3(1), dim3(BLOCK), 0, ctx->stream>>>(reinterpret_cast<const unsigned long long*>(hist_dev), round,
+                                                                fraction, state);
+  VH_HIP(hipGetLastError());
+  return VISFD_HIP_OK;
 }
-float select_key_to_float(uint32_t key) { return key_to_float(key); }
+
+int dev_select_finish(visfd_hip_ctx* ctx, const float* sal, const float* mask, i64 nvox, float fraction, float* thr_out) {
+  uint64_t* hist = nullptr;
+  SelectState* state = nullptr;
+  VH_TRY(select_workspace(ctx, &hist, &state));
+  hipStream_t st = ctx->stream;
+  const unsigned g = grid_for(nvox, BLOCK, (i64)ctx->num_cus * 32);
+  VH_TRY(dev_select_pick(ctx, hist, 0, fraction, state));
+  for (int round = 1; round <= 2; round++) {
+    VH_HIP(hipMemsetAsync(hist, 0, sizeof(uint64_t) * NBINS, st));
+    histogram_kernel<<<dim3(g), dim3(BLOCK), 0, st>>>(sal, mask, nvox, round, 0u, state, reinterpret_cast<unsigned long long*>(hist));
+    VH_HIP(hipGetLastError());
+    VH_TRY(dev_select_pick(ctx, hist, round, fraction, state));
+  }
+  SelectState s;
+  VH_HIP(hipMemcpyAsync(&s, state, sizeof(s), hipMemcpyDeviceToHost, st));
+  VH_HIP(hipStreamSynchronize(st));
+  if (s.status == SELECT_NO_VOXEL)
+    return fail(VISFD_HIP_EINVAL, "threshold fraction selects no voxel (the reference would read past its array)");
+  if (s.status != SELECT_OK) return fail(VISFD_HIP_EDEVICE, "radix select: inconsistent histogram");
+  *thr_out = key_to_float(s.prefix);
+  return VISFD_HIP_OK;
+}
 
 int dev_threshold_fraction(visfd_hip_ctx* ctx, float* sal, const float* mask, i64 nvox, float fraction,
                            float* thr_out) {
-  std::vector<uint64_t> h(NBINS);
-  uint64_t n_unmasked = 0;
-  VH_TRY(dev_select_histogram(ctx, sal, mask, nvox, 0, 0, h.data(), &n_unmasked));
-  const float prod = (float)n_unmasked * fraction;
-  uint64_t k = (uint64_t)std::floor(prod);
-  if (n_unmasked == 0 || k >= n_unmasked)
-    return fail(VISFD_HIP_EINVAL, "threshold fraction selects no voxel (the reference would read past its array)");
-  const int d0 = pick_bin_descending(h, &k);
-  if (d0 < 0) return fail(VISFD_HIP_EDEVICE, "radix select: inconsistent histogram");
-  VH_TRY(dev_select_histogram(ctx, sal, mask, nvox, 1, (uint32_t)d0, h.data(), nullptr));
-  const int d1 = pick_bin_descending(h, &k);
-  if (d1 < 0) return fail(VISFD_HIP_EDEVICE, "radix select: inconsistent histogram");
-  VH_TRY(dev_select_histogram(ctx, sal, mask, nvox, 2, ((uint32_t)d0 << 11) | (uint32_t)d1, h.data(), nullptr));
-  const int d2 = pick_bin_descending(h, &k);
-  if (d2 < 0) return fail(VISFD_HIP_EDEVICE, "radix select: inconsistent histogram");
-  const float thr = key_to_float(((uint32_t)d0 << 21) | ((uint32_t)d1 << 10) | (uint32_t)d2);
+  uint64_t* hist = nullptr;
+  VH_TRY(select_workspace(ctx, &hist, nullptr));
+  VH_TRY(dev_select_histogram_todev(ctx, sal, mask, nvox, 0, 0, hist));
+  float thr = 0.0f;
+  VH_TRY(dev_select_finish(ctx, sal, mask, nvox, fraction, &thr));
   if (thr_out) *thr_out = thr;
   return dev_apply_threshold(ctx, sal, nvox, thr);
 }
diff --git a/visfd_amd/csrc/select_dev.hpp b/visfd_amd/csrc/select_dev.hpp
--- /dev/null
+++ b/visfd_amd/csrc/select_dev.hpp
@@ -0,0 +1,47 @@
+#pragma once
+
+#include "common.hpp"
+
+namespace vh {
+
+constexpr int SELECT_NBINS = 2048;
+
+#define VH_THR_NONE (-__builtin_inff())
+__host__ __device__ __forceinline__ bool select_survives(float v, float thr) { return !(v < thr) && v != 0.0f; }
+
+__device__ __forceinline__ uint32_t select_order_key(float f) {
+  const uint32_t u = __float_as_uint(f);
+  return (u & 0x80000000u) ? ~u : (u | 0x80000000u);
+}
+__host__ __device__ __forceinline__ int select_shift(int round) { return round == 0 ? 21 : round == 1 ? 10 : 0; }
+__host__ __device__ __forceinline__ uint32_t select_digit_mask(int round) { return round == 2 ? 0x3ffu : 0x7ffu; }
+__host__ __device__ __forceinline__ int select_digit_bits(int round) { return round == 2 ? 10 : 11; }
+__device__ __forceinline__ uint32_t select_bin(uint32_t key, int round) {
+  return (key >> select_shift(round)) & select_digit_mask(round);
+}
+
+template <typename T>
+__host__ __device__ inline int select_pick_descending(const T* h, int nb, uint64_t* k) {
+  uint64_t seen = 0;
+  for (int b = nb - 1; b >= 0; b--) {
+    const uint64_t c = (uint64_t)h[b];
+    if (seen + c > *k) { *k -= seen; return b; }
+    seen += c;
+  }
+  return -1;
+}
+
+__host__ __device__ inline bool select_rank(uint64_t n, float fraction, uint64_t* k) {
+  const float prod = (float)n * fraction;
+  *k = (uint64_t)floorf(prod);
+  return n != 0 && *k < n;
+}
+
+struct SelectState {
+  unsigned long long k;
+  uint32_t prefix;
+  uint32_t status;
+};
+enum { SELECT_OK = 0, SELECT_NO_VOXEL = 1, SELECT_INCONSISTENT = 2 };
+
+}
diff --git a/visfd_amd/csrc/tv.hip b/visfd_amd/csrc/tv.hip
--- a/visfd_amd/csrc/tv.hip
+++ b/visfd_amd/csrc/tv.hip
@@ -1,6 +1,7 @@
 #include <vector>
 
 #include "common.hpp"
+#include "select_dev.hpp"
 
 namespace vh {
 
@@ -108,7 +109,7 @@
 
 int dev_tv_box(visfd_hip_ctx* ctx, const float* sal, const float* dir, float* ten, const float* mask_src,
                const float* mask_dst, i64 nx, i64 ny, i64 nz, i64 z_out0, i64 z_out1, int h, const float4* dtab_box,
-               int exponent, bool* handled, bool exact);
+               int exponent, bool* handled, bool exact, float thr);
 
 
 static int tv_table_device(visfd_hip_ctx* ctx, float sigma_tv, float cutoff, int h, const float4** out) {
@@ -146,9 +147,12 @@
 
 int dev_tv_dense_stick(visfd_hip_ctx* ctx, const float* sal, const float* dir, float* ten,
                        const float* mask_src, const float* mask_dst, i64 nx, i64 ny, i64 nz,
-                       i64 z_out0, i64 z_out1, float sigma_tv, int exponent, float cutoff, bool curves) {
+                       i64 z_out0, i64 z_out1, float sigma_tv, int exponent, float cutoff, bool curves, float thr, float* sal_rw) {
   VH_TRY(check_dims(nx, ny, nz));
   VH_TRY(check_dims32(nx, ny, nz));
+  const bool cut = !(thr == VH_THR_NONE);
+  VH_REQUIRE(!cut || sal_rw == sal, "a threshold needs the saliency volume writable");
+  ctx->tv_last_senders = -1;
   VH_REQUIRE(z_out0 >= 0 && z_out1 <= nz && z_out0 <= z_out1, "bad receiver plane range");
   if (z_out0 == z_out1) return VISFD_HIP_OK;
   const int h = host_tv_halfwidth(sigma_tv, cutoff);
@@ -161,12 +165,13 @@
   bool handled = false;
   if (!ctx->opt.tv_dense && ctx->opt.tv_fma && !curves)
     VH_TRY(dev_tv_box(ctx, sal, dir, ten, mask_src, mask_dst, nx, ny, nz, z_out0, z_out1, h, dtab + m_packed + m_padded, exponent,
-                      &handled, false));
+                      &handled, false, thr));
   if (handled) return VISFD_HIP_OK;
   if (!ctx->opt.tv_dense && !ctx->opt.tv_exact_tiled && !curves)
     VH_TRY(dev_tv_box(ctx, sal, dir, ten, mask_src, mask_dst, nx, ny, nz, z_out0, z_out1, h,
-                      dtab + m_packed + m_padded + (size_t)(2 * h + 2) * (size_t)tv_box_slice(h), exponent, &handled, true));
-  if (handled) return VISFD_HIP_OK;
+                      dtab + m_packed + m_padded + (size_t)(2 * h + 2) * (size_t)tv_box_slice(h), exponent, &handled, true, thr));
+  if (handled) return VISFD_HIP_OK;
+  if (cut) VH_TRY(dev_apply_threshold(ctx, sal_rw, nx * ny * nz, thr));
   if (!ctx->opt.tv_dense)
     VH_TRY(dev_tv_tiled(ctx, sal, dir, ten, mask_src, mask_dst, nx, ny, nz, z_out0, z_out1, h, dtab + m_packed, exponent, curves,
                         false, &handled));
diff --git a/visfd_amd/csrc/tv_box.hip b/visfd_amd/csrc/tv_box.hip
--- a/visfd_amd/csrc/tv_box.hip
+++ b/visfd_amd/csrc/tv_box.hip
@@ -3,6 +3,7 @@
 #include <vector>
 
 #include "common.hpp"
+#include "select_dev.hpp"
 
 namespace vh {
 
@@ -794,7 +795,8 @@
 
 template <bool WRITE, int MODE>
 __global__ void __launch_bounds__(LNT)
-tvl_row_kernel(const float* __restrict__ sal, const float* __restrict__ dir, const float* __restrict__ mask_src, ListGeo g,
+tvl_row_kernel(const float* __restrict__ sal, float thr , const float* __restrict__ dir,
+               const float* __restrict__ mask_src, ListGeo g,
                unsigned* __restrict__ rows, float4* __restrict__ ent, unsigned* __restrict__ pos,
                unsigned* __restrict__ neg_flag ,
                int fold ) {
@@ -828,7 +830,7 @@
 #pragma unroll
     for (int k = 0; k < LB; k++) {
       if (c0 + k >= nchunks) break;
-      const bool f = v[k] != 0.0f && m[k] != 0.0f;
+      const bool f = select_survives(v[k], thr) && m[k] != 0.0f;
       const unsigned long long bal = __builtin_amdgcn_ballot_w64(f);
       if (lane == 0) {
         bits[2 * (c0 + k)] = (unsigned)bal;
@@ -924,7 +926,7 @@
 
 int dev_tv_box(visfd_hip_ctx* ctx, const float* sal, const float* dir, float* ten, const float* mask_src,
                const float* mask_dst, i64 nx, i64 ny, i64 nz, i64 z_out0, i64 z_out1, int h, const float4* dtab_box,
-               int exponent, bool* handled, bool exact) {
+               int exponent, bool* handled, bool exact, float thr) {
   *handled = false;
   if (exponent != 2 && exponent != 4) return VISFD_HIP_OK;
   if (h < 1 || h > 40) return VISFD_HIP_OK;
@@ -971,9 +973,9 @@
   const unsigned row_blocks = (unsigned)(((i64)g.nzl * ny + LNT / 64 - 1) / (LNT / 64));
 #define VH_TVL_ROWS(WR, ENT, POS)                                                                                         \
   do {                                                                                                                    \
-    if (exact) tvl_row_kernel<WR, 1><<<dim3(row_blocks), dim3(LNT), 0, st>>>(sal, dir, mask_src, g, rows, ENT, POS, counter + 6, 0);             \
-    else if (exponent == 4) tvl_row_kernel<WR, 0><<<dim3(row_blocks), dim3(LNT), 0, st>>>(sal, dir, mask_src, g, rows, ENT, POS, counter + 6, fold); \
-    else tvl_row_kernel<WR, 2><<<dim3(row_blocks), dim3(LNT), 0, st>>>(sal, dir, mask_src, g, rows, ENT, POS, counter + 6, fold);             \
+    if (exact) tvl_row_kernel<WR, 1><<<dim3(row_blocks), dim3(LNT), 0, st>>>(sal, thr, dir, mask_src, g, rows, ENT, POS, counter + 6, 0);             \
+    else if (exponent == 4) tvl_row_kernel<WR, 0><<<dim3(row_blocks), dim3(LNT), 0, st>>>(sal, thr, dir, mask_src, g, rows, ENT, POS, counter + 6, fold); \
+    else tvl_row_kernel<WR, 2><<<dim3(row_blocks), dim3(LNT), 0, st>>>(sal, thr, dir, mask_src, g, rows, ENT, POS, counter + 6, fold);             \
   } while (0)
   int fold = 0;
   VH_TVL_ROWS(false, nullptr, nullptr);
@@ -983,6 +985,7 @@
   VH_HIP(hipMemcpyAsync(tot2, total_dev, sizeof(tot2), hipMemcpyDeviceToHost, st));
   VH_HIP(hipStreamSynchronize(st));
   const unsigned long long total = tot2[0];
+  ctx->tv_last_senders = (int64_t)total;
   fold = ((unsigned)tot2[1] & 1u) ? 0 : 1;
   if (ctx->opt.tv_no_fold) fold = 0;
   if (exact && ((unsigned)tot2[1] & 2u)) return VISFD_HIP_OK;
diff --git a/visfd_amd/pipeline.py b/visfd_amd/pipeline.py
--- a/visfd_amd/pipeline.py
+++ b/visfd_amd/pipeline.py
@@ -47,15 +47,6 @@
                     mask=None, scratch=None, sigma_background=0.0, background=None):
     order = api.DECREASING_EIVALS if minima else api.INCREASING_EIVALS
     ratio = api.ratio_from_threshold(truncate_threshold)
-    smoothed = scratch if scratch is not None else src.new_empty(src.shape)
-    bg = None
-    if sigma_background > 0:
-        bg = background if background is not None else src.new_empty(src.shape)
-        ctx.peak_background_dev(src, bg, sigma_background, ratio, mask)
-    ctx.ridge_scores_dev(src, sal, smoothed, sigma, ratio, order, mask, bg)
-    thr = ctx.threshold_fraction_dev(sal, best_fraction, mask)
-    ctx.ridge_directions_dev(smoothed, sal, dirs, sigma, order)
     sigma_tv = float(np.float32(tv_sigma_ratio) * np.float32(sigma))
-    ctx.tv_dense_stick_dev(sal, dirs, tensor, sigma_tv, tv_exponent, tv_truncate_ratio, mask, mask)
-    ctx.tensor_saliency_dev(tensor, sal, order, mask, src if bg is not None else None, bg)
-    return thr
+    return ctx.membrane_stage_dev(src, sal, sigma, ratio, order, best_fraction, 0.0, sigma_tv, tv_exponent, tv_truncate_ratio,
+                                  mask, dirs, tensor, scratch, background if sigma_background > 0 else None, sigma_background)
```

Measured after the change: 2487. 0.981x the previous value.
